# ViacheslavDanilov/oct_segmentation

Measured on AMD Instinct MI355X. Metric: OCT frames/sec (704x704, bf16) fwd+bwd, higher is better.
Workload: dtype bf16; 1 GPU; unetplusplus/resnet101 1-class 704x704, batch 16/GPU, fwd+Dice+bwd+allreduce+Adam; global_batch=16, parallelism=dp1

## Files before the change

include/octseg.h:

```cpp
#ifndef OCTSEG_H
#define OCTSEG_H
#include <stddef.h>
#include <stdint.h>

#ifdef __cplusplus
extern "C" {
#endif

typedef enum {
  OCTSEG_OK = 0,
  OCTSEG_BAD_SHAPE = -1,
  OCTSEG_BAD_DTYPE = -2,
  OCTSEG_UNSUPPORTED_ARCH = -3,
  OCTSEG_HIP_ERROR = -4,
  OCTSEG_BAD_ARG = -5
} octseg_status;

typedef enum { OCTSEG_F32 = 0, OCTSEG_BF16 = 1, OCTSEG_F16 = 2 } octseg_dtype;

typedef struct {
  const char* arch;
  const char* encoder;
  int classes;
  int batch, height, width;
  int dtype;
} octseg_net_desc;

typedef struct octseg_plan octseg_plan;

enum {
  OCTSEG_P_CONV = 0,
  OCTSEG_P_CONVT = 1,
  OCTSEG_P_STEM = 2,
  OCTSEG_P_VEC = 3
};
typedef struct {
  char name[128];
  int kind;
  int R, S, O, I, KP;
  size_t offset;
  size_t numel;
} octseg_param_info;
typedef struct {
  char name[128];
  int C;
  size_t mean_offset, var_offset;
} octseg_bn_info;

int octseg_version(void);
const char* octseg_last_error(void);

int octseg_plan_create(const octseg_net_desc* desc, octseg_plan** out);
int octseg_plan_destroy(octseg_plan* plan);
size_t octseg_plan_workspace_bytes(const octseg_plan* plan);
size_t octseg_plan_param_numel(const octseg_plan* plan);
size_t octseg_plan_buffer_numel(const octseg_plan* plan);
int octseg_plan_num_params(const octseg_plan* plan);
int octseg_plan_param_info(const octseg_plan* plan, int index, octseg_param_info* out);
int octseg_plan_num_bn(const octseg_plan* plan);
int octseg_plan_bn_info(const octseg_plan* plan, int index, octseg_bn_info* out);
double octseg_plan_fwd_macs(const octseg_plan* plan);
int octseg_plan_exec_macs(const octseg_plan* plan, double* out3);
int octseg_plan_find_tensor(const octseg_plan* plan, const char* conv_name, size_t* act_off,
                            size_t* grad_off, int* dims);

int octseg_profile_start(void);
int octseg_profile_stop(double* out);

int octseg_plan_params_changed(octseg_plan* plan);

int octseg_plan_set_dropout(octseg_plan* plan, const float* keep_dev);

int octseg_plan_set_drop_connect(octseg_plan* plan, const float* factors_dev);
int octseg_plan_num_drop_connect(const octseg_plan* plan);
float octseg_plan_drop_connect_rate(const octseg_plan* plan, int index);

int octseg_plan_set_graph(octseg_plan* plan, int enable);

int octseg_net_forward(octseg_plan* plan, const float* params, float* buffers, void* workspace,
                       const float* image, float* logits, int normalize, const float* mean,
                       const float* stdv, int train, void* stream);

#define OCTSEG_AUG_NPARAM 36
int octseg_augment(const float* img, const float* mask, float* img_out, float* mask_out, const float* params, int B,
                   int classes, int H, int W, void* stream);

int octseg_mask_assemble(const float* logits, int N, int classes, int H, int W, int ch, float* out, int out_h, int out_w,
                         int out_channels, int out_ch, const int* row_index, const int* col_index, void* stream);

#define OCTSEG_VOTE_MAX_MEMBERS 64
#define OCTSEG_VOTE_SOFT 0
#define OCTSEG_VOTE_MAJORITY 1
int octseg_vote_assemble(const float* const* logits, const int* classes, const int* ch, const int* view, int M, int N, int H, int W, int mode,
                         float* out, int out_h, int out_w, int out_channels, int out_ch, const int* row_index, const int* col_index, float* prob,
                         uint8_t* dissent, int* stats, void* stream);

#define OCTSEG_CURVE_BINS 256
int octseg_logit_histogram(const float* logits, const float* target, int N, int classes, int H, int W,
                           int* hist, void* stream);

int octseg_ingest_image(const uint8_t* src, int B, int src_h, int src_w, int swap_rb, float* out, int dst_h, int dst_w, const int* xtab,
                        const int* ytab, void* stream);
int octseg_ingest_mask(const uint8_t* src, int B, int src_h, int src_w, int src_channels, const int* channel_ids, int C, float* out, int dst_h,
                       int dst_w, const int* row_index, const int* col_index, void* stream);
int octseg_debug_set_ingest_variant(int variant);

int octseg_render_results(const float* stack, const uint8_t* frames, int N, int H, int W, int stack_channels, const int* class_channels,
                          const uint8_t* class_rgb, int C, const uint8_t* alpha_table, int ring_alpha, int close_iterations, uint8_t* overlay,
                          uint8_t* color_mask, void* stream);

int octseg_epoch_panels(const float* frames, const float* logits, const uint8_t* gt, int N, int S, int C, int src_h, int src_w, int src_channels,
                        const int* row_index, const int* col_index, const int* gt_channels, const uint8_t* class_rgb, const uint8_t* class_ids,
                        uint8_t* panels, uint8_t* labels, void* stream);

int octseg_stack_measure(const float* stack, int N, int H, int W, int stack_channels, const int* ray_pix, const int* ray_len, int R, int* counts,
                         int* radii, void* stream);

int octseg_stack_polar(const float* stack, int N, int H, int W, int stack_channels, const int* ray_pix, const int* ray_len, int R,
                       int* prof, unsigned char* map , void* stream);
int octseg_frames_unwrap(const unsigned char* frames, int N, int H, int W, int channels, const int* ray_pix, const int* ray_len, int R,
                         unsigned char* out, void* stream);

#define OCTSEG_MOMENT_FIELDS 12
#define OCTSEG_SHAPE_MAX_EXTENT 32768
int octseg_stack_moments(const float* stack, int N, int H, int W, int channels, long long* mom, void* stream);
int octseg_moment_origins(const float* stack, const long long* mom, int N, int H, int W, int channels, int ref_channel ,
                          int* origins, void* stream);
int octseg_stack_polar_at(const float* stack, int N, int H, int W, int channels, const int* origins, const int* ray_off, int R, int* prof,
                          int* len, void* stream);

size_t octseg_components_scratch_bytes(int planes, int H, int W);
int octseg_stack_components(const float* stack, int N, int H, int W, int channels, void* scratch, size_t scratch_bytes, int* labels, int* ncomp,
                            int* top, void* stream);
int octseg_stack_cleanup(const float* stack, int N, int H, int W, int channels, int smooth_k, int keep, int min_area, int fill_holes, void* scratch,
                         size_t scratch_bytes, float* out, int* ncomp, int* top, void* stream);

#define OCTSEG_CONTOUR_FIELDS 10
#define OCTSEG_CONTOUR_MAX_VERTICES (1 << 29)
int octseg_stack_contour_counts(const float* stack, int N, int H, int W, int channels, long long* counts, void* stream);
size_t octseg_contours_scratch_bytes(int planes, int H, int W, long long edge_capacity);
int octseg_stack_contours(const float* stack, int N, int H, int W, int channels, void* scratch, size_t scratch_bytes, long long edge_capacity,
                          long long contour_capacity, long long vertex_capacity, int* ncont, int* table, int* vertices, int* overflow,
                          void* stream);

#define OCTSEG_ACROSS_OVERLAP 0
#define OCTSEG_ACROSS_FULL 1
size_t octseg_lesions_scratch_bytes(int channels, int N, int H, int W);
int octseg_volume_components(const float* stack, int N, int H, int W, int channels, int across, void* scratch, size_t scratch_bytes, int* labels,
                             int* nles, int* top, int* profile, void* stream);
int octseg_volume_cleanup(const float* stack, int N, int H, int W, int channels, int across, int keep, int min_voxels, int min_slices, void* scratch,
                          size_t scratch_bytes, float* out, int* nles, int* top, void* stream);

// ... 40 lines not shown
                         const int* xkk, int xksize, const int* ybounds, const int* ykk, int yksize, void* stream);

int octseg_plan_set_frozen_bn(octseg_plan* plan, int on);
int octseg_plan_cam_target(const octseg_plan* plan, size_t* act_off, size_t* grad_off, int* dims);
int octseg_net_backward_seeded(octseg_plan* plan, const float* params, void* workspace, const float* dlogits, void* stream);
size_t octseg_cam_scratch_bytes(int N, int h, int w, int K);
int octseg_cam_maps(int dtype, const void* A, const void* G, int N, int h, int w, int K, int method, int S, void* scratch, float* maps,
                    float threshold, uint8_t* bin, const uint8_t* gt, int gt_h, int gt_w, const int* row_index, const int* col_index, int* counts,
                    const float* frames, const uint8_t* jet_bgr, double image_weight, uint8_t* overlay, void* stream);

int octseg_cam_overlay(const float* maps, const float* frames, const uint8_t* jet_bgr, int N, int S, double image_weight, uint8_t* overlay,
                       void* scratch, void* stream);

typedef enum { OCTSEG_LOSS_DICE = 0, OCTSEG_LOSS_BCE = 1, OCTSEG_LOSS_DICE_BCE = 2 } octseg_loss_kind;
int octseg_plan_set_loss(octseg_plan* plan, int kind);

int octseg_dice_forward(octseg_plan* plan, void* workspace, const float* logits, const float* target,
                        float* loss, long long* stats, void* stream);

int octseg_net_backward(octseg_plan* plan, const float* params, float* grads, void* workspace,
                        const float* logits, const float* target, float grad_scale, void* stream);

int octseg_net_train_step(octseg_plan* plan, const float* params, float* grads, float* buffers, void* workspace, const float* image,
                          const float* target, float* logits, float* loss, long long* stats, int normalize, const float* mean,
                          const float* stdv, float grad_scale, void* stream);
int octseg_plan_set_train_graph(octseg_plan* plan, int enable);

typedef void (*octseg_slice_cb)(void* user, int slice, size_t begin, size_t end);
int octseg_net_backward_sliced(octseg_plan* plan, const float* params, float* grads, void* workspace, const float* logits,
                               const float* target, float grad_scale, void* stream, int nslices, void* comm_stream,
                               octseg_slice_cb cb, void* user);

int octseg_optim_step(int kind, float* params, const float* grads, float* state_m, float* state_v,
                      size_t numel, float lr, float weight_decay, int step, float grad_scale,
                      void* stream);

int octseg_set_deterministic(int on);

int octseg_debug_set_stamp(unsigned long long* dev_buf);
int octseg_debug_set_serial(int on);

size_t octseg_conv2d_scratch_bytes(int dtype, int N, int H, int W, int Cin, int Cout, int R, int S);
int octseg_conv2d_forward(int dtype, const void* x, const float* w, const float* bias, void* y, int N,
                          int H, int W, int Cin, int Cout, int R, int S, int stride, int pad,
                          int transposed, void* scratch, void* stream);
int octseg_conv2d_backward_data(int dtype, const void* dy, const float* w, void* dx, int N, int H, int W,
                                int Cin, int Cout, int R, int S, int stride, int pad, int transposed,
                                void* scratch, void* stream);
int octseg_conv2d_backward_weight(int dtype, const void* x, const void* dy, float* dw, int N, int H,
                                  int W, int Cin, int Cout, int R, int S, int stride, int pad,
                                  int transposed, void* stream);

#define OCTSEG_CONV_MAX_SRC 5
typedef enum { OCTSEG_CONV_FORWARD = 0, OCTSEG_CONV_BACKWARD_DATA = 1, OCTSEG_CONV_BACKWARD_WEIGHT = 2 } octseg_conv_mode;
typedef enum { OCTSEG_ROUTE_THIN = 0, OCTSEG_ROUTE_GEMM1X1, OCTSEG_ROUTE_CONV3X3P, OCTSEG_ROUTE_MFMA16, OCTSEG_ROUTE_MFMA11,
               OCTSEG_ROUTE_MFMA_WIDEN,
               OCTSEG_ROUTE_MFMA11_MASKED, OCTSEG_ROUTE_MFMA16_MASKED } octseg_conv_route;
typedef enum { OCTSEG_WROUTE_THIN = 0, OCTSEG_WROUTE_WGRAD1X1, OCTSEG_WROUTE_CONVT16, OCTSEG_WROUTE_MFMA } octseg_wgrad_route;
typedef struct {
  const void* ptr; const float* scale; const float* shift;
  int C, H, W, up, relu;
} octseg_conv_src;
typedef struct { void* ptr; int accum, pool; } octseg_conv_dst;
typedef struct {
  int N, H, W, Cin, Cout, R, stride, pad, transposed;
  int nsrc;
  octseg_conv_src src[OCTSEG_CONV_MAX_SRC];
  const float* w; const float* wscale; const float* bias;
  int relu_out;
  float* stat_slab; int slab_row0;
  int head;
  octseg_conv_dst dst[OCTSEG_CONV_MAX_SRC];
  const void* dy; float* dW;
  void* scratch; size_t scratch_bytes;
} octseg_conv_layer_desc;
int octseg_conv_layer_op(int mode, int dtype, const octseg_conv_layer_desc* desc, void* stream);
int octseg_conv_layer_route(int mode, int dtype, const octseg_conv_layer_desc* desc, int* route_per_launch, int* nlaunch);
int octseg_conv_layer_slab_rows(int dtype, const octseg_conv_layer_desc* desc, int* rows);

int octseg_tied_layer_op(int pass, int dtype, const octseg_conv_layer_desc* desc, int wg_target, void* stream);
int octseg_tied_layer_route(int pass, int dtype, const octseg_conv_layer_desc* desc, int wg_target, int* route_per_launch, int* nlaunch);
size_t octseg_tied_layer_scratch_bytes(int dtype, const octseg_conv_layer_desc* desc);
int octseg_side_wgs(void);

typedef enum { OCTSEG_STEM_IM2COL = 0, OCTSEG_STEM_FORWARD = 1, OCTSEG_STEM_WGRAD = 2 } octseg_stem_stage;
typedef struct {
  int N, H, W;
  const float* img;
  int normalize; float mean[3], stdv[3];
  int ksize, pad, KP; void* col;
  const float* w; const float* wscale; const float* bias; int relu_out;
  void* y; float* stat_slab; int slab_row0;
  const void* dy; float* dW;
} octseg_stem_desc;
int octseg_stem_op(int stage, int dtype, const octseg_stem_desc* desc, void* stream);
int octseg_stem_slab_rows(int N, int H, int W);

typedef enum {
  OCTSEG_SWEEP_BN_FINALIZE_TRAIN = 0,
  OCTSEG_SWEEP_BN_FINALIZE_SMALL,
  OCTSEG_SWEEP_BN_FINALIZE_EVAL,
  OCTSEG_SWEEP_BN_FINALIZE_FROZEN,
  OCTSEG_SWEEP_BN_ACT,
  OCTSEG_SWEEP_BN_BWD_SMALL,
  OCTSEG_SWEEP_BN_BWD_REDUCE,
  OCTSEG_SWEEP_BN_BWD_FINALIZE,
  OCTSEG_SWEEP_BN_BWD_APPLY,
  OCTSEG_SWEEP_MASKED_ACCUM,
  OCTSEG_SWEEP_POOL2X2_ACCUM,
  OCTSEG_SWEEP_UP2_FILL,
  OCTSEG_SWEEP_RELU,
  OCTSEG_SWEEP_ADD2,
  OCTSEG_SWEEP_DROP_ELEM,
  OCTSEG_SWEEP_MERGE_DROP,
  OCTSEG_SWEEP_DROP_BWD,
  OCTSEG_SWEEP_CHANNEL_SUM,
  OCTSEG_SWEEP_TENSOR_STATS,
  OCTSEG_SWEEP_MAXPOOL_FWD,
  OCTSEG_SWEEP_MAXPOOL_BWD_IDX,
  OCTSEG_SWEEP_BILINEAR_RESIZE,
  OCTSEG_SWEEP_BILINEAR_RESIZE_ADJOINT,
  OCTSEG_SWEEP_BILINEAR_ADJOINT,
  OCTSEG_SWEEP_BIN_MEAN,
  OCTSEG_SWEEP_BIN_MEAN_BWD,
  OCTSEG_SWEEP_IMAGE_SUM,
  OCTSEG_SWEEP_IMAGE_BCAST,
  OCTSEG_SWEEP_SE_GATE,
  OCTSEG_SWEEP_SE_DGATE,
  OCTSEG_SWEEP_PARITY_PERMUTE,
  OCTSEG_SWEEP_MOSAIC,
  OCTSEG_SWEEP_DW_CONV,
  OCTSEG_SWEEP_DW_WGRAD,
  OCTSEG_SWEEP_CAM_SEED,
  OCTSEG_SWEEP_DWG_FWD,
  OCTSEG_SWEEP_DWG_BWD_DATA,
  OCTSEG_SWEEP_DWG_BWD_W,
  OCTSEG_SWEEP_BNX_FWD,
  OCTSEG_SWEEP_BNX_BWD,
  OCTSEG_SWEEP_DICE_BWD,
  OCTSEG_SWEEP_GN_FORWARD,
  OCTSEG_SWEEP_GN_BACKWARD,
  OCTSEG_SWEEP_SEFC_FWD,
  OCTSEG_SWEEP_SEFC_BWD,
  OCTSEG_SWEEP_NUM_OPS
} octseg_sweep;
int octseg_sweep_op(int op, int dtype, const void* const* ptrs, int nptrs, const long long* iargs, int niargs, const double* fargs,
                    int nfargs, void* stream);

typedef enum { OCTSEG_FPA_MAXPOOL2_FWD = 0, OCTSEG_FPA_MAXPOOL2_BWD, OCTSEG_FPA_IN_FWD, OCTSEG_FPA_IN_BWD, OCTSEG_FPA_PYR_FWD, OCTSEG_FPA_PYR_BWD,
               OCTSEG_FPA_MIX_FWD, OCTSEG_FPA_MIX_BWD, OCTSEG_FPA_NUM_STAGES } octseg_fpa_stage;
typedef struct {
  int N, H, W, C, K, train, accum;
  const void* x; void* p; void* dp; void* dx;
  const float* w; const float* b; float* y; const float* dy; float* dw; float* db;
  float* scratch; size_t scratch_floats; float* gscratch; size_t gscratch_floats;
  const float* pw[6]; const float* pb[6]; const float* pg[6]; const float* pbe[6]; float* prm[6]; float* prv[6];
  float* pdw[6]; float* pdb[6]; float* pdg[6]; float* pdbe[6];
  const float* uu; float* duu;
  const void* mid; const void* b1; void* out; const void* g; void* dmid;
} octseg_fpa_desc;
size_t octseg_fpa_scratch_floats(int N, int H, int W);
size_t octseg_fpa_gscratch_floats(int N, int H, int W);
size_t octseg_fpa_uu_offset(int N, int H, int W);
int octseg_fpa_op(int stage, int dtype, const octseg_fpa_desc* desc, void* stream);

typedef enum { OCTSEG_PAB_GEMM = 0, OCTSEG_PAB_SOFTMAX_FWD, OCTSEG_PAB_SOFTMAX_BWD, OCTSEG_PAB_MIX_FWD, OCTSEG_PAB_MIX_BWD, OCTSEG_PAB_NUM_STAGES } octseg_pab_stage;
// ... 17 lines not shown
```

oct_segmentation_amd/_lib.py:

```python
import ctypes as C
import os

def set_hw_queues_for_collectives():
    os.environ.setdefault('GPU_MAX_HW_QUEUES', '8')


if int(os.environ.get('WORLD_SIZE', '1') or 1) > 1:
    set_hw_queues_for_collectives()

import torch

_HERE = os.path.dirname(os.path.abspath(__file__))
LIB_PATH = os.path.join(_HERE, 'liboctseg_hip.so')

F32, BF16, F16 = 0, 1, 2
P_CONV, P_CONVT, P_STEM, P_VEC = 0, 1, 2, 3
OPT_KINDS = {'SGD': 0, 'Adam': 1, 'RMSprop': 2, 'RAdam': 3}


class NetDesc(C.Structure):
    _fields_ = [('arch', C.c_char_p), ('encoder', C.c_char_p), ('classes', C.c_int), ('batch', C.c_int),
                ('height', C.c_int), ('width', C.c_int), ('dtype', C.c_int)]


class ParamInfo(C.Structure):
    _fields_ = [('name', C.c_char * 128), ('kind', C.c_int), ('R', C.c_int), ('S', C.c_int), ('O', C.c_int),
                ('I', C.c_int), ('KP', C.c_int), ('offset', C.c_size_t), ('numel', C.c_size_t)]


class BNInfo(C.Structure):
    _fields_ = [('name', C.c_char * 128), ('C', C.c_int), ('mean_offset', C.c_size_t), ('var_offset', C.c_size_t)]


class ConvSrc(C.Structure):
    _fields_ = [('ptr', C.c_void_p), ('scale', C.c_void_p), ('shift', C.c_void_p), ('C', C.c_int), ('H', C.c_int), ('W', C.c_int),
                ('up', C.c_int), ('relu', C.c_int)]


class ConvDst(C.Structure):
    _fields_ = [('ptr', C.c_void_p), ('accum', C.c_int), ('pool', C.c_int)]


CONV_MAX_SRC = 5


class ConvLayerDesc(C.Structure):
    _fields_ = [('N', C.c_int), ('H', C.c_int), ('W', C.c_int), ('Cin', C.c_int), ('Cout', C.c_int), ('R', C.c_int), ('stride', C.c_int),
                ('pad', C.c_int), ('transposed', C.c_int), ('nsrc', C.c_int), ('src', ConvSrc * CONV_MAX_SRC), ('w', C.c_void_p),
                ('wscale', C.c_void_p), ('bias', C.c_void_p), ('relu_out', C.c_int), ('stat_slab', C.c_void_p), ('slab_row0', C.c_int),
                ('head', C.c_int), ('dst', ConvDst * CONV_MAX_SRC), ('dy', C.c_void_p), ('dW', C.c_void_p), ('scratch', C.c_void_p),
                ('scratch_bytes', C.c_size_t)]


class StemDesc(C.Structure):
    _fields_ = [('N', C.c_int), ('H', C.c_int), ('W', C.c_int), ('img', C.c_void_p), ('normalize', C.c_int), ('mean', C.c_float * 3),
                ('stdv', C.c_float * 3), ('ksize', C.c_int), ('pad', C.c_int), ('KP', C.c_int), ('col', C.c_void_p), ('w', C.c_void_p),
                ('wscale', C.c_void_p), ('bias', C.c_void_p), ('relu_out', C.c_int), ('y', C.c_void_p), ('stat_slab', C.c_void_p),
                ('slab_row0', C.c_int), ('dy', C.c_void_p), ('dW', C.c_void_p)]


_PF6 = C.c_void_p * 6


class FpaDesc(C.Structure):
    _fields_ = ([(k, C.c_int) for k in ('N', 'H', 'W', 'C', 'K', 'train', 'accum')] +
                [(k, C.c_void_p) for k in ('x', 'p', 'dp', 'dx', 'w', 'b', 'y', 'dy', 'dw', 'db')] +
                [('scratch', C.c_void_p), ('scratch_floats', C.c_size_t), ('gscratch', C.c_void_p), ('gscratch_floats', C.c_size_t)] +
                [(k, _PF6) for k in ('pw', 'pb', 'pg', 'pbe', 'prm', 'prv', 'pdw', 'pdb', 'pdg', 'pdbe')] +
                [(k, C.c_void_p) for k in ('uu', 'duu', 'mid', 'b1', 'out', 'g', 'dmid')])


class PabGemm(C.Structure):
    _fields_ = ([(k, C.c_void_p) for k in ('A', 'B', 'C')] +
                [(k, C.c_size_t) for k in ('sAb', 'sAm', 'sAk', 'sBb', 'sBk', 'sBn', 'sCb', 'sCm', 'sCn')] +
                [(k, C.c_int) for k in ('M', 'N', 'K', 'batch', 'a_f32', 'b_f32', 'c_f32', 'accum')])


class PabDesc(C.Structure):
    _fields_ = [('gemm', PabGemm), ('numelA', C.c_size_t), ('numelB', C.c_size_t), ('numelC', C.c_size_t),
                ('S', C.c_void_p), ('P', C.c_void_p), ('batch', C.c_int), ('n', C.c_size_t),
                ('x', C.c_void_p), ('M', C.c_void_p), ('y', C.c_void_p), ('dM', C.c_void_p), ('dy', C.c_void_p), ('N', C.c_int), ('HW', C.c_int),
                ('C', C.c_int)]


_P = C.c_void_p
LOSS_KINDS = {'dice': 0, 'bce': 1, 'dice+bce': 2}
SLICE_CB = C.CFUNCTYPE(None, C.c_void_p, C.c_int, C.c_size_t, C.c_size_t)
SYMBOLS = {
    'octseg_version': (C.c_int, []),
    'octseg_last_error': (C.c_char_p, []),
    'octseg_plan_create': (C.c_int, [C.POINTER(NetDesc), C.POINTER(_P)]),
    'octseg_plan_destroy': (C.c_int, [_P]),
    'octseg_plan_workspace_bytes': (C.c_size_t, [_P]),
    'octseg_plan_param_numel': (C.c_size_t, [_P]),
    'octseg_plan_buffer_numel': (C.c_size_t, [_P]),
    'octseg_plan_num_params': (C.c_int, [_P]),
    'octseg_plan_param_info': (C.c_int, [_P, C.c_int, C.POINTER(ParamInfo)]),
    'octseg_plan_num_bn': (C.c_int, [_P]),
    'octseg_plan_bn_info': (C.c_int, [_P, C.c_int, C.POINTER(BNInfo)]),
    'octseg_plan_fwd_macs': (C.c_double, [_P]),
    'octseg_plan_exec_macs': (C.c_int, [_P, C.POINTER(C.c_double)]),
    'octseg_plan_find_tensor': (C.c_int, [_P, C.c_char_p, C.POINTER(C.c_size_t), C.POINTER(C.c_size_t), C.POINTER(C.c_int)]),
    'octseg_profile_start': (C.c_int, []),
    'octseg_profile_stop': (C.c_int, [C.POINTER(C.c_double)]),
    'octseg_plan_params_changed': (C.c_int, [_P]),
    'octseg_plan_set_dropout': (C.c_int, [_P, _P]),
    'octseg_plan_set_drop_connect': (C.c_int, [_P, _P]),
    'octseg_plan_num_drop_connect': (C.c_int, [_P]),
    'octseg_plan_drop_connect_rate': (C.c_float, [_P, C.c_int]),
    'octseg_plan_set_graph': (C.c_int, [_P, C.c_int]),
    'octseg_net_forward': (C.c_int, [_P, _P, _P, _P, _P, _P, C.c_int, C.POINTER(C.c_float), C.POINTER(C.c_float),
                                     C.c_int, _P]),
    'octseg_augment': (C.c_int, [_P, _P, _P, _P, _P, C.c_int, C.c_int, C.c_int, C.c_int, _P]),
    'octseg_mask_assemble': (C.c_int, [_P, C.c_int, C.c_int, C.c_int, C.c_int, C.c_int, _P, C.c_int, C.c_int, C.c_int, C.c_int, _P, _P, _P]),
    'octseg_vote_assemble': (C.c_int, [_P, _P, _P, _P] + [C.c_int] * 5 + [_P] + [C.c_int] * 4 + [_P] * 6),
    'octseg_logit_histogram': (C.c_int, [_P, _P] + [C.c_int] * 4 + [_P, _P]),
    'octseg_ingest_image': (C.c_int, [_P, C.c_int, C.c_int, C.c_int, C.c_int, _P, C.c_int, C.c_int, _P, _P, _P]),
    'octseg_ingest_mask': (C.c_int, [_P, C.c_int, C.c_int, C.c_int, C.c_int, _P, C.c_int, _P, C.c_int, C.c_int, _P, _P, _P]),
    'octseg_debug_set_ingest_variant': (C.c_int, [C.c_int]),
    'octseg_render_results': (C.c_int, [_P, _P, C.c_int, C.c_int, C.c_int, C.c_int, _P, _P, C.c_int, _P, C.c_int, C.c_int, _P, _P, _P]),
    'octseg_epoch_panels': (C.c_int, [_P, _P, _P] + [C.c_int] * 6 + [_P] * 8),
    'octseg_stack_measure': (C.c_int, [_P, C.c_int, C.c_int, C.c_int, C.c_int, _P, _P, C.c_int, _P, _P, _P]),
    'octseg_stack_polar': (C.c_int, [_P, C.c_int, C.c_int, C.c_int, C.c_int, _P, _P, C.c_int, _P, _P, _P]),
    'octseg_frames_unwrap': (C.c_int, [_P, C.c_int, C.c_int, C.c_int, C.c_int, _P, _P, C.c_int, _P, _P]),
    'octseg_stack_moments': (C.c_int, [_P] + [C.c_int] * 4 + [_P, _P]),
    'octseg_moment_origins': (C.c_int, [_P, _P] + [C.c_int] * 5 + [_P, _P]),
    'octseg_stack_polar_at': (C.c_int, [_P] + [C.c_int] * 4 + [_P, _P, C.c_int, _P, _P, _P]),
    'octseg_components_scratch_bytes': (C.c_size_t, [C.c_int] * 3),
    'octseg_stack_components': (C.c_int, [_P] + [C.c_int] * 4 + [_P, C.c_size_t, _P, _P, _P, _P]),
    'octseg_stack_cleanup': (C.c_int, [_P] + [C.c_int] * 8 + [_P, C.c_size_t, _P, _P, _P, _P]),
    'octseg_stack_contour_counts': (C.c_int, [_P] + [C.c_int] * 4 + [_P, _P]),
    'octseg_contours_scratch_bytes': (C.c_size_t, [C.c_int] * 3 + [C.c_longlong]),
    'octseg_stack_contours': (C.c_int, [_P] + [C.c_int] * 4 + [_P, C.c_size_t] + [C.c_longlong] * 3 + [_P] * 5),
    'octseg_lesions_scratch_bytes': (C.c_size_t, [C.c_int] * 4),
    'octseg_volume_components': (C.c_int, [_P] + [C.c_int] * 5 + [_P, C.c_size_t, _P, _P, _P, _P, _P]),
    'octseg_volume_cleanup': (C.c_int, [_P] + [C.c_int] * 8 + [_P, C.c_size_t, _P, _P, _P, _P]),
    'octseg_match_scratch_bytes': (C.c_size_t, [C.c_int] * 4),
    'octseg_volume_match': (C.c_int, [_P, _P] + [C.c_int] * 5 + [_P, C.c_size_t, _P, _P, _P, _P, _P]),
    'octseg_distance_scratch_bytes': (C.c_size_t, [C.c_int] * 6),
    'octseg_stack_boundary': (C.c_int, [_P] + [C.c_int] * 4 + [_P, C.c_size_t, _P, _P]),
    'octseg_stack_distance': (C.c_int, [_P] + [C.c_int] * 5 + [_P, C.c_size_t, _P, _P]),
    'octseg_pair_distance_counts': (C.c_int, [_P, _P] + [C.c_int] * 5 + [_P] + [C.c_int] * 3 + [_P, C.c_size_t, _P, _P, _P]),
    'octseg_pair_distance_keys': (C.c_int, [_P, _P] + [C.c_int] * 5 + [_P] + [C.c_int] * 3 + [_P, C.c_size_t, C.c_longlong, _P, _P, C.c_longlong,
                                            _P, _P]),
    'octseg_pair_distance_min': (C.c_int, [_P, _P] + [C.c_int] * 5 + [_P] + [C.c_int] * 3 + [_P, C.c_size_t, _P, _P]),
    'octseg_volume_distance_scratch_bytes': (C.c_size_t, [C.c_int] * 7),
    'octseg_volume_boundary': (C.c_int, [_P] + [C.c_int] * 4 + [_P, C.c_size_t, _P, _P]),
    'octseg_volume_distance': (C.c_int, [_P] + [C.c_int] * 6 + [_P, C.c_size_t, _P, _P]),
    'octseg_volume_pair_distance_counts': (C.c_int, [_P, _P] + [C.c_int] * 5 + [_P] + [C.c_int] * 3 + [_P, C.c_size_t, _P, _P, _P]),
    'octseg_volume_pair_distance_keys': (C.c_int, [_P, _P] + [C.c_int] * 5 + [_P] + [C.c_int] * 4 + [_P, C.c_size_t, C.c_longlong, _P, _P,
                                                   C.c_longlong, _P, _P]),
    'octseg_volume_pair_distance_min': (C.c_int, [_P, _P] + [C.c_int] * 5 + [_P] + [C.c_int] * 4 + [_P, C.c_size_t, _P, _P]),
    'octseg_skeleton_scratch_bytes': (C.c_size_t, [C.c_int] * 4),
    'octseg_stack_skeleton': (C.c_int, [_P] + [C.c_int] * 5 + [_P, C.c_size_t, _P, _P, _P]),
    'octseg_volume_normalize': (C.c_int, [_P] + [C.c_int] * 6 + [_P, _P, _P]),
    'octseg_resize_pil_u8': (C.c_int, [_P] + [C.c_int] * 4 + [_P, _P, C.c_int, C.c_int, _P, _P, C.c_int, _P, _P, C.c_int, _P]),
    'octseg_plan_set_frozen_bn': (C.c_int, [_P, C.c_int]),
    'octseg_plan_cam_target': (C.c_int, [_P, C.POINTER(C.c_size_t), C.POINTER(C.c_size_t), C.POINTER(C.c_int)]),
    'octseg_net_backward_seeded': (C.c_int, [_P, _P, _P, _P, _P]),
    'octseg_cam_scratch_bytes': (C.c_size_t, [C.c_int] * 4),
    'octseg_cam_maps': (C.c_int, [C.c_int, _P, _P] + [C.c_int] * 6 + [_P, _P, C.c_float, _P, _P, C.c_int, C.c_int, _P, _P, _P, _P, _P, C.c_double, _P, _P]),
    'octseg_cam_overlay': (C.c_int, [_P, _P, _P, C.c_int, C.c_int, C.c_double, _P, _P, _P]),
    'octseg_plan_set_loss': (C.c_int, [_P, C.c_int]),
    'octseg_dice_forward': (C.c_int, [_P, _P, _P, _P, _P, _P, _P]),
    'octseg_net_backward': (C.c_int, [_P, _P, _P, _P, _P, _P, C.c_float, _P]),
    'octseg_net_train_step': (C.c_int, [_P, _P, _P, _P, _P, _P, _P, _P, _P, _P, C.c_int, C.POINTER(C.c_float), C.POINTER(C.c_float),
                                        C.c_float, _P]),
    'octseg_plan_set_train_graph': (C.c_int, [_P, C.c_int]),
    'octseg_net_backward_sliced': (C.c_int, [_P, _P, _P, _P, _P, _P, C.c_float, _P, C.c_int, _P, SLICE_CB, _P]),
    'octseg_optim_step': (C.c_int, [C.c_int, _P, _P, _P, _P, C.c_size_t, C.c_float, C.c_float, C.c_int, C.c_float, _P]),
    'octseg_set_deterministic': (C.c_int, [C.c_int]),
    'octseg_debug_set_stamp': (C.c_int, [_P]),
    'octseg_debug_set_serial': (C.c_int, [C.c_int]),
    'octseg_conv2d_scratch_bytes': (C.c_size_t, [C.c_int] * 8),
    'octseg_conv2d_forward': (C.c_int, [C.c_int, _P, _P, _P, _P] + [C.c_int] * 10 + [_P, _P]),
    'octseg_conv2d_backward_data': (C.c_int, [C.c_int, _P, _P, _P] + [C.c_int] * 10 + [_P, _P]),
    'octseg_conv2d_backward_weight': (C.c_int, [C.c_int, _P, _P, _P] + [C.c_int] * 10 + [_P]),
    'octseg_conv_layer_op': (C.c_int, [C.c_int, C.c_int, C.POINTER(ConvLayerDesc), _P]),
    'octseg_conv_layer_route': (C.c_int, [C.c_int, C.c_int, C.POINTER(ConvLayerDesc), C.POINTER(C.c_int), C.POINTER(C.c_int)]),
    'octseg_conv_layer_slab_rows': (C.c_int, [C.c_int, C.POINTER(ConvLayerDesc), C.POINTER(C.c_int)]),
    'octseg_tied_layer_op': (C.c_int, [C.c_int, C.c_int, C.POINTER(ConvLayerDesc), C.c_int, _P]),
    'octseg_tied_layer_route': (C.c_int, [C.c_int, C.c_int, C.POINTER(ConvLayerDesc), C.c_int, C.POINTER(C.c_int), C.POINTER(C.c_int)]),
    'octseg_tied_layer_scratch_bytes': (C.c_size_t, [C.c_int, C.POINTER(ConvLayerDesc)]),
    'octseg_side_wgs': (C.c_int, []),
    'octseg_stem_op': (C.c_int, [C.c_int, C.c_int, C.POINTER(StemDesc), _P]),
    'octseg_stem_slab_rows': (C.c_int, [C.c_int] * 3),
    'octseg_sweep_op': (C.c_int, [C.c_int, C.c_int, C.POINTER(_P), C.c_int, C.POINTER(C.c_longlong), C.c_int, C.POINTER(C.c_double), C.c_int, _P]),
    'octseg_fpa_scratch_floats': (C.c_size_t, [C.c_int] * 3),
    'octseg_fpa_gscratch_floats': (C.c_size_t, [C.c_int] * 3),
    'octseg_fpa_uu_offset': (C.c_size_t, [C.c_int] * 3),
    'octseg_fpa_op': (C.c_int, [C.c_int, C.c_int, C.POINTER(FpaDesc), _P]),
    'octseg_pab_op': (C.c_int, [C.c_int, C.c_int, C.POINTER(PabDesc), _P]),
}

_lib = None


def lib():
    global _lib
    if _lib is None:
        if not os.path.exists(LIB_PATH):
            raise RuntimeError(
                f'{LIB_PATH} not found: build it with `python -c "import __graft_entry__ as g; g.build()"` '
                f'(or `make -C oct_segmentation_amd/csrc`). There is no CPU fallback.')
        h = C.CDLL(LIB_PATH)
        for name, (res, args) in SYMBOLS.items():
            fn = getattr(h, name)
            fn.restype = res
            fn.argtypes = args
        _lib = h
    return _lib


def check(rc):
    if rc != 0:
        msg = lib().octseg_last_error().decode()
        if 'Expected more than 1 value per channel' in msg:
            raise ValueError(msg)
        raise RuntimeError(f'octseg error {rc}: {msg}')


def ptr(t):
    return None if t is None else C.c_void_p(t.data_ptr())


def stream_ptr():
    import torch
    return C.c_void_p(torch.cuda.current_stream().cuda_stream)
```

oct_segmentation_amd/csrc/api.cpp:

```cpp
#include "plan_internal.h"

#include <cctype>

using namespace octseg;
using namespace octseg::detail;

static std::string lower(const char* s) {
  std::string r(s ? s : "");
  for (auto& c : r) c = (char)tolower((unsigned char)c);
  return r;
}

template <class Outside, class Body>
static int graph_call(octseg_plan* p, bool train, bool same_key, hipGraphExec_t& exec, int& seen, hipStream_t st, Outside&& outside, Body&& body) {
  if (!same_key) {
    if (exec) { (void)hipGraphExecDestroy(exec); exec = nullptr; }
    seen = 0;
  }
  if (const int rc = outside()) return rc;
  auto replay = [&]() -> int { HIPCHK(hipGraphLaunch(exec, st)); if (train) p->packed_valid = false; return OCTSEG_OK; };
  if (exec) return replay();
  if (seen++ == 0) return body();
  if (train) p->packed_valid = false;
  hipGraph_t g = nullptr;
  HIPCHK(hipStreamBeginCapture(st, hipStreamCaptureModeThreadLocal));
  g_capturing = train;
  const int rc = body();
  g_capturing = false;
  const hipError_t ce = hipStreamEndCapture(st, &g);
  if (train) p->packed_valid = false;
  hipError_t ie = hipSuccess;
  if (!rc && ce == hipSuccess && (ie = hipGraphInstantiate(&exec, g, nullptr, nullptr, 0)) != hipSuccess) exec = nullptr;
  if (g) (void)hipGraphDestroy(g);
  if (rc) return rc;
  if (ce != hipSuccess) return fail(OCTSEG_HIP_ERROR, std::string(train ? "training-step capture: " : "") + hipGetErrorString(ce));
  if (ie != hipSuccess) return fail(OCTSEG_HIP_ERROR, hipGetErrorString(ie));
  return replay();
}

extern "C" {

int octseg_version(void) { return 100; }
const char* octseg_last_error(void) { return g_err.c_str(); }

int octseg_plan_create(const octseg_net_desc* d, octseg_plan** out) {
  if (!d || !out) return fail(OCTSEG_BAD_ARG, "null argument");
  *out = nullptr;
  if (d->dtype != OCTSEG_F32 && d->dtype != OCTSEG_BF16 && d->dtype != OCTSEG_F16) return fail(OCTSEG_BAD_DTYPE, "dtype must be f32, bf16 or f16");
  if (d->height <= 0 || d->width <= 0 || d->height % 32 != 0 || d->width % 32 != 0) {
    char buf[256];
    snprintf(buf, sizeof buf, "Wrong input shape height=%d, width=%d. Expected image height and width divisible by 32.",
             d->height, d->width);
    return fail(OCTSEG_BAD_SHAPE, buf);
  }
  if (d->batch <= 0 || d->classes <= 0 || d->classes > 16) return fail(OCTSEG_BAD_SHAPE, "batch > 0 and 1 <= classes <= 16 required");
  const std::string enc = lower(d->encoder);
  if (enc != "resnet18" && enc != "resnet34" && enc != "resnet50" && enc != "resnet101" && enc != "resnet152" && enc != "timm-regnetx_002" &&
      enc != "timm-regnetx_064" && enc != "timm-regnety_120" && enc != "efficientnet-b0" && enc != "efficientnet-b5" && enc != "efficientnet-b7")
    return fail(OCTSEG_UNSUPPORTED_ARCH, "unknown encoder '" + enc + "' (resnet18 | resnet34 | resnet50 | resnet101 | resnet152 | timm-regnetx_002 | timm-regnetx_064 | timm-regnety_120 | efficientnet-b0 | efficientnet-b5 | efficientnet-b7)");
  octseg_plan* P = new octseg_plan();
  P->arch = lower(d->arch); P->encoder = enc; P->classes = d->classes;
  P->B = d->batch; P->H = d->height; P->W = d->width; P->dtype = d->dtype;
  const int rc = build_plan(P);
  if (rc) { delete P; return rc; }
  *out = P;
  return OCTSEG_OK;
}
int octseg_plan_destroy(octseg_plan* p) {
  if (p) {
    if (p->side) (void)hipStreamDestroy(p->side);
    if (p->side_bwd) (void)hipStreamDestroy(p->side_bwd);
    if (p->ev_fork) (void)hipEventDestroy(p->ev_fork);
    if (p->ev_join) (void)hipEventDestroy(p->ev_join);
    if (p->ev_slice) (void)hipEventDestroy(p->ev_slice);
    if (p->graph_exec) (void)hipGraphExecDestroy(p->graph_exec);
    if (p->tgraph_exec) (void)hipGraphExecDestroy(p->tgraph_exec);
  }
  delete p;
  return OCTSEG_OK;
}
size_t octseg_plan_workspace_bytes(const octseg_plan* p) { return p ? p->ws_bytes : 0; }
size_t octseg_plan_param_numel(const octseg_plan* p) { return p ? p->param_numel : 0; }
size_t octseg_plan_buffer_numel(const octseg_plan* p) { return p ? p->buffer_numel : 0; }
int octseg_plan_num_params(const octseg_plan* p) { return p ? (int)p->params.size() : 0; }
int octseg_plan_num_bn(const octseg_plan* p) { return p ? (int)p->bns.size() : 0; }
double octseg_plan_fwd_macs(const octseg_plan* p) { return p ? p->fwd_macs : 0.0; }
int octseg_plan_exec_macs(const octseg_plan* p, double* out3) {
  if (p == nullptr || out3 == nullptr) return OCTSEG_BAD_ARG;
  for (int k = 0; k < 3; ++k) out3[k] = p->exec_macs[k];
  return OCTSEG_OK;
}

int octseg_plan_param_info(const octseg_plan* p, int i, octseg_param_info* o) {
  if (!p || !o || i < 0 || i >= (int)p->params.size()) return fail(OCTSEG_BAD_ARG, "param index out of range");
  const ParamInfo& q = p->params[i];
  memset(o, 0, sizeof(*o));
  snprintf(o->name, sizeof o->name, "%s", q.name.c_str());
  o->kind = q.kind; o->R = q.R; o->S = q.S; o->O = q.O; o->I = q.I; o->KP = q.KP; o->offset = q.off; o->numel = q.numel;
  return OCTSEG_OK;
}
int octseg_plan_bn_info(const octseg_plan* p, int i, octseg_bn_info* o) {
  if (!p || !o || i < 0 || i >= (int)p->bns.size()) return fail(OCTSEG_BAD_ARG, "bn index out of range");
  const BNInfo& b = p->bns[i];
  memset(o, 0, sizeof(*o));
  snprintf(o->name, sizeof o->name, "%s", b.name.c_str());
  o->C = b.C; o->mean_offset = b.rm_off; o->var_offset = b.rv_off;
  return OCTSEG_OK;
}

int octseg_profile_start(void) {
  for (auto& r : g_prof) { g_prof_pool.push_back(r.a); g_prof_pool.push_back(r.b); }
  g_prof.clear();
  g_prof_on = true;
  return OCTSEG_OK;
}
int octseg_profile_stop(double* out) {
  g_prof_on = false;
  if (!out) return fail(OCTSEG_BAD_ARG, "null argument");
  HIPCHK(hipDeviceSynchronize());
  for (int i = 0; i < 12; ++i) out[i] = 0.0;
  FILE* dump = nullptr;
  if (const char* path = getenv("OCTSEG_PROFILE_DUMP")) dump = fopen(path, "w");
  if (dump) fprintf(dump, "layer,class,ms,gflop,tflops\n");
  for (auto& r : g_prof) {
    float ms = 0.f;
    HIPCHK(hipEventElapsedTime(&ms, r.a, r.b));
    out[3 * r.kind] += ms; out[3 * r.kind + 1] += r.flops; out[3 * r.kind + 2] += 1.0;
    if (dump) fprintf(dump, "%s,%s,%.4f,%.3f,%.1f\n", r.name.c_str(), r.kind == 0 ? "fwd" : r.kind == 1 ? "dgrad" : r.kind == 2 ? "wgrad" : "hbm", ms,
                      r.flops / 1e9, ms > 0 ? r.flops / (ms * 1e-3) / 1e12 : 0.0);
  }
  if (dump) fclose(dump);
  for (auto& r : g_prof) { g_prof_pool.push_back(r.a); g_prof_pool.push_back(r.b); }
  g_prof.clear();
  return OCTSEG_OK;
}

int octseg_plan_find_tensor(const octseg_plan* p, const char* conv_name, size_t* act_off, size_t* grad_off, int* dims) {
  if (!p || !conv_name) return fail(OCTSEG_BAD_ARG, "null argument");
  for (auto& L : p->convs)
    if (L.name == conv_name && L.out >= 0) {
      const TensorInfo& t = p->tensors[L.out];
      if (act_off) *act_off = t.off;
      if (grad_off) *grad_off = t.goff;
      if (dims) { dims[0] = t.N; dims[1] = t.H; dims[2] = t.W; dims[3] = t.C; }
      return OCTSEG_OK;
    }
  return fail(OCTSEG_BAD_ARG, std::string("no conv layer named ") + conv_name);
}

int octseg_plan_params_changed(octseg_plan* p) {
  if (!p) return fail(OCTSEG_BAD_ARG, "null argument");
  p->packed_valid = false;
  return OCTSEG_OK;
}

int octseg_net_forward(octseg_plan* p, const float* params, float* buffers, void* workspace, const float* image,
                       float* logits, int normalize, const float* mean, const float* stdv, int train, void* stream) {
  if (!p || !params || !buffers || !workspace || !image || !logits) return fail(OCTSEG_BAD_ARG, "null argument");
  if (normalize && (!mean || !stdv)) return fail(OCTSEG_BAD_ARG, "normalize=1 needs mean/std");
  if (train && p->dtype == OCTSEG_F16)
    return fail(OCTSEG_BAD_DTYPE, "f16 is a serving dtype (eval forwards, reference predict.py); train in bf16 or f32");
  Exec E{p, params, nullptr, buffers, (char*)workspace, (hipStream_t)stream, train};
  if (train || !p->graph_enabled) return run_forward(E, image, logits, normalize, mean, stdv);
  octseg_plan::GraphKey key{params, buffers, workspace, image, logits, stream, normalize, {0, 0, 0}, {1, 1, 1}};
  if (normalize) for (int i = 0; i < 3; ++i) { key.mean[i] = mean[i]; key.stdv[i] = stdv[i]; }
  const bool same_key = key == p->graph_key;
  p->graph_key = key;
  return graph_call(p, false, same_key, p->graph_exec, p->graph_seen, E.st, [&] { return pack_all_weights(E, true); },
                    [&] { return run_forward(E, image, logits, normalize, mean, stdv); });
}

int octseg_plan_set_graph(octseg_plan* p, int enable) {
  if (!p) return fail(OCTSEG_BAD_ARG, "null argument");
  p->graph_enabled = enable != 0;
  if (!enable && p->graph_exec) { (void)hipGraphExecDestroy(p->graph_exec); p->graph_exec = nullptr; p->graph_seen = 0; }
  return OCTSEG_OK;
}

int octseg_plan_set_dropout(octseg_plan* p, const float* keep_dev) {
  if (!p) return fail(OCTSEG_BAD_ARG, "null argument");
  p->dropout_keep = keep_dev;
  return OCTSEG_OK;
}

int octseg_augment(const float* img, const float* mask, float* img_out, float* mask_out, const float* params, int B, int classes, int H,
                   int W, void* stream) {
  if (!img || !mask || !img_out || !mask_out || !params) return fail(OCTSEG_BAD_ARG, "null argument");
  if (B <= 0 || classes <= 0 || H <= 0 || W <= 0) return fail(OCTSEG_BAD_SHAPE, "augment: empty batch or frame");
  if (img == img_out || mask == mask_out) return fail(OCTSEG_BAD_ARG, "augment: outputs must not alias the inputs (gather)");
  HIPCHK(launch_augment(img, mask, img_out, mask_out, params, B, classes, H, W, (hipStream_t)stream));
  return OCTSEG_OK;
}

int octseg_mask_assemble(const float* logits, int N, int classes, int H, int W, int ch, float* out, int out_h, int out_w,
                         int out_channels, int out_ch, const int* row_index, const int* col_index, void* stream) {
  if (!logits || !out) return fail(OCTSEG_BAD_ARG, "null argument");
  if (N <= 0 || classes <= 0 || H <= 0 || W <= 0 || out_h <= 0 || out_w <= 0 || ch < 0 || ch >= classes || out_ch < 0 ||
      out_ch >= out_channels)
    return fail(OCTSEG_BAD_SHAPE, "mask_assemble: channel / extent out of range");
  HIPCHK(launch_mask_assemble(logits, N, classes, H, W, ch, out, out_h, out_w, out_channels, out_ch, row_index, col_index,
                              (hipStream_t)stream));
  return OCTSEG_OK;
}

static int g_ingest_variant = 0;
int octseg_debug_set_ingest_variant(int variant) {
  if (variant != 0 && variant != 1) return fail(OCTSEG_BAD_ARG, "ingest variant must be 0 (staged) or 1 (per-pixel gather)");
  g_ingest_variant = variant;
  return OCTSEG_OK;
}

int octseg_ingest_image(const uint8_t* src, int B, int src_h, int src_w, int swap_rb, float* out, int dst_h, int dst_w, const int* xtab,
                        const int* ytab, void* stream) {
  if (!src || !out || !xtab || !ytab) return fail(OCTSEG_BAD_ARG, "null argument");
  if (B <= 0 || src_h <= 0 || src_w <= 0 || dst_h <= 0 || dst_w <= 0) return fail(OCTSEG_BAD_SHAPE, "ingest_image: empty batch or frame");
  HIPCHK(launch_ingest_image(src, B, src_h, src_w, swap_rb != 0, out, dst_h, dst_w, xtab, ytab, g_ingest_variant, (hipStream_t)stream));
  return OCTSEG_OK;
}

int octseg_ingest_mask(const uint8_t* src, int B, int src_h, int src_w, int src_channels, const int* channel_ids, int C, float* out, int dst_h,
                       int dst_w, const int* row_index, const int* col_index, void* stream) {
  if (!src || !out || !channel_ids || !row_index || !col_index) return fail(OCTSEG_BAD_ARG, "null argument");
  if (B <= 0 || src_h <= 0 || src_w <= 0 || src_channels <= 0 || C <= 0 || dst_h <= 0 || dst_w <= 0)
    return fail(OCTSEG_BAD_SHAPE, "ingest_mask: empty batch, frame or class list");
  HIPCHK(launch_ingest_mask(src, B, src_h, src_w, src_channels, channel_ids, C, out, dst_h, dst_w, row_index, col_index, g_ingest_variant,
                            (hipStream_t)stream));
  return OCTSEG_OK;
}

int octseg_render_results(const float* stack, const uint8_t* frames, int N, int H, int W, int stack_channels, const int* class_channels,
                          const uint8_t* class_rgb, int C, const uint8_t* alpha_table, int ring_alpha, int close_iterations, uint8_t* overlay,
                          uint8_t* color_mask, void* stream) {
  if (!stack || !frames || !class_channels || !class_rgb || !alpha_table || !overlay || !color_mask) return fail(OCTSEG_BAD_ARG, "null argument");
  if (N <= 0 || H <= 0 || W <= 0 || stack_channels <= 0 || C <= 0 || C > 16)
    return fail(OCTSEG_BAD_SHAPE, "render_results: empty batch or frame, or not 1..16 classes");
// ... 386 lines not shown
```

oct_segmentation_amd/csrc/conv_api.cpp:

```cpp
#include "plan_internal.h"

using namespace octseg;
using namespace octseg::detail;

namespace {

struct Built {
  std::vector<ConvArgs> conv;
  std::vector<WgradArgs> wg;
  bool convt16 = false;
  ConvPackInfo pk{};
  int rows = 0;
};

bool aligned(const void* p) { return ((uintptr_t)p & 15) == 0; }

int build(int mode, int dtype, const octseg_conv_layer_desc* d, Built& B) {
  const std::string who = "conv_layer_op: ";
  auto bad_arg = [&](const char* m) { return fail(OCTSEG_BAD_ARG, who + m); };
  auto bad_shape = [&](const char* m) { return fail(OCTSEG_BAD_SHAPE, who + m); };
  if (mode != OCTSEG_CONV_FORWARD && mode != OCTSEG_CONV_BACKWARD_DATA && mode != OCTSEG_CONV_BACKWARD_WEIGHT) return bad_arg("unknown mode");
  if (dtype != OCTSEG_F32 && dtype != OCTSEG_BF16 && dtype != OCTSEG_F16) return fail(OCTSEG_BAD_DTYPE, who + "dtype must be f32, bf16 or f16");
  if (dtype == OCTSEG_F16 && mode != OCTSEG_CONV_FORWARD) return fail(OCTSEG_BAD_DTYPE, who + "f16 is the serving dtype: no gradient kernels");
  if (d == nullptr) return bad_arg("null descriptor");
// ... 158 lines not shown
  if (rc != OCTSEG_OK) return rc;
  int n = 0;
  if (mode == OCTSEG_CONV_BACKWARD_WEIGHT) {
    if (B.convt16) route_per_launch[n++] = OCTSEG_WROUTE_CONVT16;
    else
      for (auto& a : B.wg) {
        const WgradRoute r = wgrad_route(a, dtype);
        route_per_launch[n++] = a.ntaps <= 0 ? -1 : r == WROUTE_THIN ? OCTSEG_WROUTE_THIN : r == WROUTE_1X1 ? OCTSEG_WROUTE_WGRAD1X1 : OCTSEG_WROUTE_MFMA;
      }
  } else {
    for (auto& a : B.conv) route_per_launch[n++] = public_route(a, dtype);
  }
  *nlaunch = n;
  return OCTSEG_OK;
}

int octseg_conv_layer_slab_rows(int dtype, const octseg_conv_layer_desc* d, int* rows) {
  if (rows == nullptr) return fail(OCTSEG_BAD_ARG, "conv_layer_slab_rows: null output");
  Built B;
  const int rc = build(OCTSEG_CONV_FORWARD, dtype, d, B);
  if (rc != OCTSEG_OK) return rc;
  *rows = B.rows;
  return OCTSEG_OK;
}

}

namespace {

constexpr size_t TIE_TAB_BYTES = 512, TIE_PREFIX_BYTES = 512;
static_assert(4 * sizeof(PackJob) <= TIE_TAB_BYTES, "the job table fits its slot");

struct Tied {
  int Ca = 0, Cs = 0, ns = 0;
  Geom gu{}, gs{};
  TieImages im{};
  TieOffsets at{};
  size_t dk4_off = 0, bytes = 0;
  std::vector<PackJob> jobs; std::vector<unsigned long long> prefix; unsigned long long total = 0;
  std::vector<ConvArgs> conv;
  std::vector<WgradArgs> wg;
  bool convt16 = false, masked = false;
};

int tied_shape(int dtype, const octseg_conv_layer_desc* d, Tied& B) {
  const std::string who = "tied_layer_op: ";
  auto bad_shape = [&](const char* m) { return fail(OCTSEG_BAD_SHAPE, who + m); };
  if (dtype != OCTSEG_F32 && dtype != OCTSEG_BF16 && dtype != OCTSEG_F16) return fail(OCTSEG_BAD_DTYPE, who + "dtype must be f32, bf16 or f16");
  if (dtype != OCTSEG_BF16) return fail(OCTSEG_BAD_DTYPE, who + "the tied decomposition is a bf16 training path");
  if (d == nullptr) return fail(OCTSEG_BAD_ARG, who + "null descriptor");
  if (d->N < 1 || d->H < 1 || d->W < 1 || d->Cin < 1 || d->Cout < 1) return bad_shape("empty tensor");
  if (d->nsrc < 1 || d->nsrc > MAX_SRC) return bad_shape("1 .. 5 sources");
  if ((long long)d->N * d->H * d->W * std::max(d->Cin, d->Cout) >= (1ll << 31)) return bad_shape("tensor of 2^31 elements or more");
  int c = 0;
  TieQuery q{};
  q.esz = (int)dtype_size(dtype); q.transposed = d->transposed != 0; q.head = d->head != 0; q.has_bn = true; q.has_bias = d->bias != nullptr;
  q.R = q.S = d->R; q.stride = d->stride; q.pad = d->pad; q.nsrc = d->nsrc;
  q.up0_whole_grad = d->src[0].up == 1; q.skips_plain_grad = true;
  for (int i = 0; i < d->nsrc; ++i) {
    const octseg_conv_src& s = d->src[i];
    if (s.C < 1 || s.C % 8 != 0) return bad_shape("a source's C is not a whole number of 16-byte vectors");
    if (s.up != 0 && s.up != 1) return fail(OCTSEG_BAD_ARG, who + "up is 0 or 1");
    if ((s.H << s.up) != d->H || (s.W << s.up) != d->W) return bad_shape("a source's stored extent is not H >> up x W >> up");
    if (i > 0 && s.up) q.skips_plain_grad = false;
    c += s.C;
  }
  if (c != d->Cin) return bad_shape("the sources' channels do not add up to Cin");
  q.Ca = d->src[0].C; q.Cs = d->Cin - q.Ca; q.Cout = d->Cout;
  if (d->Cout % 8 != 0) return bad_shape("Cout is not a whole number of 16-byte vectors");
  if (!tie_eligible(q)) return bad_shape("the plan would not tie this layer (tie_eligible: src[0] nearest x2 with >= 64 channels, plain skips of 0 or >= 32, 3x3 stride 1 pad 1, Cout >= 32)");
  B.Ca = q.Ca; B.Cs = q.Cs; B.ns = d->nsrc;
  B.gu = Geom{4, 4, 2, 1, true, d->N, d->H / 2, d->W / 2, B.Ca, d->H, d->W, d->Cout};
  B.gs = Geom{3, 3, 1, 1, false, d->N, d->H, d->W, B.Cs, d->H, d->W, d->Cout};
  B.im = tie_images(dtype, B.gu, B.gs);
  size_t off = TIE_TAB_BYTES + TIE_PREFIX_BYTES;
  B.at.fu = off; off += align_up(conv_image_bytes(B.im.pk_fu, 16));
  B.at.du = off; off += align_up(conv_image_bytes(B.im.pk_du, B.im.du_taps()));
  if (B.Cs > 0) {
    B.at.fs = off; off += align_up(conv_image_bytes(B.im.pk_fs, 9));
    B.at.ds = off; off += align_up(conv_image_bytes(B.im.pk_ds, 9));
  }
  B.dk4_off = off; off += align_up(((size_t)16 * B.Ca + (size_t)9 * B.Cs) * d->Cout * sizeof(float));
  B.bytes = off;
  tie_pack_jobs(B.im, B.at, 0, d->Cout, d->Cin, B.Ca, B.Cs, B.jobs, B.prefix, B.total);
  return OCTSEG_OK;
}

int tied_build(int pass, int dtype, const octseg_conv_layer_desc* d, int wg_target, Tied& B) {
  const std::string who = "tied_layer_op: ";
  auto bad_arg = [&](const char* m) { return fail(OCTSEG_BAD_ARG, who + m); };
  if (pass != OCTSEG_CONV_FORWARD && pass != OCTSEG_CONV_BACKWARD_DATA && pass != OCTSEG_CONV_BACKWARD_WEIGHT) return bad_arg("unknown pass");
  const int rc = tied_shape(dtype, d, B);
  if (rc != OCTSEG_OK) return rc;
  const bool fwd = pass == OCTSEG_CONV_FORWARD, dgrad = pass == OCTSEG_CONV_BACKWARD_DATA;
  if (wg_target < 0) return bad_arg("negative wg_target");
  if (d->wscale || d->bias || d->relu_out || d->stat_slab || d->slab_row0 || d->head)
    return bad_arg("wscale, bias, relu_out, the slab and head mode are not part of a tied pass (training only; the statistics are a sweep of their own)");
  if (!aligned(d->w) || !aligned(d->dy) || !aligned(d->dW) || !aligned(d->scratch)) return bad_arg("misaligned pointer");
  if (d->scratch == nullptr) return bad_arg("null scratch");
  if (d->scratch_bytes < B.bytes) return bad_arg("scratch smaller than octseg_tied_layer_scratch_bytes()");
  SrcDesc src[MAX_SRC];
  int c0 = 0;
  for (int i = 0; i < d->nsrc; ++i) {
    const octseg_conv_src& s = d->src[i];
    if (!dgrad && (s.scale != nullptr) != (s.shift != nullptr)) return bad_arg("scale and shift come together");
    if (!dgrad && s.relu && s.scale == nullptr) return bad_arg("relu without the affine (the plan never builds it)");
    if (!dgrad && (s.ptr == nullptr || !aligned(s.ptr) || !aligned(s.scale) || !aligned(s.shift))) return bad_arg("null or misaligned source pointer");
    SrcDesc o;
    o.ptr = s.ptr; o.scale = dgrad ? nullptr : s.scale; o.shift = dgrad ? nullptr : s.shift; o.C = s.C; o.c0 = c0; o.H = s.H; o.W = s.W; o.up = s.up;
    o.relu = s.relu ? 1 : 0;
    src[i] = o;
    c0 += s.C;
  }
  char* ws = (char*)d->scratch;
  const int O = d->Cout;
  if (fwd) {
    if (d->w == nullptr) return bad_arg("null weight");
    if (d->dst[0].ptr == nullptr || !aligned(d->dst[0].ptr)) return bad_arg("null or misaligned destination");
    if (d->dst[0].accum || d->dst[0].pool) return bad_arg("the tied forward stores its output (no accum, no pool)");
    DstDesc dd;
    dd.ptr = d->dst[0].ptr; dd.C = O; dd.c0 = 0; dd.cn = O; dd.H = d->H; dd.W = d->W; dd.accum = 0; dd.pool = 0;
    if (B.Cs > 0) {
      std::vector<ConvArgs> v;
      fwd_launches(B.gs, v);
      ConvArgs& a = v[0];
      a.nsrc = B.ns - 1;
      for (int i = 1; i < B.ns; ++i) { a.src[i - 1] = src[i]; a.src[i - 1].c0 -= B.Ca; }
      a.W = ws + B.at.fs;
      a.dst[0] = dd; a.ndst = 1; a.out_mode = OUT_STORE;
      B.conv.push_back(a);
    }
    std::vector<ConvArgs> v;
    fwd_launches(B.gu, v);
    for (auto& a : v) {
      a.nsrc = 1; a.src[0] = src[0]; a.src[0].up = 0; a.src[0].c0 = 0;
      a.W = ws + B.at.fu;
      dd.accum = B.Cs > 0 ? 1 : 0;
      a.dst[0] = dd; a.ndst = 1; a.out_mode = OUT_STORE;
      B.conv.push_back(a);
    }
  } else if (dgrad) {
    if (d->w == nullptr || d->dy == nullptr) return bad_arg("null weight or dy");
    for (int i = 0; i < d->nsrc; ++i) {
      if (d->dst[i].ptr == nullptr || !aligned(d->dst[i].ptr)) return bad_arg("null or misaligned destination");
      if (d->dst[i].pool) return bad_arg("pool: the tied data gradient is computed at the low resolution, nothing is pooled");
    }
    const size_t esz = dtype_size(dtype);
    std::vector<ConvArgs> lu;
    B.masked = B.im.du_masked;
    if (B.masked) { lu.resize(1); tied_dgrad_masked(B.gu, lu[0]); }
    else dgrad_launches(B.gu, lu);
    for (int k = 0; k < (int)lu.size(); ++k) {
      ConvArgs& a = lu[k];
      if (B.masked) {
        for (int p = 0; p < 4; ++p) {
          SrcDesc& s = a.src[p];
          s.ptr = (const char*)d->dy + ((size_t)(p >> 1) * d->W + (p & 1)) * O * esz;
          s.scale = nullptr; s.shift = nullptr; s.C = 2 * O; s.c0 = p * O; s.H = d->H / 2; s.W = d->W; s.up = 0; s.relu = 0;
        }
      } else {
        SrcDesc s;
        s.ptr = d->dy; s.scale = nullptr; s.shift = nullptr; s.C = O; s.c0 = 0; s.H = d->H; s.W = d->W; s.up = 0; s.relu = 0;
        a.src[0] = s; a.nsrc = 1;
        a.Cin = O;
      }
      a.W = ws + B.at.du;
      DstDesc t;
      t.ptr = d->dst[0].ptr; t.C = B.Ca; t.c0 = 0; t.cn = B.Ca; t.H = d->H / 2; t.W = d->W / 2; t.accum = k == 0 ? (d->dst[0].accum ? 1 : 0) : 1; t.pool = 0;
      a.dst[0] = t; a.ndst = 1; a.out_mode = OUT_STORE; a.bias = nullptr; a.stat_slab = nullptr;
      B.conv.push_back(a);
    }
    if (B.Cs > 0) {
      std::vector<ConvArgs> ls;
      dgrad_launches(B.gs, ls);
      ConvArgs& a = ls[0];
      SrcDesc s;
      s.ptr = d->dy; s.scale = nullptr; s.shift = nullptr; s.C = O; s.c0 = 0; s.H = d->H; s.W = d->W; s.up = 0; s.relu = 0;
      a.src[0] = s; a.nsrc = 1;
      a.Cin = O;
      a.W = ws + B.at.ds;
      int nd = 0, cc = 0;
      for (int i = 1; i < d->nsrc; ++i) {
        DstDesc t;
        t.ptr = d->dst[i].ptr; t.C = src[i].C; t.c0 = cc; t.cn = src[i].C; t.H = d->H; t.W = d->W; t.accum = d->dst[i].accum ? 1 : 0; t.pool = 0;
        a.dst[nd++] = t;
        cc += src[i].C;
      }
      a.ndst = nd; a.out_mode = OUT_STORE; a.bias = nullptr; a.stat_slab = nullptr;
      B.conv.push_back(a);
    }
  } else {
    if (d->dy == nullptr || d->dW == nullptr) return bad_arg("null dy or dW");
    float* dK4 = (float*)(ws + B.dk4_off);
    float* dW3s = dK4 + (size_t)16 * O * B.Ca;
    wgrad_launches(B.gu, B.wg);
    for (auto& a : B.wg) {
      a.nsrc = 1; a.src[0] = src[0]; a.src[0].up = 0; a.src[0].c0 = 0;
      a.dy = d->dy; a.dyC = O; a.dW = dK4; a.stamp = nullptr;
      a.wg_target = wg_target;
    }
    B.convt16 = wgrad_convt16_eligible(B.wg[0], dtype);
    if (B.Cs > 0) {
      std::vector<WgradArgs> lw;
      wgrad_launches(B.gs, lw);
      WgradArgs& a = lw[0];
      a.nsrc = B.ns - 1;
      for (int i = 1; i < B.ns; ++i) { a.src[i - 1] = src[i]; a.src[i - 1].c0 -= B.Ca; }
      a.dy = d->dy; a.dyC = O; a.dW = dW3s; a.stamp = nullptr;
      a.wg_target = wg_target;
      B.wg.push_back(a);
    }
  }
  return OCTSEG_OK;
}

int tied_route_of(const ConvArgs& a, int dtype) {
  const int r = public_route(a, dtype);
  if (a.taps_per_src == 0) return r;
  return r == OCTSEG_ROUTE_MFMA11 ? OCTSEG_ROUTE_MFMA11_MASKED : r == OCTSEG_ROUTE_MFMA16 ? OCTSEG_ROUTE_MFMA16_MASKED : r;
}

}

extern "C" {

int octseg_tied_layer_op(int pass, int dtype, const octseg_conv_layer_desc* d, int wg_target, void* stream) {
  Tied B;
  const int rc = tied_build(pass, dtype, d, wg_target, B);
  if (rc != OCTSEG_OK) return rc;
  hipStream_t st = (hipStream_t)stream;
  char* ws = (char*)d->scratch;
  if (pass == OCTSEG_CONV_BACKWARD_WEIGHT) {
    const size_t O = d->Cout;
    float* dK4 = (float*)(ws + B.dk4_off);
    float* dW3s = dK4 + (size_t)16 * O * B.Ca;
    HIPCHK(hipMemsetAsync(dK4, 0, ((size_t)16 * B.Ca + (size_t)9 * B.Cs) * O * sizeof(float), st));
    if (B.convt16) HIPCHK(launch_wgrad_convt16(dtype, B.wg[0], st));
    else
      for (int k = 0; k < 4; ++k) HIPCHK(launch_wgrad(dtype, B.wg[k], st));
    if (B.Cs > 0) HIPCHK(launch_wgrad(dtype, B.wg[4], st));
    HIPCHK(launch_tied_fold(dK4, B.Cs > 0 ? dW3s : nullptr, d->dW, d->Cout, B.Ca, B.Cs, st));
    return OCTSEG_OK;
  }
  HIPCHK(hipMemcpyAsync(ws, B.jobs.data(), B.jobs.size() * sizeof(PackJob), hipMemcpyHostToDevice, st));
  HIPCHK(hipMemcpyAsync(ws + TIE_TAB_BYTES, B.prefix.data(), B.prefix.size() * sizeof(unsigned long long), hipMemcpyHostToDevice, st));
  HIPCHK(hipStreamSynchronize(st));
  HIPCHK(launch_pack_all(dtype, d->w, ws, (const PackJob*)ws, (const unsigned long long*)(ws + TIE_TAB_BYTES), (int)B.jobs.size(), B.total, 0, st));
  for (auto& a : B.conv) HIPCHK(launch_conv(dtype, a, st));
  return OCTSEG_OK;
}

int octseg_tied_layer_route(int pass, int dtype, const octseg_conv_layer_desc* d, int wg_target, int* route_per_launch, int* nlaunch) {
  if (route_per_launch == nullptr || nlaunch == nullptr) return fail(OCTSEG_BAD_ARG, "tied_layer_route: null output");
  Tied B;
  const int rc = tied_build(pass, dtype, d, wg_target, B);
  if (rc != OCTSEG_OK) return rc;
  int n = 0;
  if (pass == OCTSEG_CONV_BACKWARD_WEIGHT) {
    auto name = [&](const WgradArgs& a) {
      const WgradRoute r = wgrad_route(a, dtype);
      return a.ntaps <= 0 ? -1 : r == WROUTE_THIN ? (int)OCTSEG_WROUTE_THIN : r == WROUTE_1X1 ? (int)OCTSEG_WROUTE_WGRAD1X1 : (int)OCTSEG_WROUTE_MFMA;
    };
    if (B.convt16) route_per_launch[n++] = OCTSEG_WROUTE_CONVT16;
    else
      for (int k = 0; k < 4; ++k) route_per_launch[n++] = name(B.wg[k]);
    if (B.Cs > 0) route_per_launch[n++] = name(B.wg[4]);
  } else {
    for (auto& a : B.conv) route_per_launch[n++] = tied_route_of(a, dtype);
  }
  *nlaunch = n;
  return OCTSEG_OK;
}

size_t octseg_tied_layer_scratch_bytes(int dtype, const octseg_conv_layer_desc* d) {
  Tied B;
  return tied_shape(dtype, d, B) == OCTSEG_OK ? B.bytes : 0;
}

int octseg_side_wgs(void) { return side_wgs(); }

}
```

oct_segmentation_amd/csrc/elementwise.hip:

```cpp
#include "common.h"
#include "ev.h"

#include <cstdlib>
#include <type_traits>
#include "kernels.h"
#include "sigmoid.h"

namespace octseg {

__device__ __forceinline__ bool slab_sum(const float* __restrict__ slab, int rows, int C, int cpb, double* part, unsigned* counters,
                                         double& s1, double& s2, int& c) {
  __shared__ double red[1280][2];
  __shared__ unsigned is_last;
  const int sh = __ffs(cpb) - 1, RL = (int)blockDim.x >> sh, pitch = cpb + 1;
  const int rl = threadIdx.x >> sh, cl = threadIdx.x & (cpb - 1);
  const int G = gridDim.y;
  c = blockIdx.x * cpb + cl;
  const int per = (rows + G - 1) / G;
  const int r0 = blockIdx.y * per, r1 = min(rows, r0 + per);
  s1 = 0.0; s2 = 0.0;
  if (c < C) {
    int r = r0 + rl;
    for (; r + 7 * RL < r1; r += 8 * RL) {
      float2 v[8];
// ... 869 lines not shown
  constexpr int MAXV = MAXC / VEC;
  const size_t npix = (size_t)a.B * a.HW;
  const bool want_dice = a.loss_kind != LOSS_BCE, want_bce = a.loss_kind != LOSS_DICE;
  const float bce_scale = grad_scale / ((float)a.B * (float)a.C * (float)a.HW);
  for (size_t p = (size_t)blockIdx.x * blockDim.x + threadIdx.x; p < npix; p += (size_t)gridDim.x * blockDim.x) {
    const size_t b = p / a.HW, i = p - b * a.HW;
    float d[MAXC];
#pragma unroll
    for (int c = 0; c < MAXC; ++c) {
      d[c] = 0.f;
      if (c < a.C) {
        const float I = (float)a.sums[c * DICE_NS], S = (float)a.sums[c * DICE_NS + 1], Tt = (float)a.sums[c * DICE_NS + 2];
        if (want_bce) {
          const float z = a.logits[(b * a.C + c) * a.HW + i], t = a.target[(b * a.C + c) * a.HW + i];
          d[c] = (sigmoid_acc(z) - t) * bce_scale;
        }
        if (want_dice && Tt > 0.f) {
          const float z = a.logits[(b * a.C + c) * a.HW + i], t = a.target[(b * a.C + c) * a.HW + i];
          const float e = expf(-fabsf(z));
          const float dpdz = e / ((1.0f + e) * (1.0f + e));
          float dscore;
          if (S > 1e-7f) dscore = (2.0f * t * S - 2.0f * I) / (S * S);
          else dscore = 2.0f * t / 1e-7f;
          d[c] += -dscore * dpdz * grad_scale / (float)a.C;
        }
      }
    }
    const size_t row = p * (size_t)(CP / VEC);
#pragma unroll
    for (int v = 0; v < MAXV; ++v)
      if (v < CP / VEC) stv<T>(dl, row + v, EV<T>::pack(d + v * VEC));
  }
}
hipError_t launch_dice_bwd(int dtype, const DiceArgs& a, float grad_scale, void* dlogits, int CP, hipStream_t st) {
  OCTSEG_NO_F16(dtype);
  if (a.C > CP || CP > 16 || CP % 8 != 0) return hipErrorInvalidValue;
  const size_t npix = (size_t)a.B * a.HW;
  const int gr = grid_for(npix, 256);
  OCTSEG_LAUNCH_TRAIN(dice_bwd_kernel, dim3(gr), dim3(256), a, grad_scale, dlogits, CP);
  return hipGetLastError();
}

template <typename T>
__global__ __launch_bounds__(256) void pack_image_kernel(const float* w, void* img, int taps, int O, int I, int transpose,
                                                         int BN, int RB, int nchunks, int ntiles, const float* oscale) {
  constexpr int VEC = EV<T>::VEC;
  const int VPR = RB / 16, KC = RB / (int)sizeof(T), swz_div = 256 / RB;
  const int rows = transpose ? I : O, K = transpose ? O : I;
  const size_t total = (size_t)taps * nchunks * ntiles * BN * VPR;
  for (size_t v = (size_t)blockIdx.x * blockDim.x + threadIdx.x; v < total; v += (size_t)gridDim.x * blockDim.x) {
    size_t rem = v;
    const int q = (int)(rem % VPR); rem /= VPR;
    const int row = (int)(rem % BN); rem /= BN;
    const int nt = (int)(rem % ntiles); rem /= ntiles;
    const int chunk = (int)(rem % nchunks);
    const int tap = (int)(rem / nchunks);
    const int lq = q ^ ((row / swz_div) & (VPR - 1));
    const int co = nt * BN + row, c0 = chunk * KC + lq * VEC;
    float x[VEC];
#pragma unroll
    for (int i = 0; i < VEC; ++i) {
      const int c = c0 + i;
      float val = 0.f;
      if (co < rows && c < K) val = transpose ? w[((size_t)tap * O + c) * I + co] : w[((size_t)tap * O + co) * I + c];
      if (oscale != nullptr && !transpose && co < rows) val *= oscale[co];
      x[i] = val;
    }
    stv<T>(img, v, EV<T>::pack(x));
  }
}
hipError_t launch_pack_weight_image(int dtype, const float* w, void* img, int taps, int O, int I, int transpose,
                                    const ConvPackInfo& p, hipStream_t st, const float* oscale) {
  const size_t total = (size_t)taps * p.nchunks * p.ntiles * p.BN * (p.RB / 16);
  const int gr = grid_for(total, 256, 4096);
  if (dtype == DT_F16)
    hipLaunchKernelGGL(pack_image_kernel<f16_t>, dim3(gr), dim3(256), 0, st, w, img, taps, O, I, transpose, p.BN, p.RB, p.nchunks, p.ntiles, oscale);
  else if (dtype == DT_F32)
    hipLaunchKernelGGL(pack_image_kernel<float>, dim3(gr), dim3(256), 0, st, w, img, taps, O, I, transpose, p.BN, p.RB, p.nchunks, p.ntiles, oscale);
  else
    hipLaunchKernelGGL(pack_image_kernel<bf16_t>, dim3(gr), dim3(256), 0, st, w, img, taps, O, I, transpose, p.BN, p.RB, p.nchunks, p.ntiles, oscale);
  return hipGetLastError();
}

template <typename T>
__global__ __launch_bounds__(256) void pack_all_kernel(const float* params, char* ws, const PackJob* tab, const unsigned long long* prefix,
                                                       int njobs, unsigned long long total, int fold) {
  constexpr int VEC = EV<T>::VEC;
  for (unsigned long long g = (unsigned long long)blockIdx.x * blockDim.x + threadIdx.x; g < total; g += (unsigned long long)gridDim.x * blockDim.x) {
    int lo = 0, hi = njobs - 1;
    while (lo < hi) {
      const int mid = (lo + hi + 1) >> 1;
      if (prefix[mid] <= g) lo = mid; else hi = mid - 1;
    }
    const PackJob jb = tab[lo];
    if (fold && jb.src_I != 0) continue;
    const float* w = params + jb.src_off;
    const int VPR = jb.RB / 16, KC = jb.RB / (int)sizeof(T), swz_div = 256 / jb.RB;
    const int rows = jb.transpose ? jb.I : jb.O, K = jb.transpose ? jb.O : jb.I, sI = jb.src_I ? jb.src_I : jb.I;
    size_t rem = (size_t)(g - prefix[lo]);
    const size_t v = rem;
    const int q = (int)(rem % VPR); rem /= VPR;
    const int row = (int)(rem % jb.BN); rem /= jb.BN;
    const int nt = (int)(rem % jb.ntiles); rem /= jb.ntiles;
    const int chunk = (int)(rem % jb.nchunks);
    const int tap = (int)(rem / jb.nchunks);
    const int lq = q ^ ((row / swz_div) & (VPR - 1));
    const int co = nt * jb.BN + row, c0 = chunk * KC + lq * VEC;
    float osc = 1.f;
    if (fold && !jb.transpose && jb.scale_off != ~(size_t)0 && co < rows) osc = ((const float*)(ws + jb.scale_off))[co];
    float x[VEC];
#pragma unroll
    for (int i = 0; i < VEC; ++i) {
      const int c = c0 + i;
      float val = 0.f;
      if (jb.tied == 2) {
        if (co < jb.I && c < 4 * jb.O) {
          const int p = c / jb.O, o = c - p * jb.O;
          const int u = (p >> 1) + 1 + 2 * (tap / 3 - 1), vv = (p & 1) + 1 + 2 * (tap % 3 - 1);
          if (u >= 0 && u <= 3 && vv >= 0 && vv <= 3)
            for (int r3 = max(0, 2 - u); r3 <= min(2, 3 - u); ++r3)
              for (int s3 = max(0, 2 - vv); s3 <= min(2, 3 - vv); ++s3) val += w[((size_t)(r3 * 3 + s3) * jb.O + o) * sI + co + jb.src_c0];
        }
      } else if (co < rows && c < K) {
        const int o = jb.transpose ? c : co, ci = (jb.transpose ? co : c) + jb.src_c0;
        if (!jb.tied) val = w[((size_t)tap * jb.O + o) * sI + ci];
        else {
          const int u = tap >> 2, vv = tap & 3;
          for (int r3 = max(0, 2 - u); r3 <= min(2, 3 - u); ++r3)
            for (int s3 = max(0, 2 - vv); s3 <= min(2, 3 - vv); ++s3) val += w[((size_t)(r3 * 3 + s3) * jb.O + o) * sI + ci];
        }
        if (!jb.transpose) val *= osc;
      }
      x[i] = val;
    }
    stv<T>(ws + jb.dst_off, v, EV<T>::pack(x));
  }
}
hipError_t launch_pack_all(int dtype, const float* params, void* ws, const PackJob* tab, const unsigned long long* prefix, int njobs,
                           unsigned long long total, int fold, hipStream_t st) {
  const int gr = grid_for((size_t)total, 256, 8192);
  if (dtype == DT_F16) hipLaunchKernelGGL(pack_all_kernel<f16_t>, dim3(gr), dim3(256), 0, st, params, (char*)ws, tab, prefix, njobs, total, fold);
  else if (dtype == DT_F32) hipLaunchKernelGGL(pack_all_kernel<float>, dim3(gr), dim3(256), 0, st, params, (char*)ws, tab, prefix, njobs, total, fold);
  else hipLaunchKernelGGL(pack_all_kernel<bf16_t>, dim3(gr), dim3(256), 0, st, params, (char*)ws, tab, prefix, njobs, total, fold);
  return hipGetLastError();
}

__global__ __launch_bounds__(256) void tied_fold_kernel(const float* dK4, const float* dW3s, float* dW3, int O, int Ca, int Cs) {
  const int I = Ca + Cs;
  const size_t total = (size_t)9 * O * I;
  for (size_t idx = (size_t)blockIdx.x * blockDim.x + threadIdx.x; idx < total; idx += (size_t)gridDim.x * blockDim.x) {
    const int i = (int)(idx % I);
    const int o = (int)((idx / I) % O);
    const int t = (int)(idx / ((size_t)I * O));
    float val;
    if (i < Ca) {
      const int r3 = t / 3, s3 = t - 3 * r3;
      val = 0.f;
      for (int u = 2 - r3; u <= 3 - r3; ++u)
        for (int v = 2 - s3; v <= 3 - s3; ++v) val += dK4[((size_t)(u * 4 + v) * O + o) * Ca + i];
    } else {
      val = dW3s[((size_t)t * O + o) * Cs + (i - Ca)];
    }
    dW3[idx] += val;
  }
}
hipError_t launch_tied_fold(const float* dK4, const float* dW3s, float* dW3, int O, int Ca, int Cs, hipStream_t st) {
  hipLaunchKernelGGL(tied_fold_kernel, dim3(grid_for((size_t)9 * O * (Ca + Cs), 256)), dim3(256), 0, st, dK4, dW3s, dW3, O, Ca, Cs);
  return hipGetLastError();
}

__global__ __launch_bounds__(256) void mask_assemble_kernel(const float* logits, int N, int C, int SH, int SW, int ch, float* out, int OH,
                                                            int OW, int OC, int out_ch, const int* rows, const int* cols) {
  const size_t total = (size_t)N * OH * OW;
  for (size_t i = (size_t)blockIdx.x * blockDim.x + threadIdx.x; i < total; i += (size_t)gridDim.x * blockDim.x) {
    const int x = (int)(i % OW);
    const int y = (int)((i / OW) % OH);
    const int n = (int)(i / ((size_t)OW * OH));
    int sy = rows ? rows[y] : (int)(((long long)(2 * y + 1) * SH) / (2 * OH));
    int sx = cols ? cols[x] : (int)(((long long)(2 * x + 1) * SW) / (2 * OW));
    sy = min(max(sy, 0), SH - 1); sx = min(max(sx, 0), SW - 1);
    const float z = logits[(((size_t)n * C + ch) * SH + sy) * SW + sx];
    out[i * OC + out_ch] = sigmoid_acc(z) > 0.5f ? 1.f : 0.f;
  }
}
hipError_t launch_mask_assemble(const float* logits, int N, int C, int SH, int SW, int ch, float* out, int OH, int OW, int OC, int out_ch,
                                const int* rows, const int* cols, hipStream_t st) {
  hipLaunchKernelGGL(mask_assemble_kernel, dim3(grid_for((size_t)N * OH * OW, 256)), dim3(256), 0, st, logits, N, C, SH, SW, ch, out, OH, OW,
                     OC, out_ch, rows, cols);
  return hipGetLastError();
}

__global__ __launch_bounds__(256) void optim_kernel(const OptArgs a, float bc1, float bc2, float radam_rect, int radam_use) {
  for (size_t i = (size_t)blockIdx.x * blockDim.x + threadIdx.x; i < a.n; i += (size_t)gridDim.x * blockDim.x) {
    float p = a.p[i];
    float g = a.g[i] * a.grad_scale;
    if (a.wd != 0.f) g = fmaf(a.wd, p, g);
    if (a.kind == 0) {
      p -= a.lr * g;
    } else if (a.kind == 2) {
      float v = a.alpha * a.v[i] + (1.f - a.alpha) * g * g;
      a.v[i] = v;
      p -= a.lr * g / (sqrtf(v) + a.eps);
    } else {
      float m = a.m[i] + (g - a.m[i]) * (1.f - a.beta1);
      float v = a.beta2 * a.v[i] + (1.f - a.beta2) * g * g;
      a.m[i] = m; a.v[i] = v;
      if (a.kind == 1) {
        const float denom = sqrtf(v) / sqrtf(bc2) + a.eps;
        p -= (a.lr / bc1) * (m / denom);
      } else {
        const float mhat = m / bc1;
        if (radam_use) p -= mhat * a.lr * (sqrtf(bc2) / (sqrtf(v) + a.eps)) * radam_rect;
        else p -= mhat * a.lr;
      }
    }
    a.p[i] = p;
  }
}
hipError_t launch_optim_step(const OptArgs& a, hipStream_t st) {
  const double b1t = pow((double)a.beta1, (double)a.step), b2t = pow((double)a.beta2, (double)a.step);
  const float bc1 = (float)(1.0 - b1t), bc2 = (float)(1.0 - b2t);
  float rect = 1.f; int use = 0;
  if (a.kind == 3) {
    const double rho_inf = 2.0 / (1.0 - (double)a.beta2) - 1.0;
    const double rho_t = rho_inf - 2.0 * a.step * b2t / (1.0 - b2t);
    if (rho_t > 5.0) {
// ... 10 lines not shown
```

oct_segmentation_amd/csrc/kernels.h:

```cpp
#pragma once
#include "common.h"

namespace octseg {

int conv_num_mtiles(const ConvArgs& a, int dtype);
int conv_num_mtiles_flat(const ConvArgs& a, int dtype);
struct ConvPackInfo { int BN, RB, nchunks, ntiles; };
ConvPackInfo conv_pack_info(const ConvArgs& a, int dtype);
static inline size_t conv_image_bytes(const ConvPackInfo& p, int wtaps) {
  return (size_t)wtaps * p.nchunks * p.ntiles * p.BN * p.RB;
}
hipError_t launch_conv(int dtype, const ConvArgs& a, hipStream_t st);
enum ConvRoute { ROUTE_THIN, ROUTE_GEMM1X1, ROUTE_CONV3X3P, ROUTE_MFMA };
enum ConvTile { TILE_16, TILE_11, TILE_WIDE_N };
ConvRoute conv_route(const ConvArgs& a, int dtype);
int conv_mfma_tile(const ConvArgs& a, int dtype);
bool conv_masked_eligible(const ConvArgs& a, int dtype);

bool gemm1x1_eligible(const ConvArgs& a, int dtype);
int gemm1x1_rows(const ConvArgs& a);
hipError_t launch_gemm1x1(int dtype, const ConvArgs& a, hipStream_t st);

bool deterministic_mode();

// ... 87 lines not shown
hipError_t launch_bn_finalize_train(const float* slab, int rows, int C, double count, const float* gamma,
                                    const float* beta, float* running_mean, float* running_var,
                                    float momentum, float eps, float* scale, float* shift, float* mean,
                                    float* rstd, double* part, unsigned* counters, hipStream_t st);
constexpr int SLAB_PART_CAP = 16384;
constexpr int BN_SMALL_COUNT = 1024;
hipError_t launch_bn_finalize_small(int dtype, const void* y, int count, int C, const float* gamma, const float* beta, float* running_mean,
                                    float* running_var, float momentum, float eps, float* scale, float* shift, float* mean, float* rstd,
                                    hipStream_t st);
hipError_t launch_bn_finalize_eval(int C, const float* gamma, const float* beta, const float* running_mean,
                                   const float* running_var, float eps, float* scale, float* shift,
                                   hipStream_t st);

hipError_t launch_bn_finalize_frozen(int C, const float* gamma, const float* beta, const float* running_mean, const float* running_var, float eps,
                                     float* scale, float* shift, float* mean, float* rstd, float* coef, hipStream_t st);

struct BnEvalJob { size_t gamma_off, beta_off, rm_off, rv_off , ss_off ; int C;
                   size_t bias_off;
                   float eps;        };
hipError_t launch_bn_finalize_eval_all(const float* params, const float* buffers, void* ws, const BnEvalJob* tab, const unsigned* prefix,
                                       int njobs, unsigned total, float eps, hipStream_t st);

struct BnActArgs {
  const void* y; const float* scale; const float* shift;
  const void* res; const float* rscale; const float* rshift;
  const void* post;
  void* out; size_t npix; int C; int relu;
  unsigned char* maskbits;
};
hipError_t launch_bn_act(int dtype, const BnActArgs& a, hipStream_t st);

struct BnBwdArgs {
  const void* g; const void* y; const void* out;
  const unsigned char* maskbits;
  const float* scale; const float* shift; const float* mean; const float* rstd; const float* gamma;
  size_t npix; int C; int mask;
  float* slab; int rows;
  float* dgamma; float* dbeta;
  float* coef;
  void* dy;
  double* part; unsigned* counters;
  void* res_grad; int res_store;
};

hipError_t launch_bn_bwd_small(int dtype, const BnBwdArgs& a, hipStream_t st);
hipError_t launch_bn_bwd_reduce(int dtype, const BnBwdArgs& a, hipStream_t st);
hipError_t launch_bn_bwd_finalize(const BnBwdArgs& a, hipStream_t st);
hipError_t launch_bn_bwd_apply(int dtype, const BnBwdArgs& a, hipStream_t st);

hipError_t launch_masked_accum(int dtype, void* dst, const void* g, const void* out_mask, size_t n, int store,
                               hipStream_t st);
hipError_t launch_pool2x2_accum(int dtype, void* dst, const void* src, int N, int H, int W, int C, int store,
                                hipStream_t st);
hipError_t launch_channel_sum(int dtype, const void* g, size_t npix, int Cstride, int C, float* out,
                              hipStream_t st);

hipError_t launch_maxpool_fwd(int dtype, const void* in, void* out, unsigned char* idx ,
                              int N, int H, int W, int C, hipStream_t st);
hipError_t launch_maxpool_bwd_idx(int dtype, const unsigned char* idx, const void* gout, void* gin, int N, int H, int W, int C, int store,
                                  hipStream_t st);
hipError_t launch_stem_im2col(int dtype, const float* img, void* col, int N, int H, int W, int KP,
                              const float* mean, const float* stdv, int normalize, hipStream_t st, int ksize = 7, int pad = -1 );

constexpr int DICE_NS = 4;
enum { LOSS_DICE = 0, LOSS_BCE = 1, LOSS_DICE_BCE = 2 };
struct DiceArgs {
  const float* logits; const float* target; int B, C; size_t HW;
  int loss_kind;
  double* sums;
  long long* stats;
  float* loss;
};
hipError_t launch_dice_fwd(const DiceArgs& a, hipStream_t st);
hipError_t launch_dice_bwd(int dtype, const DiceArgs& a, float grad_scale, void* dlogits, int CP,
                           hipStream_t st);

hipError_t launch_pack_weight_image(int dtype, const float* w, void* img, int taps, int O, int I, int transpose,
                                    const ConvPackInfo& p, hipStream_t st, const float* oscale = nullptr);

struct PackJob { size_t src_off , dst_off ; int taps, O, I, transpose, BN, RB, nchunks, ntiles;
                 size_t scale_off;
                 int src_I;
                 int src_c0;
                 int tied;          };
hipError_t launch_tied_fold(const float* dK4, const float* dW3s, float* dW3, int O, int Ca, int Cs, hipStream_t st);
hipError_t launch_pack_all(int dtype, const float* params, void* ws, const PackJob* tab, const unsigned long long* prefix, int njobs,
                           unsigned long long total, int fold, hipStream_t st);

struct GnArgs {
  const void* y;
  const void* g; void* dy;
  void* out;
  const float* gamma; const float* beta; float* dgamma; float* dbeta;
  float* part;
  float* ss;
  float* stat;
  float* coef;
  size_t HW; int C, G, cpg; float eps;
};
int gn_num_slabs(size_t HW);
hipError_t launch_gn_forward(int dtype, const GnArgs& a, int N, int H, int W, int up, hipStream_t st);
hipError_t launch_gn_backward(int dtype, const GnArgs& a, int N, hipStream_t st);
hipError_t launch_bilinear_adjoint(int dtype, const void* gout, void* gin, int N, int H, int W, int C, int up, hipStream_t st);
hipError_t launch_up2_fill(int dtype, const void* in, void* out, int N, int H, int W, int C, hipStream_t st);
hipError_t launch_merge_drop(int dtype, const void* a0, const void* a1, const void* a2, const void* a3, const float* m, float mscale, void* out,
                             int N, size_t HW, int C, hipStream_t st);
hipError_t launch_drop_bwd(int dtype, const void* gout, const float* m, float mscale, void* gin, int N, size_t HW, int C, hipStream_t st);
hipError_t launch_bilinear_nchw(const float* z, float* out, int NC, int H, int W, int up, hipStream_t st);

hipError_t launch_parity_permute(int dtype, const void* src, void* dst, int N, int H, int W, int C, int to_coarse, int accum, hipStream_t st);
hipError_t launch_dw_conv(int dtype, const void* in, int inC, int ic0, void* out, int outC, int oc0, const float* w, int wC, int wc0, int N, int H,
                          int W, int C, int dil, int flip, int accum, hipStream_t st);
hipError_t launch_dw_wgrad(int dtype, const void* in, int inC, int ic0, const void* gout, int goC, int oc0, float* dw, int wC, int wc0, int N, int H,
                           int W, int C, int dil, hipStream_t st);
hipError_t launch_image_sum(int dtype, const void* in, void* out, int N, int HW, int C, float div, hipStream_t st);
hipError_t launch_image_bcast(int dtype, const void* in, void* out, int N, int HW, int C, float scale, int accum, hipStream_t st);
hipError_t launch_drop_elem(int dtype, const void* in, const float* keep, float mscale, void* out, size_t numel, hipStream_t st);
hipError_t launch_bilinear_up(int dtype, const void* in, void* out, int N, int H, int W, int C, int up, hipStream_t st);
hipError_t launch_mosaic(int dtype, const void* src, void* dst, int N, int H, int W, int C, int r, int to_mosaic, int accum, hipStream_t st);
hipError_t launch_tensor_stats(int dtype, const void* y, size_t npix, int C, float* slab, int rows, hipStream_t st);
hipError_t launch_bin_mean(int dtype, const void* in, void* out, int N, int H, int W, int C, int k, hipStream_t st);
hipError_t launch_bin_mean_bwd(int dtype, const void* gout, void* gin, int N, int H, int W, int C, int k, int accum, hipStream_t st);
hipError_t launch_bilinear_resize(int dtype, const void* in, void* out, int N, int IH, int IW, int OH, int OW, int C, hipStream_t st);
hipError_t launch_bilinear_resize_adjoint(int dtype, const void* gout, void* gin, int N, int IH, int IW, int OH, int OW, int C, hipStream_t st);
bool bilinear_adjoint_grid(long long npx, int& gy, int& gz);
hipError_t launch_relu(int dtype, const void* in, const void* mask, void* out, size_t numel, hipStream_t st);

hipError_t launch_mask_assemble(const float* logits, int N, int C, int SH, int SW, int ch, float* out, int OH, int OW, int OC, int out_ch,
                                const int* rows, const int* cols, hipStream_t st);

constexpr int VOTE_MAX_MEMBERS = 64;
struct VoteArgs {
  const float* z[VOTE_MAX_MEMBERS]; int classes[VOTE_MAX_MEMBERS], ch[VOTE_MAX_MEMBERS], view[VOTE_MAX_MEMBERS];
  int M, N, H, W, mode;
  float* out; int OH, OW, OC, out_ch;
  const int* rows; const int* cols;
  float* prob; uint8_t* dissent; int* stats;
};
hipError_t launch_vote_assemble(const VoteArgs& a, hipStream_t st);

constexpr int CURVE_BINS = 256;
hipError_t launch_logit_histogram(const float* logits, const float* target, int N, int classes, int H, int W, int* hist, hipStream_t st);

constexpr int AUG_NPARAM = 36;
hipError_t launch_augment(const float* img, const float* mask, float* img_out, float* mask_out, const float* params, int B, int C, int H,
                          int W, hipStream_t st);

hipError_t launch_ingest_image(const uint8_t* src, int B, int Hs, int Ws, int swap_rb, float* out, int Hd, int Wd, const int* xtab,
                               const int* ytab, int variant, hipStream_t st);
hipError_t launch_ingest_mask(const uint8_t* src, int B, int Hs, int Ws, int Cs, const int* ch_ids, int C, float* out, int Hd, int Wd,
                              const int* rows, const int* cols, int variant, hipStream_t st);

hipError_t launch_render_results(const float* stack, const uint8_t* frames, int N, int H, int W, int SC, const int* class_ch,
                                 const uint8_t* class_rgb, int C, const uint8_t* alpha_tab, int ring_alpha, int iters, uint8_t* overlay,
                                 uint8_t* cmask, hipStream_t st);

hipError_t launch_epoch_panels(const float* frames, const float* logits, const uint8_t* gt, int N, int S, int C, int Hs, int Ws, int SC,
                               const int* rows, const int* cols, const int* gt_ch, const uint8_t* class_rgb, const uint8_t* class_ids,
                               uint8_t* panels, uint8_t* labels, hipStream_t st);

hipError_t launch_stack_measure(const float* stack, int N, int H, int W, int SC, const int* ray_pix, const int* ray_len, int R, int* counts,
                                int* radii, hipStream_t st);

hipError_t launch_stack_polar(const float* stack, int N, int H, int W, int SC, const int* ray_pix, const int* ray_len, int R, int* prof,
                              uint8_t* map, hipStream_t st);
hipError_t launch_frames_unwrap(const uint8_t* frames, int N, int H, int W, int C, const int* ray_pix, const int* ray_len, int R, uint8_t* out,
                                hipStream_t st);

constexpr int SHAPE_MOMENT_FIELDS = 12;
constexpr int SHAPE_MAX_EXTENT = 32768;
// ... 79 lines not shown
```

oct_segmentation_amd/csrc/plan.h:

```cpp
#pragma once
#include <string>
#include <vector>
#include "common.h"
#include "kernels.h"
#include "../../include/octseg.h"

namespace octseg {

struct TensorInfo {
  int N, H, W, C;
  size_t off;
  size_t goff;
  bool need_grad;
  bool external;
  size_t mask_off = 0;
  int grad_alias = -1;
};

struct Value {
  int t = -1;
  int bn = -1;
};

struct ParamInfo {
// ... 52 lines not shown

enum OpKind { OP_STEM_COL, OP_CONV, OP_BN_FIN, OP_BN_ACT, OP_MAXPOOL,
              OP_UP2,
              OP_GN,
              OP_MERGE,
              OP_UPLOGITS,
              OP_PARITY,
              OP_DW,
              OP_GAP,
              OP_BCAST,
              OP_DROPE,
              OP_UPB,
              OP_BINPOOL,
              OP_RESIZE,
              OP_RELU,
              OP_DROP2D,
              OP_MOSAIC,
              OP_STATS,
              OP_SEGATE,
              OP_DWG,
              OP_BNX,
              OP_SEFC,
              OP_PAB,
              OP_FPA,
              OP_ADD };
struct Op {
  OpKind kind;
  int conv = -1;
  int bn = -1;
  Value y, res;
  int post = -1;
  bool relu = true;
  int in = -1, out = -1;
  int lane = 0;
  int gn = -1, up = 1;
  int ins[4] = {-1, -1, -1, -1};
  int dwp = -1, oc0 = 0, wc0 = 0;
  bool dw_first = true;
  size_t aux_off = 0;
  bool conv_bn = false;
};

}

struct octseg_plan {
  std::string arch, encoder;
  int classes, B, H, W, dtype;
  std::vector<octseg::TensorInfo> tensors;
  std::vector<octseg::ParamInfo> params;
  std::vector<octseg::BNInfo> bns;
  std::vector<octseg::ConvLayer> convs;
  std::vector<octseg::GNInfo> gns;
  std::vector<octseg::Op> ops;
  int head_up = 1;
  size_t z4_off = 0, dz4_off = 0;
  const float* stem_image = nullptr; int stem_normalize = 0; float stem_mean[3] = {0, 0, 0}, stem_std[3] = {1, 1, 1};
  const float* dropout_keep = nullptr;
  float dropout_p = 0.2f;
  size_t param_numel = 0, buffer_numel = 0;
  size_t ws_bytes = 0;
  size_t act_begin = 0, act_end = 0, grad_begin = 0, grad_end = 0;
  size_t slab_off = 0, slab_bytes = 0;
  bool has_lanes = false;
  size_t fin_part_off = 0, fin_cnt_off = 0;
  size_t pool_idx_off = 0;
  size_t tmp_off = 0, tmp_bytes = 0;
  size_t se_part_off = 0;
  int stem_pad = 3;
  const float* drop_connect = nullptr;
  std::vector<float> dc_rates;
  std::string run_error;
  struct { int w[6], b[6], bn[6]; int pool = -1; size_t scratch_off = 0, gscratch_off = 0; } fpa;
  size_t dlogits_off = 0;
  bool frozen_bn = false;
  int loss_kind = 0;
  size_t dice_off = 0;
  int col_tensor = -1;
  int stem_k = 7;
  int dlogits_C = 16;
  double fwd_macs = 0;
  double exec_macs[3] = {0, 0, 0};
  size_t tie_scratch_off = 0;
  bool packed_valid = false;
  bool packed_fold = false;
  const void* packed_buffers = nullptr;
  const void* packed_ws = nullptr;
  const void* packed_params = nullptr;
  std::vector<octseg::PackJob> pack_jobs;
  std::vector<unsigned long long> pack_prefix;
  unsigned long long pack_total = 0;
  size_t pack_tab_off = 0, pack_prefix_off = 0;
  const void* pack_tab_ws = nullptr;
  std::vector<octseg::BnEvalJob> bn_jobs;
  std::vector<unsigned> bn_prefix;
  unsigned bn_total = 0;
  size_t bn_tab_off = 0, bn_prefix_off = 0;
  hipStream_t side = nullptr;
  hipStream_t side_bwd = nullptr;
  hipEvent_t ev_fork = nullptr, ev_join = nullptr, ev_slice = nullptr;
  bool graph_enabled = false;
  int graph_seen = 0;
  hipGraphExec_t graph_exec = nullptr;
  struct GraphKey {
    const void* params; const void* buffers; const void* ws; const void* image; const void* logits; const void* stream;
    int normalize; float mean[3], stdv[3];
    bool operator==(const GraphKey& o) const {
      return params == o.params && buffers == o.buffers && ws == o.ws && image == o.image && logits == o.logits &&
             stream == o.stream && normalize == o.normalize && mean[0] == o.mean[0] && mean[1] == o.mean[1] &&
             mean[2] == o.mean[2] && stdv[0] == o.stdv[0] && stdv[1] == o.stdv[1] && stdv[2] == o.stdv[2];
    }
  } graph_key{};
  bool tgraph_enabled = false;
  int tgraph_seen = 0;
  hipGraphExec_t tgraph_exec = nullptr;
  struct TrainKey {
    const void *params, *grads, *buffers, *ws, *image, *target, *logits, *loss, *stats, *stream, *dropout, *drop_connect;
    int normalize; float mean[3], stdv[3], grad_scale;
    bool operator==(const TrainKey& o) const {
      return params == o.params && grads == o.grads && buffers == o.buffers && ws == o.ws && image == o.image && target == o.target &&
             logits == o.logits && loss == o.loss && stats == o.stats && stream == o.stream && dropout == o.dropout && drop_connect == o.drop_connect &&
             normalize == o.normalize && grad_scale == o.grad_scale && mean[0] == o.mean[0] && mean[1] == o.mean[1] &&
             mean[2] == o.mean[2] && stdv[0] == o.stdv[0] && stdv[1] == o.stdv[1] && stdv[2] == o.stdv[2];
    }
  } tgraph_key{};
};
```

oct_segmentation_amd/csrc/plan_backward.cpp:

```cpp
#include "plan_internal.h"

namespace octseg {
namespace detail {

int side_wgs() { return 144; }

static int bn_backward(Exec& E, int bn, const void* g, int mask, const void* out_mask, void* res_grad = nullptr, int res_store = 0,
                       const unsigned char* maskbits = nullptr) {
  octseg_plan* P = E.P;
  const BNInfo& b = P->bns[bn];
  const TensorInfo& t = P->tensors[b.y];
  BnBwdArgs a;
  memset(&a, 0, sizeof(a));
  a.g = g; a.y = E.act(b.y); a.out = out_mask; a.maskbits = maskbits;
  a.scale = E.bn_scale(bn); a.shift = E.bn_shift(bn); a.mean = E.bn_mean(bn); a.rstd = E.bn_rstd(bn);
  a.gamma = E.params + P->params[b.gamma].off;
  a.npix = (size_t)t.N * t.H * t.W; a.C = b.C; a.mask = mask;
  a.slab = (float*)(E.ws + P->slab_off);
  a.part = (double*)(E.ws + P->fin_part_off); a.counters = (unsigned*)(E.ws + P->fin_cnt_off);
  const int VEC = ev_vec(P->dtype);
  const int vpc = b.C / VEC;
  const int tpv = vpc >= 256 ? 1 : 256 / vpc;
  size_t rows = (a.npix + tpv - 1) / tpv;
  if (rows > 1024) rows = 1024;
// ... 230 lines not shown
    if (up_src >= 0) {
      const TensorInfo& t = P->tensors[L.srcs[up_src].v.t];
      const int ti = L.srcs[up_src].v.t;
      const int acc = E.claim(ti);
      HIPCHK(launch_pool2x2_accum(P->dtype, E.grad(ti), E.ws + P->tmp_off, t.N, t.H, t.W, t.C, acc ? 0 : 1, E.st));
    }
    return OCTSEG_OK;
  };
  if (!E.data_only) { const int rc = wgrad_part(); if (rc) return rc; }
  return dgrad_part();
}

DiceArgs dice_args(const octseg_plan* P, char* ws, const float* logits, const float* target) {
  DiceArgs a;
  memset(&a, 0, sizeof(a));
  a.logits = logits; a.target = target; a.B = P->B; a.C = P->classes; a.HW = (size_t)P->H * P->W;
  a.sums = (double*)(ws + P->dice_off); a.loss_kind = P->loss_kind;
  return a;
}

static void slice_plan(const octseg_plan* P, SliceCtx& S) {
  const int n = S.n;
  S.bounds.assign(n + 1, 0);
  S.bounds[n] = P->param_numel;
  for (int k = 1; k < n; ++k) {
    const size_t want = P->param_numel * (size_t)k / n;
    size_t b = P->param_numel;
    for (auto& q : P->params) if (q.off >= want && q.off < b) b = q.off;
    S.bounds[k] = b;
  }
  for (int k = 1; k <= n; ++k) S.bounds[k] = std::max(S.bounds[k], S.bounds[k - 1]);
  S.last_op.assign(n, -1);
  auto touch = [&](int oi, int param) {
    if (param < 0) return;
    const size_t off = P->params[param].off;
    for (int k = 0; k < n; ++k)
      if (off >= S.bounds[k] && off < S.bounds[k + 1]) { if (S.last_op[k] < 0 || oi < S.last_op[k]) S.last_op[k] = oi; }
  };
  for (int oi = 0; oi < (int)P->ops.size(); ++oi) {
    const Op& op = P->ops[oi];
    if (op.kind == OP_CONV) { touch(oi, P->convs[op.conv].w); touch(oi, P->convs[op.conv].b); }
    else if (op.kind == OP_BN_FIN) { if (P->bns[op.bn].lazy) { touch(oi, P->bns[op.bn].gamma); touch(oi, P->bns[op.bn].beta); } }
    else if (op.kind == OP_GN) { touch(oi, P->gns[op.gn].gamma); touch(oi, P->gns[op.gn].beta); }
    else if (op.kind == OP_DW || op.kind == OP_DWG) touch(oi, op.dwp);
    else if (op.kind == OP_BNX) { touch(oi, P->bns[op.y.bn].gamma); touch(oi, P->bns[op.y.bn].beta); }
    else if (op.kind == OP_SEFC) { for (int i = 0; i < 4; ++i) touch(oi, op.ins[i]); }
    else if (op.kind == OP_FPA) {
      for (int l = 0; l < 6; ++l) { touch(oi, P->fpa.w[l]); touch(oi, P->fpa.b[l]); touch(oi, P->bns[P->fpa.bn[l]].gamma); touch(oi, P->bns[P->fpa.bn[l]].beta); }
    }
    else if (op.kind == OP_BN_ACT) {
      touch(oi, P->bns[op.y.bn].gamma); touch(oi, P->bns[op.y.bn].beta);
      if (op.res.t >= 0 && op.res.bn >= 0) { touch(oi, P->bns[op.res.bn].gamma); touch(oi, P->bns[op.res.bn].beta); }
    }
  }
}

int run_backward(Exec& E, const float* logits, const float* target, float grad_scale, SliceCtx* S) {
  octseg_plan* P = E.P;
  if (S) slice_plan(P, *S);
  auto fire = [&](int k) -> int {
    if (S->bounds[k + 1] == S->bounds[k]) return OCTSEG_OK;
    if (!P->ev_slice) HIPCHK(hipEventCreateWithFlags(&P->ev_slice, hipEventDisableTiming));
    HIPCHK(hipEventRecord(P->ev_slice, E.st));
    HIPCHK(hipStreamWaitEvent(S->comm, P->ev_slice, 0));
    if (E.wst && E.wst != E.st) {
      HIPCHK(hipEventRecord(P->ev_slice, E.wst));
      HIPCHK(hipStreamWaitEvent(S->comm, P->ev_slice, 0));
    }
    S->cb(S->user, k, S->bounds[k], S->bounds[k + 1]);
    return OCTSEG_OK;
  };
  if (E.data_only) {
    if (S || !P->frozen_bn) return fail(OCTSEG_BAD_ARG, "a data-only backward needs the plan in frozen-BatchNorm mode and takes no slices");
    for (int oi = (int)P->ops.size() - 1; oi > E.stop_op; --oi) {
      const OpKind k = P->ops[oi].kind;
      if (k == OP_GN || k == OP_DW || k == OP_DWG || k == OP_BNX || k == OP_FPA || k == OP_MERGE || k == OP_DROPE || k == OP_DROP2D)
        return fail(OCTSEG_UNSUPPORTED_ARCH, "a data-only backward of this graph is not built (" + P->arch + ")");
    }
  } else {
    HIPCHK(hipMemsetAsync(E.grads, 0, P->param_numel * sizeof(float), E.st));
  }
  HIPCHK(hipMemsetAsync(E.ws + P->fin_cnt_off, 0, 2 * 64 * sizeof(unsigned), E.st));
  E.ginit.assign(P->tensors.size(), 0);
  if (!serial_mode() && !E.data_only) {
    hipStream_t* wsp = P->tgraph_enabled ? &P->side : &P->side_bwd;
    if (!*wsp) HIPCHK(create_side_stream(wsp, !P->tgraph_enabled));
    if (!P->ev_fork) {
      HIPCHK(hipEventCreateWithFlags(&P->ev_fork, hipEventDisableTiming));
      HIPCHK(hipEventCreateWithFlags(&P->ev_join, hipEventDisableTiming));
    }
    E.wst = *wsp;
    HIPCHK(hipEventRecord(P->ev_fork, E.st));
    HIPCHK(hipStreamWaitEvent(E.wst, P->ev_fork, 0));
  }
  if (E.seed) {
    HIPCHK(launch_cam_seed(P->dtype, E.seed, E.ws + P->dlogits_off, P->B, P->classes, (size_t)P->H * P->W, P->dlogits_C, E.st));
  } else {
    const DiceArgs da = dice_args(P, E.ws, logits, target);
    HIPCHK(launch_dice_bwd(P->dtype, da, grad_scale, E.ws + P->dlogits_off, P->dlogits_C, E.st));
  }
  int rc;
  for (int oi = (int)P->ops.size() - 1; oi >= 0; --oi) {
    if (oi == E.stop_op) break;
    const Op& op = P->ops[oi];
    switch (op.kind) {
      case OP_STEM_COL: break;
      case OP_CONV: {
        const ConvLayer& L = P->convs[op.conv];
        if (L.head) rc = conv_backward(E, L, E.ws + (P->head_up > 1 ? P->dz4_off : P->dlogits_off), P->dlogits_C);
        else if (L.sliced) rc = conv_backward(E, L, (char*)E.grad(L.out) + (size_t)L.out_c0 * dtype_size(P->dtype), P->tensors[L.out].C);
        else rc = conv_backward(E, L, E.grad(L.out), L.Cout);
        if (rc) return rc;
        break;
      }
      case OP_BN_FIN: {
        const BNInfo& b = P->bns[op.bn];
        if (b.lazy) {
          rc = bn_backward(E, op.bn, E.grad(b.y), 1, nullptr);
          if (rc) return rc;
        }
        break;
      }
      case OP_BN_ACT: {
        const TensorInfo& t = P->tensors[op.out];
        const void* G = E.grad(op.out);
        const size_t n = (size_t)t.N * t.H * t.W * t.C;
        const int mask = !op.relu ? 0 : (op.post >= 0 ? 1 : 2);
        const bool fuse_res = mask == 2 && op.res.t >= 0 && op.res.bn < 0 && P->tensors[op.res.t].need_grad &&
                              E.grad(op.res.t) != G && E.grad(op.res.t) != E.grad(P->bns[op.y.bn].y);
        const unsigned char* mbits = (mask == 2 && t.mask_off) ? (const unsigned char*)(E.ws + t.mask_off) : nullptr;
        if (fuse_res) {
          const int acc = E.claim(op.res.t);
          rc = bn_backward(E, op.y.bn, G, mask, E.act(op.out), E.grad(op.res.t), acc ? 0 : 1, mbits);
        } else {
          rc = bn_backward(E, op.y.bn, G, mask, E.act(op.out), nullptr, 0, mbits);
        }
        if (rc) return rc;
        if (op.res.t >= 0 && !fuse_res) {
          if (op.res.bn >= 0) {
            rc = bn_backward(E, op.res.bn, G, op.relu ? 2 : 0, E.act(op.out), nullptr, 0, (op.relu && t.mask_off) ? (const unsigned char*)(E.ws + t.mask_off) : nullptr);
            if (rc) return rc;
          } else if (P->tensors[op.res.t].need_grad) {
            const int acc = E.claim(op.res.t);
            HIPCHK(launch_masked_accum(P->dtype, E.grad(op.res.t), G, op.relu ? E.act(op.out) : nullptr, n, acc ? 0 : 1, E.st));
          }
        }
        if (op.post >= 0 && P->tensors[op.post].need_grad) {
          const int acc = E.claim(op.post);
          HIPCHK(launch_masked_accum(P->dtype, E.grad(op.post), G, nullptr, n, acc ? 0 : 1, E.st));
        }
        break;
      }
      case OP_DROP2D: {
        const TensorInfo& t = P->tensors[op.out];
        HIPCHK(launch_drop_bwd(P->dtype, E.grad(op.out), P->dropout_keep, 1.0f / (1.0f - P->dropout_p), E.grad(op.in), t.N, (size_t)t.H * t.W, t.C, E.st));
        E.ginit[op.in] = 1;
        break;
      }
      case OP_RELU: {
        const TensorInfo& t = P->tensors[op.out];
        HIPCHK(launch_relu(P->dtype, E.grad(op.out), E.act(op.out), E.grad(op.in), (size_t)t.N * t.H * t.W * t.C, E.st));
        E.ginit[op.in] = 1;
        break;
      }
      case OP_RESIZE: {
        const TensorInfo& ti = P->tensors[op.in];
// ... 255 lines not shown
```

oct_segmentation_amd/csrc/plan_build.cpp:

```cpp
#include "plan_internal.h"

#include <map>

namespace octseg {
namespace detail {

namespace {

struct Builder {
  octseg_plan* P;
  size_t esz;

  int tensor(int N, int H, int W, int C, bool need_grad = true, bool external = false) {
    TensorInfo t{N, H, W, C, 0, 0, need_grad, external};
    P->tensors.push_back(t);
    return (int)P->tensors.size() - 1;
  }
  int param(const std::string& name, int kind, int R, int S, int O, int I, int KP) {
    ParamInfo p;
    p.name = name; p.kind = kind; p.R = R; p.S = S; p.O = O; p.I = I; p.KP = KP;
    p.numel = kind == OCTSEG_P_VEC ? (size_t)O : kind == OCTSEG_P_STEM ? (size_t)O * KP : (size_t)R * S * O * I;
    p.off = P->param_numel;
    P->param_numel += (p.numel + 3) / 4 * 4;
    P->params.push_back(p);
// ... 778 lines not shown
      const int t = b.tensor(tx.N, tx.H, tx.W, tx.C);
      b.dw(X, t, 0, wp, 0, rates[i]);
      cat.push_back({b.conv(pre + ".0.1", {{mat(t), 0}}, 256, 1, 1, 0, pre + ".1", false), 0});
    }
    {
      const std::string pre = A + ".convs.4";
      const int g = b.gap(X);
      const Value v = b.conv(pre + ".1", {{mat(g), 0}}, 256, 1, 1, 0, pre + ".2", false);
      cat.push_back({mat(b.bcast(b.bn_act(v, Value(), -1, true), tx.H, tx.W)), 0});
    }
    const Value pr = b.conv(A + ".project.0", cat, 256, 1, 1, 0, A + ".project.1", false);
    const int pd = b.drope(b.bn_act(pr, Value(), -1, true));
    const int wp1 = b.dw_param("decoder.aspp.1.0", 256);
    const int t1 = b.tensor(tx.N, tx.H, tx.W, 256);
    b.dw(pd, t1, 0, wp1, 0, 1);
    const Value a2 = b.conv("decoder.aspp.1.1", {{mat(t1), 0}}, 256, 1, 1, 0, "decoder.aspp.2", false);
    const int au = b.upb(b.bn_act(a2, Value(), -1, true), 4);
    const Value h1 = b.conv("decoder.block1.0", {{mat(f[1]), 0}}, 48, 1, 1, 0, "decoder.block1.1", false);
    const int hm = b.bn_act(h1, Value(), -1, true);
    const int wp2 = b.dw_param("decoder.block2.0.0", 256 + 48);
    const TensorInfo tu = P->tensors[au];
    const int t2 = b.tensor(tu.N, tu.H, tu.W, 256 + 48);
    b.dw(au, t2, 0, wp2, 0, 1);
    b.dw(hm, t2, 256, wp2, 256, 1);
    x = b.conv("decoder.block2.0.1", {{mat(t2), 0}}, 256, 1, 1, 0, "decoder.block2.1", false);
  } else {
    return fail(OCTSEG_UNSUPPORTED_ARCH, "unknown arch '" + P->arch + "' (unet | unetplusplus | linknet | fpn | deeplabv3plus | deeplabv3 | pspnet | manet | pan)");
  }
  b.conv("segmentation_head.0", {{x, 0}}, P->classes, head_k, 1, head_k / 2, "", true, false, true);
  if (P->head_up > 1) { Op op; op.kind = OP_UPLOGITS; P->ops.push_back(op); }

  if (!regnet && !effnet && P->arch != "manet" && P->arch != "pan" && P->arch != "fpn" && P->arch != "deeplabv3plus" && P->arch != "pspnet" && P->arch != "deeplabv3") assign_lanes(P);

  P->dlogits_C = 16;
  const size_t esz = dtype_size(P->dtype);
  size_t off = 0;
  P->act_begin = off;
  for (auto& t : P->tensors) { t.off = off; off += align_up((size_t)t.N * t.H * t.W * t.C * esz); }
  P->act_end = off;
  P->grad_begin = off;
  for (auto& t : P->tensors)
    if (t.need_grad && t.grad_alias < 0) { t.goff = off; off += align_up((size_t)t.N * t.H * t.W * t.C * esz); }
  for (auto& t : P->tensors)
    if (t.need_grad && t.grad_alias >= 0) t.goff = P->tensors[t.grad_alias].goff;
  P->grad_end = off;
  for (auto& op : P->ops)
    if (op.kind == OP_BN_ACT && op.relu && op.post < 0) {
      TensorInfo& t = P->tensors[op.out];
      const size_t nvec = (size_t)t.N * t.H * t.W * t.C * esz / 16;
      t.mask_off = off; off += align_up(nvec);
    }
  for (auto& g : P->gns) {
    const TensorInfo& t = P->tensors[g.y];
    const size_t S = (size_t)gn_num_slabs((size_t)t.H * t.W);
    g.part_off = off; off += align_up((size_t)t.N * S * g.C * 2 * sizeof(float));
    g.ss_off = off; off += align_up((size_t)t.N * g.C * 2 * sizeof(float));
    g.stat_off = off; off += align_up((size_t)t.N * g.G * 2 * sizeof(float));
    g.coef_off = off; off += align_up((size_t)t.N * g.G * 2 * sizeof(float));
  }
  if (P->head_up > 1) {
    const size_t h4 = P->H / P->head_up, w4 = P->W / P->head_up;
    P->z4_off = off; off += align_up((size_t)P->B * P->classes * h4 * w4 * sizeof(float));
    P->dz4_off = off; off += align_up((size_t)P->B * h4 * w4 * 16 * esz);
  }
  for (auto& bn : P->bns) { bn.ss_off = off; off += align_up((size_t)bn.C * 6 * sizeof(float)); }
  size_t slab = 0, tmp = 0, tie_scratch = 0;
  for (auto& L : P->convs) {
    Geom g{L.R, L.S, L.stride, L.pad, L.transposed, L.N, L.IH, L.IW, L.Cin, L.OH, L.OW, L.Cout};
    if (L.stem) { g.R = g.S = 1; g.pad = 0; }
    const int wtaps = g.R * g.S;
    std::vector<ConvArgs> la;
    fwd_launches(g, la);
    L.pk_fwd = conv_pack_info(la[0], P->dtype);
    L.wimg_fwd_off = off; off += align_up(conv_image_bytes(L.pk_fwd, wtaps));
    L.has_dgrad = false;
    for (auto& s : L.srcs) L.has_dgrad = L.has_dgrad || P->tensors[s.v.t].need_grad;
    if (L.has_dgrad) {
      std::vector<ConvArgs> ld;
      dgrad_launches(g, ld);
      ConvArgs d0 = ld[0];
      for (auto& d : ld) if (d.ntaps > 0) { d0 = d; break; }
      d0.Cin = L.head ? P->dlogits_C : L.Cout;
      L.pk_dgrad = conv_pack_info(d0, P->dtype);
      L.wimg_dgrad_off = off; off += align_up(conv_image_bytes(L.pk_dgrad, wtaps));
    }
    L.tie = 0;
    if (tie_mask() != 0 && !L.srcs.empty()) {
      TieQuery q{};
      q.esz = (int)esz; q.transposed = L.transposed; q.stem = L.stem; q.head = L.head; q.sliced = L.sliced; q.accum_out = L.accum_out;
      q.has_bn = L.bn >= 0; q.has_bias = L.b >= 0; q.R = L.R; q.S = L.S; q.stride = L.stride; q.pad = L.pad; q.nsrc = (int)L.srcs.size();
      q.up0_whole_grad = L.srcs[0].up && L.srcs[0].cn == 0 && P->tensors[L.srcs[0].v.t].need_grad;
      q.skips_plain_grad = true;
      for (size_t i = 1; i < L.srcs.size(); ++i)
        q.skips_plain_grad = q.skips_plain_grad && !L.srcs[i].up && L.srcs[i].cn == 0 && P->tensors[L.srcs[i].v.t].need_grad;
      q.Ca = P->tensors[L.srcs[0].v.t].C; q.Cs = L.Cin - q.Ca; q.Cout = L.Cout;
      if (tie_eligible(q)) {
        const int Ca = q.Ca, Cs = q.Cs;
        L.tie = tie_mask(); L.tie_Ca = Ca; L.tie_Cs = Cs;
        const TieImages im = tie_images(P->dtype, tie_geom_up(L), tie_geom_skip(L));
        L.tie_pk_fu = im.pk_fu; L.tie_pk_du = im.pk_du; L.tie_du_masked = im.du_masked;
        L.tie_fu_off = off; off += align_up(conv_image_bytes(L.tie_pk_fu, 16));
        L.tie_du_off = off; off += align_up(conv_image_bytes(L.tie_pk_du, im.du_taps()));
        if (Cs > 0) {
          L.tie_pk_fs = im.pk_fs; L.tie_pk_ds = im.pk_ds;
          L.tie_fs_off = off; off += align_up(conv_image_bytes(L.tie_pk_fs, 9));
          L.tie_ds_off = off; off += align_up(conv_image_bytes(L.tie_pk_ds, 9));
        }
        tie_scratch = std::max(tie_scratch, ((size_t)16 * Ca + (size_t)9 * Cs) * L.Cout * sizeof(float));
      }
    }
    if ((L.tie & 1) && L.bn >= 0) {
      P->bns[L.bn].rows = 512;
      slab = std::max(slab, (size_t)512 * L.Cout * 2 * sizeof(float));
    } else if (L.bn >= 0 && L.stem && (P->stem_k == 7 && thin_stem_eligible(P->dtype))) {
      P->bns[L.bn].rows = thin_stem_rows(L.N, P->H, P->W);
      slab = std::max(slab, (size_t)P->bns[L.bn].rows * L.Cout * 2 * sizeof(float));
    } else if (L.bn >= 0) {
      int rows = 0;
      for (auto& a : la) {
        a.nsrc = 0;
        int c0 = 0;
        for (auto& s : L.srcs) {
          SrcDesc d{}; d.H = P->tensors[s.v.t].H; d.W = P->tensors[s.v.t].W; d.up = s.up; d.C = P->tensors[s.v.t].C; d.c0 = c0;
          c0 += s.cn ? s.cn : d.C; a.src[a.nsrc++] = d;
        }
        DstDesc dd{}; dd.H = L.OH; dd.W = L.OW; dd.C = L.Cout; dd.cn = L.Cout; a.dst[0] = dd; a.ndst = 1;
        a.bias = L.b >= 0 ? (const float*)(uintptr_t)16 : nullptr;
        a.stat_slab = (float*)(uintptr_t)16;
        a.Wmaster = (const float*)(uintptr_t)16; a.wO = L.Cout; a.wI = L.Cin; a.wtrans = 0;
        a.out_mode = L.head ? OUT_HEAD_NCHW : OUT_STORE;
        rows += conv_num_mtiles_flat(a, P->dtype);
      }
      P->bns[L.bn].rows = rows;
      slab = std::max(slab, (size_t)rows * L.Cout * 2 * sizeof(float));
    }
    for (auto& s : L.srcs)
      if (s.up) tmp = std::max(tmp, (size_t)L.N * L.IH * L.IW * P->tensors[s.v.t].C * esz);
  }
  for (auto& bn : P->bns)
    if (bn.rows == 0) bn.rows = 512;
  P->pack_jobs.clear(); P->pack_prefix.clear(); P->pack_total = 0;
  for (auto& L : P->convs) {
    const int taps = L.stem ? 1 : L.R * L.S;
    for (int tr = 0; tr < 2; ++tr) {
      if (tr == 1 && !L.has_dgrad) continue;
      const ConvPackInfo& pk = tr ? L.pk_dgrad : L.pk_fwd;
      PackJob j{P->params[L.w].off, tr ? L.wimg_dgrad_off : L.wimg_fwd_off, taps, L.Cout, L.Cin, tr, pk.BN, pk.RB, pk.nchunks, pk.ntiles,
                (!tr && L.bn >= 0) ? P->bns[L.bn].ss_off : (!tr && L.fold_bn >= 0) ? P->bns[L.fold_bn].ss_off + (size_t)L.out_c0 * sizeof(float) : ~(size_t)0};
      P->pack_prefix.push_back(P->pack_total);
      P->pack_jobs.push_back(j);
      P->pack_total += (unsigned long long)taps * pk.nchunks * pk.ntiles * pk.BN * (pk.RB / 16);
    }
    if (L.tie)
      tie_pack_jobs(TieImages{L.tie_pk_fu, L.tie_pk_du, L.tie_pk_fs, L.tie_pk_ds, L.tie_du_masked},
                    TieOffsets{L.tie_fu_off, L.tie_du_off, L.tie_fs_off, L.tie_ds_off}, P->params[L.w].off, L.Cout, L.Cin, L.tie_Ca, L.tie_Cs,
                    P->pack_jobs, P->pack_prefix, P->pack_total);
  }
  P->bn_jobs.clear(); P->bn_prefix.clear(); P->bn_total = 0;
  for (auto& b : P->bns) {
    P->bn_prefix.push_back(P->bn_total);
    P->bn_jobs.push_back(BnEvalJob{P->params[b.gamma].off, P->params[b.beta].off, b.rm_off, b.rv_off, b.ss_off, b.C, ~(size_t)0, b.eps});
    P->bn_total += (unsigned)b.C;
  }
  for (auto& L : P->convs)
    if (L.bn >= 0 && L.b >= 0) P->bn_jobs[L.bn].bias_off = P->params[L.b].off;
  P->bn_tab_off = off; off += align_up(P->bn_jobs.size() * sizeof(BnEvalJob));
  P->bn_prefix_off = off; off += align_up(P->bn_prefix.size() * sizeof(unsigned));
  P->pack_tab_off = off; off += align_up(P->pack_jobs.size() * sizeof(PackJob));
  P->pack_prefix_off = off; off += align_up(P->pack_prefix.size() * sizeof(unsigned long long));
  for (auto& bn : P->bns) slab = std::max(slab, (size_t)1024 * bn.C * 2 * sizeof(float));
  P->slab_off = off; P->slab_bytes = align_up(slab); off += 2 * align_up(slab);
  P->fin_part_off = off; off += 2 * align_up((size_t)SLAB_PART_CAP * 2 * sizeof(double));
  P->fin_cnt_off = off; off += align_up(2 * 64 * sizeof(unsigned));
  {
    size_t pool_elems = 0;
    for (auto& op : P->ops)
      if (op.kind == OP_MAXPOOL) { const TensorInfo& t = P->tensors[op.out]; pool_elems = std::max(pool_elems, (size_t)t.N * t.H * t.W * t.C); }
    P->pool_idx_off = off; off += align_up(pool_elems);
  }
  P->tmp_off = off; P->tmp_bytes = tmp; off += align_up(tmp);
  P->tie_scratch_off = off; off += align_up(tie_scratch);
  for (int k = 0; k < 3; ++k) {
    P->exec_macs[k] = P->fwd_macs;
    for (auto& L : P->convs)
      if (L.tie & (1 << k)) P->exec_macs[k] -= layer_macs(L) * L.tie_Ca / L.Cin * (5.0 / 9.0);
  }
  {
    size_t se_part = 0;
    for (auto& op : P->ops)
      if (op.kind == OP_SEGATE) { const TensorInfo& t = P->tensors[op.in]; se_part = std::max(se_part, (size_t)t.N * se_dgate_shares(t.H * t.W) * t.C * sizeof(float)); }
    P->se_part_off = off; off += align_up(se_part);
    for (auto& op : P->ops)
      if (op.kind == OP_SEFC) { const TensorInfo& t = P->tensors[op.in]; op.aux_off = off; off += align_up((size_t)2 * t.N * op.up * sizeof(float)); }
      else if (op.kind == OP_FPA) {
        const TensorInfo& t = P->tensors[op.in];
        P->fpa.scratch_off = off; off += align_up(fpa_pyr_scratch_floats(t.N, t.H, t.W) * sizeof(float));
        P->fpa.gscratch_off = off; off += align_up((fpa_pyr_gscratch_floats(t.N, t.H, t.W) + (size_t)t.N * t.H * t.W) * sizeof(float));
      }
      else if (op.kind == OP_PAB) {
        const TensorInfo& t = P->tensors[op.in];
        const size_t hw = (size_t)t.H * t.W;
        op.aux_off = off; off += align_up((size_t)t.N * hw * hw * sizeof(float)) * 2 + align_up((size_t)t.N * hw * t.C * sizeof(float));
      }
  }
  P->dlogits_off = off; off += align_up((size_t)P->B * P->H * P->W * P->dlogits_C * esz);
  P->dice_off = off; off += align_up((size_t)(1 + P->B) * P->classes * DICE_NS * sizeof(double));
  P->ws_bytes = off;
  return OCTSEG_OK;
}

}
}
```

oct_segmentation_amd/csrc/plan_forward.cpp:

```cpp
#include "plan_internal.h"

namespace octseg {
namespace detail {

thread_local std::string g_err;
int fail(int code, const std::string& msg) { g_err = msg; return code; }

bool g_prof_on = false;
bool g_capturing = false;
bool g_prof_hbm = false;
std::vector<ProfRec> g_prof;
std::vector<hipEvent_t> g_prof_pool;
hipEvent_t prof_event() {
  if (!g_prof_pool.empty()) { hipEvent_t e = g_prof_pool.back(); g_prof_pool.pop_back(); return e; }
  hipEvent_t e;
  if (hipEventCreate(&e) != hipSuccess) return nullptr;
  return e;
}

hipError_t create_side_stream(hipStream_t* st, bool backward) {
  if (backward) {
    int least = 0, greatest = 0;
    hipError_t e = hipDeviceGetStreamPriorityRange(&least, &greatest);
    if (e != hipSuccess) return e;
    return hipStreamCreateWithPriority(st, hipStreamNonBlocking, least);
  }
  return hipStreamCreateWithFlags(st, hipStreamNonBlocking);
}

int pack_all_weights(Exec& E, bool fold) {
  octseg_plan* P = E.P;
  if (P->packed_valid && P->packed_fold == fold && P->packed_ws == (const void*)E.ws && P->packed_params == (const void*)E.params &&
      (!fold || P->packed_buffers == (const void*)E.buffers))
    return OCTSEG_OK;
  if (P->pack_tab_ws != (const void*)E.ws) {
    HIPCHK(hipMemcpyAsync(E.ws + P->pack_tab_off, P->pack_jobs.data(), P->pack_jobs.size() * sizeof(PackJob), hipMemcpyHostToDevice, E.st));
    HIPCHK(hipMemcpyAsync(E.ws + P->pack_prefix_off, P->pack_prefix.data(), P->pack_prefix.size() * sizeof(unsigned long long),
                          hipMemcpyHostToDevice, E.st));
    if (!P->bn_jobs.empty()) {
      HIPCHK(hipMemcpyAsync(E.ws + P->bn_tab_off, P->bn_jobs.data(), P->bn_jobs.size() * sizeof(BnEvalJob), hipMemcpyHostToDevice, E.st));
      HIPCHK(hipMemcpyAsync(E.ws + P->bn_prefix_off, P->bn_prefix.data(), P->bn_prefix.size() * sizeof(unsigned), hipMemcpyHostToDevice, E.st));
    }
    P->pack_tab_ws = E.ws;
  }
  if (fold && !P->bn_jobs.empty())
    HIPCHK(launch_bn_finalize_eval_all(E.params, E.buffers, E.ws, (const BnEvalJob*)(E.ws + P->bn_tab_off),
                                       (const unsigned*)(E.ws + P->bn_prefix_off), (int)P->bn_jobs.size(), P->bn_total, 1e-5f, E.st));
  HIPCHK(launch_pack_all(P->dtype, E.params, E.ws, (const PackJob*)(E.ws + P->pack_tab_off),
                         (const unsigned long long*)(E.ws + P->pack_prefix_off), (int)P->pack_jobs.size(), P->pack_total, fold ? 1 : 0, E.st));
  P->packed_valid = true; P->packed_fold = fold; P->packed_ws = E.ws; P->packed_params = E.params; P->packed_buffers = E.buffers;
  return OCTSEG_OK;
}

static const void* fwd_weight(const Exec& E, const ConvLayer& L) { return E.ws + L.wimg_fwd_off; }

static int tied_forward(Exec& E, const ConvLayer& L, hipStream_t st, float* slab) {
  octseg_plan* P = E.P;
  SrcDesc src[MAX_SRC];
  const int ns = E.fill_srcs(L, src);
  DstDesc d;
  d.ptr = E.act(L.out); d.C = L.Cout; d.c0 = 0; d.cn = L.Cout; d.H = L.OH; d.W = L.OW; d.accum = 0; d.pool = 0;
  const double macs = layer_macs(L);
  if (L.tie_Cs > 0) {
    std::vector<ConvArgs> v;
    fwd_launches(tie_geom_skip(L), v);
    ConvArgs& a = v[0];
    a.nsrc = ns - 1;
    for (int i = 1; i < ns; ++i) { a.src[i - 1] = src[i]; a.src[i - 1].c0 -= L.tie_Ca; }
    a.W = E.ws + L.tie_fs_off;
    a.dst[0] = d; a.ndst = 1; a.out_mode = OUT_STORE;
    ProfScope ps(0, 2.0 * macs * L.tie_Cs / L.Cin, st, L.name);
    HIPCHK(launch_conv(P->dtype, a, st));
  }
  std::vector<ConvArgs> v;
  fwd_launches(tie_geom_up(L), v);
  for (auto& a : v) {
    a.nsrc = 1; a.src[0] = src[0]; a.src[0].up = 0; a.src[0].c0 = 0;
    a.W = E.ws + L.tie_fu_off;
    d.accum = L.tie_Cs > 0 ? 1 : 0;
    a.dst[0] = d; a.ndst = 1; a.out_mode = OUT_STORE;
    ProfScope ps(0, 2.0 * macs * L.tie_Ca / L.Cin / 4.0, st, L.name);
    HIPCHK(launch_conv(P->dtype, a, st));
  }
  const BNInfo& b = P->bns[L.bn];
  HIPCHK(launch_tensor_stats(P->dtype, E.act(L.out), (size_t)L.N * L.OH * L.OW, b.C, slab, b.rows, st));
  return OCTSEG_OK;
}

int run_forward(Exec& E, const float* image, float* logits, int normalize, const float* mean, const float* stdv) {
  octseg_plan* P = E.P;
  if (!P->run_error.empty()) return fail(OCTSEG_BAD_SHAPE, P->run_error);
  const bool frozen = E.train && P->frozen_bn;
  if (E.train && !frozen)
    for (auto& b : P->bns)
      if (b.count <= 1.0) {
        const TensorInfo& t = P->tensors[b.y];
        char buf[192];
        snprintf(buf, sizeof buf, "Expected more than 1 value per channel when training, got input size torch.Size([%d, %d, %d, %d])",
                 t.N, t.C, t.H, t.W);
        return fail(OCTSEG_BAD_SHAPE, buf);
      }
  int rc = pack_all_weights(E, !E.train);
  if (rc) return rc;
  if (E.train) HIPCHK(hipMemsetAsync(E.ws + P->fin_cnt_off, 0, 2 * 64 * sizeof(unsigned), E.st));
  const bool folded = !E.train;
  const bool lanes = P->has_lanes && !serial_mode();
  hipStream_t lst[2] = {E.st, E.st};
  if (lanes) {
    const bool low = E.train && !P->tgraph_enabled;
    hipStream_t* lsp = low ? &P->side_bwd : &P->side;
    if (!*lsp) HIPCHK(create_side_stream(lsp, low));
    if (!P->ev_fork) {
      HIPCHK(hipEventCreateWithFlags(&P->ev_fork, hipEventDisableTiming));
      HIPCHK(hipEventCreateWithFlags(&P->ev_join, hipEventDisableTiming));
    }
    lst[1] = *lsp;
  }
  std::vector<int> tseq(P->tensors.size(), 0), bseq(P->bns.size(), 0);
  int enq[2] = {1, 0}, seen[2] = {0, 0};
  auto need = [&](int lane, int stamp) -> int {
    if (!lanes) return OCTSEG_OK;
    const int pl = stamp >> 24, ps = stamp & 0xffffff;
    if (pl == lane || ps <= seen[lane]) return OCTSEG_OK;
    hipEvent_t ev = lane == 1 ? P->ev_fork : P->ev_join;
    HIPCHK(hipEventRecord(ev, lst[pl]));
    HIPCHK(hipStreamWaitEvent(lst[lane], ev, 0));
    seen[lane] = enq[pl];
    return OCTSEG_OK;
  };
  auto need_val = [&](int lane, const Value& v) -> int {
    int rc2 = OCTSEG_OK;
    if (v.t >= 0) rc2 = need(lane, tseq[v.t]);
// ... 342 lines not shown
```

oct_segmentation_amd/csrc/plan_geom.cpp:

```cpp
#include "plan_internal.h"

namespace octseg {
namespace detail {

static void set_taps(int* tdy, int* tdx, int* tw, int n, int& ntaps, int& min_dy,
                     int& min_dx, int& span_y, int& span_x) {
  ntaps = n;
  if (n == 0) { min_dy = min_dx = 0; span_y = span_x = 1; return; }
  int mny = 127, mnx = 127, mxy = -127, mxx = -127;
  for (int i = 0; i < n; ++i) {
    mny = std::min(mny, (int)tdy[i]); mxy = std::max(mxy, (int)tdy[i]);
    mnx = std::min(mnx, (int)tdx[i]); mxx = std::max(mxx, (int)tdx[i]);
  }
  (void)tw;
  min_dy = mny; min_dx = mnx; span_y = mxy - mny + 1; span_x = mxx - mnx + 1;
}

void fwd_launches(const Geom& g, std::vector<ConvArgs>& out) {
  if (!g.transposed) {
    ConvArgs a;
    memset(&a, 0, sizeof(a));
    int n = 0;
    for (int r = 0; r < g.R; ++r)
      for (int s = 0; s < g.S; ++s) { a.tap_dy[n] = r - g.pad; a.tap_dx[n] = s - g.pad; a.tap_w[n] = r * g.S + s; ++n; }
// ... 82 lines not shown
        WgradArgs a;
        memset(&a, 0, sizeof(a));
        int n = 0;
        for (int r = 0; r < g.R; ++r) {
          if (((py + g.pad - r) & 1) != 0) continue;
          for (int s = 0; s < g.S; ++s) {
            if (((px + g.pad - s) & 1) != 0) continue;
            a.tap_dy[n] = (py + g.pad - r) / 2; a.tap_dx[n] = (px + g.pad - s) / 2; a.tap_w[n] = r * g.S + s; ++n;
          }
        }
        set_taps(a.tap_dy, a.tap_dx, a.tap_w, n, a.ntaps, a.min_dy, a.min_dx, a.span_y, a.span_x);
        a.istride = 1; a.N = g.N; a.IH = g.IH; a.IW = g.IW; a.OH = g.IH; a.OW = g.IW;
        a.Cin = g.Cin; a.Cout = g.Cout; a.DH = g.OH; a.DW = g.OW; a.dstride = 2; a.doy = py; a.dox = px;
        out.push_back(a);
      }
  }
}

void tied_dgrad_masked(const Geom& g, ConvArgs& a) {
  memset(&a, 0, sizeof(a));
  int n = 0;
  for (int t = 0; t < 9; ++t) { a.tap_dy[n] = t / 3 - 1; a.tap_dx[n] = t % 3 - 1; a.tap_w[n] = t; ++n; }
  set_taps(a.tap_dy, a.tap_dx, a.tap_w, n, a.ntaps, a.min_dy, a.min_dx, a.span_y, a.span_x);
  a.istride = 1; a.N = g.N; a.IH = g.IH; a.IW = g.IW; a.OH = g.IH; a.OW = g.IW;
  a.Cin = 4 * g.Cout; a.Cout = g.Cin; a.ostride = 1;
  a.taps_per_src = 4; a.nsrc = 4;
  for (int p = 0; p < 4; ++p) {
    const int py = p >> 1, px = p & 1;
    int list = 0, k = 0;
    for (int t = 0; t < 9; ++t) {
      const int r = py + 1 + 2 * (t / 3 - 1), s = px + 1 + 2 * (t % 3 - 1);
      if (r >= 0 && r <= 3 && s >= 0 && s <= 3) list |= t << (4 * k++);
    }
    a.src_taps[p] = list;
    SrcDesc d{};
    d.C = 2 * g.Cout; d.c0 = p * g.Cout; d.H = g.IH; d.W = 2 * g.IW;
    a.src[p] = d;
  }
}

int tie_mask() {
  const char* e = getenv("OCTSEG_TIED");
  if (e == nullptr) return 2 | 4;
  int v = 0;
  for (const char* c = e; *c; ++c) v |= *c == 'f' ? 1 : *c == 'd' ? 2 : *c == 'w' ? 4 : 0;
  return v;
}

Geom tie_geom_up(const ConvLayer& L) { return Geom{4, 4, 2, 1, true, L.N, L.IH / 2, L.IW / 2, L.tie_Ca, L.OH, L.OW, L.Cout}; }
Geom tie_geom_skip(const ConvLayer& L) { return Geom{3, 3, 1, 1, false, L.N, L.IH, L.IW, L.tie_Cs, L.OH, L.OW, L.Cout}; }

bool tie_eligible(const TieQuery& q) {
  if (!(q.esz == 2 && !q.transposed && !q.stem && !q.head && !q.sliced && !q.accum_out && q.R == 3 && q.S == 3 && q.stride == 1 && q.pad == 1 &&
        q.has_bn && !q.has_bias && q.nsrc >= 1 && q.up0_whole_grad))
    return false;
  if (!q.skips_plain_grad) return false;
  return q.Ca >= 64 && q.Ca % 8 == 0 && q.Cs % 8 == 0 && q.Cout >= 32 && (q.Cs == 0 || q.Cs >= 32);
}

TieImages tie_images(int dtype, const Geom& gu, const Geom& gs) {
  TieImages im{};
  std::vector<ConvArgs> v;
  fwd_launches(gu, v);
  im.pk_fu = conv_pack_info(v[0], dtype);
  v.clear();
  im.du_masked = false;
  if (gu.Cout % 64 == 0) {
    ConvArgs am;
    tied_dgrad_masked(gu, am);
    DstDesc dd{}; dd.H = gu.IH; dd.W = gu.IW; dd.C = gu.Cin; dd.cn = gu.Cin; am.dst[0] = dd; am.ndst = 1;
    if (conv_masked_eligible(am, dtype)) { im.du_masked = true; v.push_back(am); }
  }
  if (!im.du_masked) dgrad_launches(gu, v);
  im.pk_du = conv_pack_info(v[0], dtype);
  if (gs.Cin > 0) {
    v.clear(); fwd_launches(gs, v);
    im.pk_fs = conv_pack_info(v[0], dtype);
    v.clear(); dgrad_launches(gs, v);
    im.pk_ds = conv_pack_info(v[0], dtype);
  }
  return im;
}

void tie_pack_jobs(const TieImages& im, const TieOffsets& at, size_t w_off, int Cout, int Cin, int Ca, int Cs, std::vector<PackJob>& jobs,
                   std::vector<unsigned long long>& prefix, unsigned long long& total) {
  auto add = [&](size_t dst, int ntaps, int I, int c0, int tr, int tied, const ConvPackInfo& pk) {
    PackJob j{w_off, dst, ntaps, Cout, I, tr, pk.BN, pk.RB, pk.nchunks, pk.ntiles, ~(size_t)0, Cin, c0, tied};
    prefix.push_back(total);
    jobs.push_back(j);
    total += (unsigned long long)ntaps * pk.nchunks * pk.ntiles * pk.BN * (pk.RB / 16);
  };
  add(at.fu, 16, Ca, 0, 0, 1, im.pk_fu);
  add(at.du, im.du_taps(), Ca, 0, 1, im.du_masked ? 2 : 1, im.pk_du);
  if (Cs > 0) {
    add(at.fs, 9, Cs, Ca, 0, 0, im.pk_fs);
    add(at.ds, 9, Cs, Ca, 1, 0, im.pk_ds);
  }
}

double layer_macs(const ConvLayer& L) {
  return (double)L.N * L.OH * L.OW * L.Cout * (L.stem ? 3.0 * L.stem_k * L.stem_k : (double)L.Cin * (L.transposed ? 4.0 : (double)L.R * L.S));
}

bool geom_ok(int dtype, int Cin, int Cout, int R, int S, int stride, int transposed) {
  const int v = ev_vec(dtype);
  (void)Cout;
  if (Cin % v != 0) return false;
  if (R != S || R < 1 || R > 7) return false;
  if (stride != 1 && stride != 2) return false;
  if (transposed && !(R == 4 && stride == 2)) return false;
  return true;
}
Geom op_geom(int N, int H, int W, int Cin, int Cout, int R, int S, int stride, int pad, int transposed) {
  Geom g{R, S, stride, pad, transposed != 0, N, H, W, Cin, 0, 0, Cout};
  if (transposed) { g.OH = H * 2; g.OW = W * 2; } else { g.OH = (H + 2 * pad - R) / stride + 1; g.OW = (W + 2 * pad - S) / stride + 1; }
  return g;
}

}
}
```

oct_segmentation_amd/csrc/plan_internal.h:

```cpp
#pragma once
#include "plan.h"
#include "ev.h"

#include <algorithm>
#include <cstdint>
#include <cstdio>
#include <cstdlib>
#include <cstring>
#include <string>
#include <vector>

namespace octseg {
namespace detail __attribute__((visibility("hidden"))) {

extern thread_local std::string g_err;
int fail(int code, const std::string& msg);
#define HIPCHK(expr)                                                                      \
  do {                                                                                    \
    hipError_t _e = (expr);                                                               \
    if (_e != hipSuccess)                                                                 \
      return fail(OCTSEG_HIP_ERROR, std::string(#expr) + ": " + hipGetErrorString(_e));   \
  } while (0)

inline size_t align_up(size_t x, size_t a = 256) { return (x + a - 1) / a * a; }

struct ProfRec { hipEvent_t a, b; int kind; double flops; std::string name; };
extern bool g_prof_on;
extern bool g_capturing;
extern bool g_prof_hbm;
extern std::vector<ProfRec> g_prof;
extern std::vector<hipEvent_t> g_prof_pool;
hipEvent_t prof_event();
struct ProfScope {
  hipStream_t st; ProfRec r; bool on;
  ProfScope(int kind, double flops, hipStream_t s, const std::string& name = std::string()) : st(s), on(g_prof_on && !g_capturing) {
    if (kind == 3 && !g_prof_hbm) on = false;
    if (!on) return;
    r.kind = kind; r.flops = flops; r.name = name; r.a = prof_event(); r.b = prof_event();
    if (!r.a || !r.b) { on = false; return; }
    (void)hipEventRecord(r.a, st);
  }
  ~ProfScope() {
    if (!on) return;
    (void)hipEventRecord(r.b, st);
    g_prof.push_back(r);
  }
};

struct Geom {
  int R, S, stride, pad;
  bool transposed;
  int N, IH, IW, Cin, OH, OW, Cout;
};
void fwd_launches(const Geom& g, std::vector<ConvArgs>& out);
void dgrad_launches(const Geom& g, std::vector<ConvArgs>& out);
void wgrad_launches(const Geom& g, std::vector<WgradArgs>& out);
void tied_dgrad_masked(const Geom& g, ConvArgs& a);
int tie_mask();
Geom tie_geom_up(const ConvLayer& L);
Geom tie_geom_skip(const ConvLayer& L);
struct TieQuery {
  int esz;
  bool transposed, stem, head, sliced, accum_out, has_bn, has_bias;
  int R, S, stride, pad, nsrc;
  bool up0_whole_grad;
  bool skips_plain_grad;
  int Ca, Cs, Cout;
};
bool tie_eligible(const TieQuery& q);
struct TieImages {
  ConvPackInfo pk_fu, pk_du, pk_fs, pk_ds;
  bool du_masked;
  int du_taps() const { return du_masked ? 9 : 16; }
};
TieImages tie_images(int dtype, const Geom& up, const Geom& skip);
struct TieOffsets { size_t fu, du, fs, ds; };
void tie_pack_jobs(const TieImages& im, const TieOffsets& at, size_t w_off, int Cout, int Cin, int Ca, int Cs, std::vector<PackJob>& jobs,
                   std::vector<unsigned long long>& prefix, unsigned long long& total);
int side_wgs();
double layer_macs(const ConvLayer& L);
bool geom_ok(int dtype, int Cin, int Cout, int R, int S, int stride, int transposed);
Geom op_geom(int N, int H, int W, int Cin, int Cout, int R, int S, int stride, int pad, int transposed);

bool serial_mode();
hipError_t create_side_stream(hipStream_t* st, bool backward = false);

struct Exec {
  octseg_plan* P;
  const float* params;
  float* grads;
  float* buffers;
  char* ws;
  hipStream_t st;
  int train;
  hipStream_t wst = nullptr;
  const float* seed = nullptr;
  bool data_only = false;
  int stop_op = -1;
  std::vector<char> ginit;
  int claim(int t) { const int acc = ginit[t] ? 1 : 0; ginit[t] = 1; return acc; }

  void* act(int t) const { return ws + P->tensors[t].off; }
  void* grad(int t) const { return ws + P->tensors[t].goff; }
  float* ss(int bn) const { return (float*)(ws + P->bns[bn].ss_off); }
  float* bn_scale(int bn) const { return ss(bn); }
  float* bn_shift(int bn) const { return ss(bn) + P->bns[bn].C; }
  float* bn_mean(int bn) const { return ss(bn) + 2 * P->bns[bn].C; }
  float* bn_rstd(int bn) const { return ss(bn) + 3 * P->bns[bn].C; }
  float* bn_coef(int bn) const { return ss(bn) + 4 * P->bns[bn].C; }

  GnArgs gn_args(int gi) const {
    const GNInfo& g = P->gns[gi];
    const TensorInfo& t = P->tensors[g.y];
    GnArgs a;
    memset(&a, 0, sizeof(a));
    a.y = act(g.y);
    a.gamma = params + P->params[g.gamma].off; a.beta = params + P->params[g.beta].off;
    if (grads) { a.dgamma = grads + P->params[g.gamma].off; a.dbeta = grads + P->params[g.beta].off; }
    a.part = (float*)(ws + g.part_off); a.ss = (float*)(ws + g.ss_off); a.stat = (float*)(ws + g.stat_off); a.coef = (float*)(ws + g.coef_off);
    a.HW = (size_t)t.H * t.W; a.C = g.C; a.G = g.G; a.cpg = g.C / g.G; a.eps = 1e-5f;
    return a;
  }
  Geom geom(const ConvLayer& L) const {
    Geom g{L.R, L.S, L.stride, L.pad, L.transposed, L.N, L.IH, L.IW, L.Cin, L.OH, L.OW, L.Cout};
    if (L.stem) { g.R = g.S = 1; g.pad = 0; }
    return g;
  }
  int fill_srcs(const ConvLayer& L, SrcDesc* src) const {
    int c0 = 0, n = 0;
    for (auto& s : L.srcs) {
      const TensorInfo& t = P->tensors[s.v.t];
      SrcDesc d;
      d.ptr = (char*)act(s.v.t) + (size_t)s.c0 * dtype_size(P->dtype);
      d.scale = s.v.bn >= 0 ? bn_scale(s.v.bn) + s.c0 : nullptr;
      d.shift = s.v.bn >= 0 ? bn_shift(s.v.bn) + s.c0 : nullptr;
      d.C = t.C; d.c0 = c0; d.H = t.H; d.W = t.W; d.up = s.up; d.relu = s.v.bn >= 0 ? 1 : 0;
      src[n++] = d;
      c0 += s.cn ? s.cn : t.C;
    }
    return n;
  }
};

struct SliceCtx {
  int n = 0;
  hipStream_t comm = nullptr;
  octseg_slice_cb cb = nullptr;
  void* user = nullptr;
  std::vector<size_t> bounds;
  std::vector<int> last_op;
};

int build_plan(octseg_plan* P);
int pack_all_weights(Exec& E, bool fold);
int run_forward(Exec& E, const float* image, float* logits, int normalize, const float* mean, const float* stdv);
DiceArgs dice_args(const octseg_plan* P, char* ws, const float* logits, const float* target);
int run_backward(Exec& E, const float* logits, const float* target, float grad_scale, SliceCtx* S = nullptr);
int cam_target_op(const octseg_plan* P);

}
// ... 2 lines not shown
```

Baseline: 259.4 frames/s.

## Split weight packing into forward and gradient groups, overlap gradient packing on side stream

Weight-image packing jobs are tagged by group (forward, forward-tied, gradient) and sorted, so forward images can be packed on the main stream while dgrad/transposed images are packed on a side stream joined later by an event. The pack kernel is rewritten to process one block per tile, with vectorised float4 loads and a shared-memory transpose for transposed images, replacing the per-element binary search. Validity is tracked separately for forward and gradient images. It adds event/stream synchronisation complexity and some debug API surface.

```diff
diff --git a/include/octseg.h b/include/octseg.h
--- a/include/octseg.h
+++ b/include/octseg.h
@@ -68,6 +68,15 @@
 int octseg_profile_stop(double* out);
 
 int octseg_plan_params_changed(octseg_plan* plan);
+int octseg_plan_pack_info(const octseg_plan* plan, int group, int* jobs, size_t* bytes);
+typedef struct {
+  size_t param_offset, bytes;
+  int taps, O, I, transpose, BN, RB, nchunks, ntiles, src_I, src_c0;
+  int tied;
+  int group;
+  int eval;
+} octseg_pack_job_info;
+int octseg_plan_pack_job(const octseg_plan* plan, int index, octseg_pack_job_info* out);
 
 int octseg_plan_set_dropout(octseg_plan* plan, const float* keep_dev);
 
@@ -274,6 +283,8 @@
 int octseg_tied_layer_route(int pass, int dtype, const octseg_conv_layer_desc* desc, int wg_target, int* route_per_launch, int* nlaunch);
 size_t octseg_tied_layer_scratch_bytes(int dtype, const octseg_conv_layer_desc* desc);
 int octseg_side_wgs(void);
+int octseg_debug_pack_jobs(int dtype, const float* w, octseg_pack_job_info* jobs, int njobs, const float* oscale, int single, void* scratch,
+                           size_t scratch_bytes, size_t* image_off, void* stream);
 
 typedef enum { OCTSEG_STEM_IM2COL = 0, OCTSEG_STEM_FORWARD = 1, OCTSEG_STEM_WGRAD = 2 } octseg_stem_stage;
 typedef struct {
diff --git a/oct_segmentation_amd/_lib.py b/oct_segmentation_amd/_lib.py
--- a/oct_segmentation_amd/_lib.py
+++ b/oct_segmentation_amd/_lib.py
@@ -30,6 +30,11 @@
 
 class BNInfo(C.Structure):
     _fields_ = [('name', C.c_char * 128), ('C', C.c_int), ('mean_offset', C.c_size_t), ('var_offset', C.c_size_t)]
+
+
+class PackJobInfo(C.Structure):
+    _fields_ = ([('param_offset', C.c_size_t), ('bytes', C.c_size_t)] +
+                [(k, C.c_int) for k in ('taps', 'O', 'I', 'transpose', 'BN', 'RB', 'nchunks', 'ntiles', 'src_I', 'src_c0', 'tied', 'group', 'eval')])
 
 
 class ConvSrc(C.Structure):
@@ -104,6 +109,8 @@
     'octseg_profile_start': (C.c_int, []),
     'octseg_profile_stop': (C.c_int, [C.POINTER(C.c_double)]),
     'octseg_plan_params_changed': (C.c_int, [_P]),
+    'octseg_plan_pack_info': (C.c_int, [_P, C.c_int, C.POINTER(C.c_int), C.POINTER(C.c_size_t)]),
+    'octseg_plan_pack_job': (C.c_int, [_P, C.c_int, C.POINTER(PackJobInfo)]),
     'octseg_plan_set_dropout': (C.c_int, [_P, _P]),
     'octseg_plan_set_drop_connect': (C.c_int, [_P, _P]),
     'octseg_plan_num_drop_connect': (C.c_int, [_P]),
@@ -182,6 +189,7 @@
     'octseg_tied_layer_op': (C.c_int, [C.c_int, C.c_int, C.POINTER(ConvLayerDesc), C.c_int, _P]),
     'octseg_tied_layer_route': (C.c_int, [C.c_int, C.c_int, C.POINTER(ConvLayerDesc), C.c_int, C.POINTER(C.c_int), C.POINTER(C.c_int)]),
     'octseg_tied_layer_scratch_bytes': (C.c_size_t, [C.c_int, C.POINTER(ConvLayerDesc)]),
+    'octseg_debug_pack_jobs': (C.c_int, [C.c_int, _P, C.POINTER(PackJobInfo), C.c_int, _P, C.c_int, _P, C.c_size_t, C.POINTER(C.c_size_t), _P]),
     'octseg_side_wgs': (C.c_int, []),
     'octseg_stem_op': (C.c_int, [C.c_int, C.c_int, C.POINTER(StemDesc), _P]),
     'octseg_stem_slab_rows': (C.c_int, [C.c_int] * 3),
diff --git a/oct_segmentation_amd/csrc/api.cpp b/oct_segmentation_amd/csrc/api.cpp
--- a/oct_segmentation_amd/csrc/api.cpp
+++ b/oct_segmentation_amd/csrc/api.cpp
@@ -18,17 +18,19 @@
     seen = 0;
   }
   if (const int rc = outside()) return rc;
-  auto replay = [&]() -> int { HIPCHK(hipGraphLaunch(exec, st)); if (train) p->packed_valid = false; return OCTSEG_OK; };
+  auto replay = [&]() -> int { HIPCHK(hipGraphLaunch(exec, st)); if (train) p->packed_valid = p->packed_grad_valid = false; return OCTSEG_OK; };
   if (exec) return replay();
   if (seen++ == 0) return body();
-  if (train) p->packed_valid = false;
+  if (train) p->packed_valid = p->packed_grad_valid = false;
   hipGraph_t g = nullptr;
   HIPCHK(hipStreamBeginCapture(st, hipStreamCaptureModeThreadLocal));
   g_capturing = train;
   const int rc = body();
   g_capturing = false;
   const hipError_t ce = hipStreamEndCapture(st, &g);
-  if (train) p->packed_valid = false;
+  if (train) {
+    p->packed_valid = p->packed_grad_valid = false; p->pack_pending = false;
+  }
   hipError_t ie = hipSuccess;
   if (!rc && ce == hipSuccess && (ie = hipGraphInstantiate(&exec, g, nullptr, nullptr, 0)) != hipSuccess) exec = nullptr;
   if (g) (void)hipGraphDestroy(g);
@@ -68,8 +70,10 @@
 }
 int octseg_plan_destroy(octseg_plan* p) {
   if (p) {
-    if (p->side) (void)hipStreamDestroy(p->side);
-    if (p->side_bwd) (void)hipStreamDestroy(p->side_bwd);
+    if (p->side) { (void)hipStreamSynchronize(p->side); (void)hipStreamDestroy(p->side); }
+    if (p->side_bwd) { (void)hipStreamSynchronize(p->side_bwd); (void)hipStreamDestroy(p->side_bwd); }
+    if (p->ev_pack_fork) (void)hipEventDestroy(p->ev_pack_fork);
+    if (p->ev_pack) (void)hipEventDestroy(p->ev_pack);
     if (p->ev_fork) (void)hipEventDestroy(p->ev_fork);
     if (p->ev_join) (void)hipEventDestroy(p->ev_join);
     if (p->ev_slice) (void)hipEventDestroy(p->ev_slice);
@@ -150,7 +154,27 @@
 
 int octseg_plan_params_changed(octseg_plan* p) {
   if (!p) return fail(OCTSEG_BAD_ARG, "null argument");
-  p->packed_valid = false;
+  p->packed_valid = p->packed_grad_valid = false;
+  return OCTSEG_OK;
+}
+
+int octseg_plan_pack_info(const octseg_plan* p, int group, int* jobs, size_t* bytes) {
+  if (!p || group < 0 || group > 3) return fail(OCTSEG_BAD_ARG, "pack_info: null plan, or group not 0 forward, 1 gradient, 2 eval, 3 all");
+  const int* nj = p->pack_group_jobs; const size_t* nb = p->pack_group_bytes;
+  const int j = group == 0 ? nj[PACK_FWD] + nj[PACK_FWD_TIED] : group == 1 ? nj[PACK_GRAD] : group == 2 ? nj[PACK_FWD] : nj[0] + nj[1] + nj[2];
+  const size_t b = group == 0 ? nb[PACK_FWD] + nb[PACK_FWD_TIED] : group == 1 ? nb[PACK_GRAD] : group == 2 ? nb[PACK_FWD] : nb[0] + nb[1] + nb[2];
+  if (jobs) *jobs = j;
+  if (bytes) *bytes = b;
+  return OCTSEG_OK;
+}
+int octseg_plan_pack_job(const octseg_plan* p, int i, octseg_pack_job_info* o) {
+  if (!p || !o || i < 0 || i >= (int)p->pack_jobs.size()) return fail(OCTSEG_BAD_ARG, "pack job index out of range");
+  const PackJob& j = p->pack_jobs[i];
+  memset(o, 0, sizeof(*o));
+  o->param_offset = j.src_off; o->bytes = pack_job_bytes(j);
+  o->taps = j.taps; o->O = j.O; o->I = j.I; o->transpose = j.transpose; o->BN = j.BN; o->RB = j.RB; o->nchunks = j.nchunks; o->ntiles = j.ntiles;
+  o->src_I = j.src_I ? j.src_I : j.I; o->src_c0 = j.src_c0; o->tied = j.tied;
+  o->group = j.group == PACK_GRAD ? 1 : 0; o->eval = j.group == PACK_FWD ? 1 : 0;
   return OCTSEG_OK;
 }
 
diff --git a/oct_segmentation_amd/csrc/conv_api.cpp b/oct_segmentation_amd/csrc/conv_api.cpp
--- a/oct_segmentation_amd/csrc/conv_api.cpp
+++ b/oct_segmentation_amd/csrc/conv_api.cpp
@@ -264,7 +264,7 @@
   }
   B.dk4_off = off; off += align_up(((size_t)16 * B.Ca + (size_t)9 * B.Cs) * d->Cout * sizeof(float));
   B.bytes = off;
-  tie_pack_jobs(B.im, B.at, 0, d->Cout, d->Cin, B.Ca, B.Cs, B.jobs, B.prefix, B.total);
+  tie_pack_jobs(B.im, B.at, 1 | 2, 0, d->Cout, d->Cin, B.Ca, B.Cs, B.jobs, B.prefix, B.total);
   return OCTSEG_OK;
 }
 
@@ -427,7 +427,7 @@
   HIPCHK(hipMemcpyAsync(ws, B.jobs.data(), B.jobs.size() * sizeof(PackJob), hipMemcpyHostToDevice, st));
   HIPCHK(hipMemcpyAsync(ws + TIE_TAB_BYTES, B.prefix.data(), B.prefix.size() * sizeof(unsigned long long), hipMemcpyHostToDevice, st));
   HIPCHK(hipStreamSynchronize(st));
-  HIPCHK(launch_pack_all(dtype, d->w, ws, (const PackJob*)ws, (const unsigned long long*)(ws + TIE_TAB_BYTES), (int)B.jobs.size(), B.total, 0, st));
+  HIPCHK(launch_pack_all(dtype, d->w, ws, (const PackJob*)ws, (const unsigned long long*)(ws + TIE_TAB_BYTES), (int)B.jobs.size(), 0, B.total, 0, st));
   for (auto& a : B.conv) HIPCHK(launch_conv(dtype, a, st));
   return OCTSEG_OK;
 }
@@ -461,4 +461,54 @@
 
 int octseg_side_wgs(void) { return side_wgs(); }
 
-}
+int octseg_debug_pack_jobs(int dtype, const float* w, octseg_pack_job_info* jobs, int njobs, const float* oscale, int single, void* scratch,
+                           size_t scratch_bytes, size_t* image_off, void* stream) {
+  const std::string who = "debug_pack_jobs: ";
+  if (dtype != OCTSEG_F32 && dtype != OCTSEG_BF16 && dtype != OCTSEG_F16) return fail(OCTSEG_BAD_DTYPE, who + "dtype must be f32, bf16 or f16");
+  if (!w || !jobs || !image_off || njobs < 1 || njobs > 64) return fail(OCTSEG_BAD_ARG, who + "null argument, or not 1..64 jobs");
+  const int esz = (int)dtype_size(dtype);
+  std::vector<PackJob> tab; std::vector<unsigned long long> prefix; unsigned long long total = 0;
+  int maxO = 0;
+  for (int k = 0; k < njobs; ++k) maxO = std::max(maxO, jobs[k].O);
+  size_t off = align_up(njobs * sizeof(PackJob));
+  const size_t prefix_off = off; off += align_up(njobs * sizeof(unsigned long long));
+  const size_t scale_off = off; off += align_up((size_t)std::max(maxO, 1) * sizeof(float));
+  for (int k = 0; k < njobs; ++k) {
+    octseg_pack_job_info& q = jobs[k];
+    if (q.taps < 1 || q.O < 1 || q.I < 1 || q.BN < 32 || q.BN > 256 || q.BN % 32 != 0 || (q.RB != 64 && q.RB != 128) || q.tied < 0 || q.tied > 2 ||
+        q.src_c0 < 0 || q.src_I < q.src_c0 + q.I)
+      return fail(OCTSEG_BAD_SHAPE, who + "job outside what the packers stage");
+    if ((q.tied == 1 && q.taps != 16) || (q.tied == 2 && !(q.taps == 9 && q.transpose))) return fail(OCTSEG_BAD_SHAPE, who + "tied job with the wrong tap count");
+    if (single && (q.tied || q.src_I != q.I || q.src_c0)) return fail(OCTSEG_BAD_ARG, who + "launch_pack_weight_image packs plain whole-weight images only");
+    const int KC = q.RB / esz, rows = q.transpose ? q.I : q.O, K = q.transpose ? (q.tied == 2 ? 4 * q.O : q.O) : q.I;
+    q.nchunks = (K + KC - 1) / KC; q.ntiles = (rows + q.BN - 1) / q.BN;
+    PackJob j{q.param_offset, off, q.taps, q.O, q.I, q.transpose ? 1 : 0, q.BN, q.RB, q.nchunks, q.ntiles,
+              (q.eval && oscale && !q.transpose) ? scale_off : ~(size_t)0, q.src_I == q.I ? 0 : q.src_I, q.src_c0, q.tied, q.transpose ? PACK_GRAD : PACK_FWD};
+    q.bytes = pack_job_bytes(j);
+    image_off[k] = off; off += align_up(q.bytes);
+    prefix.push_back(total); tab.push_back(j); total += pack_job_blocks(j);
+  }
+  image_off[njobs] = off;
+  if (scratch == nullptr) return OCTSEG_OK;
+  if (!aligned(w) || !aligned(scratch)) return fail(OCTSEG_BAD_ARG, who + "misaligned pointer");
+  if (scratch_bytes < off) return fail(OCTSEG_BAD_ARG, who + "scratch smaller than image_off[njobs]");
+  hipStream_t st = (hipStream_t)stream;
+  char* ws = (char*)scratch;
+  if (oscale) HIPCHK(hipMemcpyAsync(ws + scale_off, oscale, (size_t)maxO * sizeof(float), hipMemcpyDeviceToDevice, st));
+  if (single) {
+    for (int k = 0; k < njobs; ++k) {
+      const PackJob& j = tab[k];
+      const ConvPackInfo pk{j.BN, j.RB, j.nchunks, j.ntiles};
+      HIPCHK(launch_pack_weight_image(dtype, w + j.src_off, ws + j.dst_off, j.taps, j.O, j.I, j.transpose, pk, st,
+                                      j.scale_off != ~(size_t)0 ? (const float*)(ws + scale_off) : nullptr));
+    }
+    return OCTSEG_OK;
+  }
+  HIPCHK(hipMemcpyAsync(ws, tab.data(), tab.size() * sizeof(PackJob), hipMemcpyHostToDevice, st));
+  HIPCHK(hipMemcpyAsync(ws + prefix_off, prefix.data(), prefix.size() * sizeof(unsigned long long), hipMemcpyHostToDevice, st));
+  HIPCHK(hipStreamSynchronize(st));
+  HIPCHK(launch_pack_all(dtype, w, ws, (const PackJob*)ws, (const unsigned long long*)(ws + prefix_off), njobs, 0, total, 1, st));
+  return OCTSEG_OK;
+}
+
+}
diff --git a/oct_segmentation_amd/csrc/elementwise.hip b/oct_segmentation_amd/csrc/elementwise.hip
--- a/oct_segmentation_amd/csrc/elementwise.hip
+++ b/oct_segmentation_amd/csrc/elementwise.hip
@@ -975,66 +975,118 @@
   return hipGetLastError();
 }
 
+constexpr int PACK_RT = 64, PACK_KC_MAX = 64;
+
+static __device__ __forceinline__ void pack_src4(const float* __restrict__ w, int O, int sI, int c0s, int nI, bool vec_ok, int o, int i0, bool sum,
+                                                 int tap, int r_lo, int r_hi, int s_lo, int s_hi, float* x) {
+  const bool vec = vec_ok && i0 + 3 < nI;
+  auto ld4 = [&](int t, float* y) {
+    const float* src = w + ((size_t)t * O + o) * sI + c0s + i0;
+    if (vec) { const float4 f = *(const float4*)src; y[0] = f.x; y[1] = f.y; y[2] = f.z; y[3] = f.w; }
+    else {
+#pragma unroll
+      for (int j = 0; j < 4; ++j) y[j] = i0 + j < nI ? src[j] : 0.f;
+    }
+  };
+  if (!sum) { ld4(tap, x); return; }
+  x[0] = x[1] = x[2] = x[3] = 0.f;
+  for (int r3 = r_lo; r3 <= r_hi; ++r3)
+    for (int s3 = s_lo; s3 <= s_hi; ++s3) {
+      float y[4];
+      ld4(r3 * 3 + s3, y);
+#pragma unroll
+      for (int j = 0; j < 4; ++j) x[j] += y[j];
+    }
+}
+
 template <typename T>
 __global__ __launch_bounds__(256) void pack_all_kernel(const float* params, char* ws, const PackJob* tab, const unsigned long long* prefix,
-                                                       int njobs, unsigned long long total, int fold) {
+                                                       int njobs, unsigned long long base, int fold) {
   constexpr int VEC = EV<T>::VEC;
-  for (unsigned long long g = (unsigned long long)blockIdx.x * blockDim.x + threadIdx.x; g < total; g += (unsigned long long)gridDim.x * blockDim.x) {
-    int lo = 0, hi = njobs - 1;
-    while (lo < hi) {
-      const int mid = (lo + hi + 1) >> 1;
-      if (prefix[mid] <= g) lo = mid; else hi = mid - 1;
-    }
-    const PackJob jb = tab[lo];
-    if (fold && jb.src_I != 0) continue;
-    const float* w = params + jb.src_off;
-    const int VPR = jb.RB / 16, KC = jb.RB / (int)sizeof(T), swz_div = 256 / jb.RB;
-    const int rows = jb.transpose ? jb.I : jb.O, K = jb.transpose ? jb.O : jb.I, sI = jb.src_I ? jb.src_I : jb.I;
-    size_t rem = (size_t)(g - prefix[lo]);
-    const size_t v = rem;
-    const int q = (int)(rem % VPR); rem /= VPR;
-    const int row = (int)(rem % jb.BN); rem /= jb.BN;
-    const int nt = (int)(rem % jb.ntiles); rem /= jb.ntiles;
-    const int chunk = (int)(rem % jb.nchunks);
-    const int tap = (int)(rem / jb.nchunks);
-    const int lq = q ^ ((row / swz_div) & (VPR - 1));
-    const int co = nt * jb.BN + row, c0 = chunk * KC + lq * VEC;
-    float osc = 1.f;
-    if (fold && !jb.transpose && jb.scale_off != ~(size_t)0 && co < rows) osc = ((const float*)(ws + jb.scale_off))[co];
-    float x[VEC];
-#pragma unroll
-    for (int i = 0; i < VEC; ++i) {
-      const int c = c0 + i;
-      float val = 0.f;
-      if (jb.tied == 2) {
-        if (co < jb.I && c < 4 * jb.O) {
-          const int p = c / jb.O, o = c - p * jb.O;
+  __shared__ float tile[PACK_KC_MAX * (PACK_RT + 1)];
+  const unsigned long long g = base + blockIdx.x;
+  int lo = 0, hi = njobs - 1;
+  while (lo < hi) {
+    const int mid = (lo + hi + 1) >> 1;
+    if (prefix[mid] <= g) lo = mid; else hi = mid - 1;
+  }
+  const PackJob jb = tab[lo];
+  const float* w = params + jb.src_off;
+  const int VPR = jb.RB / 16, KC = jb.RB / (int)sizeof(T), swz_div = 256 / jb.RB;
+  const int O = jb.O, sI = jb.src_I ? jb.src_I : jb.I;
+  const bool vec_ok = (sI & 3) == 0 && (jb.src_c0 & 3) == 0 && (((uintptr_t)w) & 15) == 0;
+  const unsigned blk = (unsigned)(g - prefix[lo]);
+  const int nt = (int)(blk % (unsigned)jb.ntiles), chunk = (int)((blk / (unsigned)jb.ntiles) % (unsigned)jb.nchunks);
+  const int tap = (int)(blk / ((unsigned)jb.ntiles * (unsigned)jb.nchunks));
+  char* img = ws + jb.dst_off;
+  const size_t v0 = (size_t)blk * jb.BN * VPR;
+  if (!jb.transpose) {
+    const int u = tap >> 2, vv = tap & 3;
+    const int r_lo = max(0, 2 - u), r_hi = min(2, 3 - u), s_lo = max(0, 2 - vv), s_hi = min(2, 3 - vv);
+    const float* scale = (fold && jb.scale_off != ~(size_t)0) ? (const float*)(ws + jb.scale_off) : nullptr;
+    for (int v = threadIdx.x; v < jb.BN * VPR; v += 256) {
+      const int q = v % VPR, row = v / VPR;
+      const int lq = q ^ ((row / swz_div) & (VPR - 1));
+      const int co = nt * jb.BN + row, c0 = chunk * KC + lq * VEC;
+      float x[VEC];
+#pragma unroll
+      for (int i = 0; i < VEC; ++i) x[i] = 0.f;
+      if (co < O) {
+#pragma unroll
+        for (int h = 0; h < VEC / 4; ++h)
+          if (c0 + 4 * h < jb.I) pack_src4(w, O, sI, jb.src_c0, jb.I, vec_ok, co, c0 + 4 * h, jb.tied == 1, tap, r_lo, r_hi, s_lo, s_hi, x + 4 * h);
+        if (scale != nullptr) {
+          const float osc = scale[co];
+#pragma unroll
+          for (int i = 0; i < VEC; ++i)
+            if (c0 + i < jb.I) x[i] *= osc;
+        }
+      }
+      stv<T>(img, v0 + v, EV<T>::pack(x));
+    }
+    return;
+  }
+  const int K = jb.tied == 2 ? 4 * O : O;
+  for (int sub = 0; sub < jb.BN; sub += PACK_RT) {
+    for (int e = threadIdx.x; e < KC * (PACK_RT / 4); e += 256) {
+      const int kk = e / (PACK_RT / 4), r4 = (e % (PACK_RT / 4)) * 4;
+      const int c = chunk * KC + kk, co = nt * jb.BN + sub + r4;
+      float x[4] = {0.f, 0.f, 0.f, 0.f};
+      if (c < K && co < jb.I && sub + r4 < jb.BN) {
+        if (jb.tied == 2) {
+          const int p = c / O, o = c - p * O;
           const int u = (p >> 1) + 1 + 2 * (tap / 3 - 1), vv = (p & 1) + 1 + 2 * (tap % 3 - 1);
           if (u >= 0 && u <= 3 && vv >= 0 && vv <= 3)
-            for (int r3 = max(0, 2 - u); r3 <= min(2, 3 - u); ++r3)
-              for (int s3 = max(0, 2 - vv); s3 <= min(2, 3 - vv); ++s3) val += w[((size_t)(r3 * 3 + s3) * jb.O + o) * sI + co + jb.src_c0];
+            pack_src4(w, O, sI, jb.src_c0, jb.I, vec_ok, o, co, true, 0, max(0, 2 - u), min(2, 3 - u), max(0, 2 - vv), min(2, 3 - vv), x);
+        } else {
+          const int u = tap >> 2, vv = tap & 3;
+          pack_src4(w, O, sI, jb.src_c0, jb.I, vec_ok, c, co, jb.tied == 1, tap, max(0, 2 - u), min(2, 3 - u), max(0, 2 - vv), min(2, 3 - vv), x);
         }
-      } else if (co < rows && c < K) {
-        const int o = jb.transpose ? c : co, ci = (jb.transpose ? co : c) + jb.src_c0;
-        if (!jb.tied) val = w[((size_t)tap * jb.O + o) * sI + ci];
-        else {
-          const int u = tap >> 2, vv = tap & 3;
-          for (int r3 = max(0, 2 - u); r3 <= min(2, 3 - u); ++r3)
-            for (int s3 = max(0, 2 - vv); s3 <= min(2, 3 - vv); ++s3) val += w[((size_t)(r3 * 3 + s3) * jb.O + o) * sI + ci];
-        }
-        if (!jb.transpose) val *= osc;
-      }
-      x[i] = val;
-    }
-    stv<T>(ws + jb.dst_off, v, EV<T>::pack(x));
+      }
+#pragma unroll
+      for (int j = 0; j < 4; ++j) tile[kk * (PACK_RT + 1) + r4 + j] = x[j];
+    }
+    __syncthreads();
+    const int nrow = min(PACK_RT, jb.BN - sub);
+    for (int v = threadIdx.x; v < nrow * VPR; v += 256) {
+      const int q = v % VPR, r = v / VPR, row = sub + r;
+      const int lq = q ^ ((row / swz_div) & (VPR - 1));
+      float x[VEC];
+#pragma unroll
+      for (int i = 0; i < VEC; ++i) x[i] = tile[(lq * VEC + i) * (PACK_RT + 1) + r];
+      stv<T>(img, v0 + (size_t)sub * VPR + v, EV<T>::pack(x));
+    }
+    __syncthreads();
   }
 }
 hipError_t launch_pack_all(int dtype, const float* params, void* ws, const PackJob* tab, const unsigned long long* prefix, int njobs,
-                           unsigned long long total, int fold, hipStream_t st) {
-  const int gr = grid_for((size_t)total, 256, 8192);
-  if (dtype == DT_F16) hipLaunchKernelGGL(pack_all_kernel<f16_t>, dim3(gr), dim3(256), 0, st, params, (char*)ws, tab, prefix, njobs, total, fold);
-  else if (dtype == DT_F32) hipLaunchKernelGGL(pack_all_kernel<float>, dim3(gr), dim3(256), 0, st, params, (char*)ws, tab, prefix, njobs, total, fold);
-  else hipLaunchKernelGGL(pack_all_kernel<bf16_t>, dim3(gr), dim3(256), 0, st, params, (char*)ws, tab, prefix, njobs, total, fold);
+                           unsigned long long base, unsigned long long nblocks, int fold, hipStream_t st) {
+  if (nblocks == 0) return hipSuccess;
+  if (nblocks > 0x7fffffffull) return hipErrorInvalidValue;
+  const dim3 gr((unsigned)nblocks);
+  if (dtype == DT_F16) hipLaunchKernelGGL(pack_all_kernel<f16_t>, gr, dim3(256), 0, st, params, (char*)ws, tab, prefix, njobs, base, fold);
+  else if (dtype == DT_F32) hipLaunchKernelGGL(pack_all_kernel<float>, gr, dim3(256), 0, st, params, (char*)ws, tab, prefix, njobs, base, fold);
+  else hipLaunchKernelGGL(pack_all_kernel<bf16_t>, gr, dim3(256), 0, st, params, (char*)ws, tab, prefix, njobs, base, fold);
   return hipGetLastError();
 }
 
diff --git a/oct_segmentation_amd/csrc/kernels.h b/oct_segmentation_amd/csrc/kernels.h
--- a/oct_segmentation_amd/csrc/kernels.h
+++ b/oct_segmentation_amd/csrc/kernels.h
@@ -193,10 +193,14 @@
                  size_t scale_off;
                  int src_I;
                  int src_c0;
-                 int tied;          };
+                 int tied;
+                 int group;         };
+enum { PACK_FWD = 0, PACK_FWD_TIED = 1, PACK_GRAD = 2 };
+static inline unsigned long long pack_job_blocks(const PackJob& j) { return (unsigned long long)j.taps * j.nchunks * j.ntiles; }
+static inline size_t pack_job_bytes(const PackJob& j) { return (size_t)pack_job_blocks(j) * j.BN * j.RB; }
 hipError_t launch_tied_fold(const float* dK4, const float* dW3s, float* dW3, int O, int Ca, int Cs, hipStream_t st);
 hipError_t launch_pack_all(int dtype, const float* params, void* ws, const PackJob* tab, const unsigned long long* prefix, int njobs,
-                           unsigned long long total, int fold, hipStream_t st);
+                           unsigned long long base, unsigned long long nblocks, int fold, hipStream_t st);
 
 struct GnArgs {
   const void* y;
diff --git a/oct_segmentation_amd/csrc/plan.h b/oct_segmentation_amd/csrc/plan.h
--- a/oct_segmentation_amd/csrc/plan.h
+++ b/oct_segmentation_amd/csrc/plan.h
@@ -158,6 +158,7 @@
   double exec_macs[3] = {0, 0, 0};
   size_t tie_scratch_off = 0;
   bool packed_valid = false;
+  bool packed_grad_valid = false;
   bool packed_fold = false;
   const void* packed_buffers = nullptr;
   const void* packed_ws = nullptr;
@@ -165,6 +166,11 @@
   std::vector<octseg::PackJob> pack_jobs;
   std::vector<unsigned long long> pack_prefix;
   unsigned long long pack_total = 0;
+  unsigned long long pack_group_end[3] = {0, 0, 0};
+  int pack_group_jobs[3] = {0, 0, 0};
+  size_t pack_group_bytes[3] = {0, 0, 0};
+  hipEvent_t ev_pack_fork = nullptr, ev_pack = nullptr;
+  bool pack_pending = false;
   size_t pack_tab_off = 0, pack_prefix_off = 0;
   const void* pack_tab_ws = nullptr;
   std::vector<octseg::BnEvalJob> bn_jobs;
diff --git a/oct_segmentation_amd/csrc/plan_backward.cpp b/oct_segmentation_amd/csrc/plan_backward.cpp
--- a/oct_segmentation_amd/csrc/plan_backward.cpp
+++ b/oct_segmentation_amd/csrc/plan_backward.cpp
@@ -336,6 +336,7 @@
   }
   HIPCHK(hipMemsetAsync(E.ws + P->fin_cnt_off, 0, 2 * 64 * sizeof(unsigned), E.st));
   E.ginit.assign(P->tensors.size(), 0);
+  if (P->pack_pending) HIPCHK(hipStreamWaitEvent(E.st, P->ev_pack, 0));
   if (!serial_mode() && !E.data_only) {
     hipStream_t* wsp = P->tgraph_enabled ? &P->side : &P->side_bwd;
     if (!*wsp) HIPCHK(create_side_stream(wsp, !P->tgraph_enabled));
diff --git a/oct_segmentation_amd/csrc/plan_build.cpp b/oct_segmentation_amd/csrc/plan_build.cpp
--- a/oct_segmentation_amd/csrc/plan_build.cpp
+++ b/oct_segmentation_amd/csrc/plan_build.cpp
@@ -884,7 +884,6 @@
       for (auto& d : ld) if (d.ntaps > 0) { d0 = d; break; }
       d0.Cin = L.head ? P->dlogits_C : L.Cout;
       L.pk_dgrad = conv_pack_info(d0, P->dtype);
-      L.wimg_dgrad_off = off; off += align_up(conv_image_bytes(L.pk_dgrad, wtaps));
     }
     L.tie = 0;
     if (tie_mask() != 0 && !L.srcs.empty()) {
@@ -901,16 +900,19 @@
         L.tie = tie_mask(); L.tie_Ca = Ca; L.tie_Cs = Cs;
         const TieImages im = tie_images(P->dtype, tie_geom_up(L), tie_geom_skip(L));
         L.tie_pk_fu = im.pk_fu; L.tie_pk_du = im.pk_du; L.tie_du_masked = im.du_masked;
-        L.tie_fu_off = off; off += align_up(conv_image_bytes(L.tie_pk_fu, 16));
-        L.tie_du_off = off; off += align_up(conv_image_bytes(L.tie_pk_du, im.du_taps()));
-        if (Cs > 0) {
-          L.tie_pk_fs = im.pk_fs; L.tie_pk_ds = im.pk_ds;
-          L.tie_fs_off = off; off += align_up(conv_image_bytes(L.tie_pk_fs, 9));
-          L.tie_ds_off = off; off += align_up(conv_image_bytes(L.tie_pk_ds, 9));
+        if (Cs > 0) { L.tie_pk_fs = im.pk_fs; L.tie_pk_ds = im.pk_ds; }
+        if (L.tie & 1) {
+          L.tie_fu_off = off; off += align_up(conv_image_bytes(L.tie_pk_fu, 16));
+          if (Cs > 0) { L.tie_fs_off = off; off += align_up(conv_image_bytes(L.tie_pk_fs, 9)); }
+        }
+        if (L.tie & 2) {
+          L.tie_du_off = off; off += align_up(conv_image_bytes(L.tie_pk_du, im.du_taps()));
+          if (Cs > 0) { L.tie_ds_off = off; off += align_up(conv_image_bytes(L.tie_pk_ds, 9)); }
         }
         tie_scratch = std::max(tie_scratch, ((size_t)16 * Ca + (size_t)9 * Cs) * L.Cout * sizeof(float));
       }
     }
+    if (L.has_dgrad && !(L.tie & 2)) { L.wimg_dgrad_off = off; off += align_up(conv_image_bytes(L.pk_dgrad, wtaps)); }
     if ((L.tie & 1) && L.bn >= 0) {
       P->bns[L.bn].rows = 512;
       slab = std::max(slab, (size_t)512 * L.Cout * 2 * sizeof(float));
@@ -945,18 +947,27 @@
   for (auto& L : P->convs) {
     const int taps = L.stem ? 1 : L.R * L.S;
     for (int tr = 0; tr < 2; ++tr) {
-      if (tr == 1 && !L.has_dgrad) continue;
+      if (tr == 1 && !(L.has_dgrad && !(L.tie & 2))) continue;
       const ConvPackInfo& pk = tr ? L.pk_dgrad : L.pk_fwd;
       PackJob j{P->params[L.w].off, tr ? L.wimg_dgrad_off : L.wimg_fwd_off, taps, L.Cout, L.Cin, tr, pk.BN, pk.RB, pk.nchunks, pk.ntiles,
-                (!tr && L.bn >= 0) ? P->bns[L.bn].ss_off : (!tr && L.fold_bn >= 0) ? P->bns[L.fold_bn].ss_off + (size_t)L.out_c0 * sizeof(float) : ~(size_t)0};
-      P->pack_prefix.push_back(P->pack_total);
+                (!tr && L.bn >= 0) ? P->bns[L.bn].ss_off : (!tr && L.fold_bn >= 0) ? P->bns[L.fold_bn].ss_off + (size_t)L.out_c0 * sizeof(float) : ~(size_t)0,
+                0, 0, 0, tr ? PACK_GRAD : PACK_FWD};
       P->pack_jobs.push_back(j);
-      P->pack_total += (unsigned long long)taps * pk.nchunks * pk.ntiles * pk.BN * (pk.RB / 16);
-    }
-    if (L.tie)
+    }
+    if (L.tie & 3)
       tie_pack_jobs(TieImages{L.tie_pk_fu, L.tie_pk_du, L.tie_pk_fs, L.tie_pk_ds, L.tie_du_masked},
-                    TieOffsets{L.tie_fu_off, L.tie_du_off, L.tie_fs_off, L.tie_ds_off}, P->params[L.w].off, L.Cout, L.Cin, L.tie_Ca, L.tie_Cs,
+                    TieOffsets{L.tie_fu_off, L.tie_du_off, L.tie_fs_off, L.tie_ds_off}, L.tie, P->params[L.w].off, L.Cout, L.Cin, L.tie_Ca, L.tie_Cs,
                     P->pack_jobs, P->pack_prefix, P->pack_total);
+  }
+  std::stable_sort(P->pack_jobs.begin(), P->pack_jobs.end(), [](const PackJob& a, const PackJob& b) { return a.group < b.group; });
+  P->pack_prefix.clear(); P->pack_total = 0;
+  for (int k = 0; k < 3; ++k) { P->pack_group_end[k] = 0; P->pack_group_jobs[k] = 0; P->pack_group_bytes[k] = 0; }
+  for (auto& j : P->pack_jobs) {
+    if (j.RB > 128 || j.BN % 32 != 0) return fail(OCTSEG_BAD_SHAPE, "internal: a weight image with rows the packer does not stage");
+    P->pack_prefix.push_back(P->pack_total);
+    P->pack_total += pack_job_blocks(j);
+    P->pack_group_jobs[j.group] += 1; P->pack_group_bytes[j.group] += pack_job_bytes(j);
+    for (int k = j.group; k < 3; ++k) P->pack_group_end[k] = P->pack_total;
   }
   P->bn_jobs.clear(); P->bn_prefix.clear(); P->bn_total = 0;
   for (auto& b : P->bns) {
diff --git a/oct_segmentation_amd/csrc/plan_forward.cpp b/oct_segmentation_amd/csrc/plan_forward.cpp
--- a/oct_segmentation_amd/csrc/plan_forward.cpp
+++ b/oct_segmentation_amd/csrc/plan_forward.cpp
@@ -30,9 +30,10 @@
 
 int pack_all_weights(Exec& E, bool fold) {
   octseg_plan* P = E.P;
-  if (P->packed_valid && P->packed_fold == fold && P->packed_ws == (const void*)E.ws && P->packed_params == (const void*)E.params &&
-      (!fold || P->packed_buffers == (const void*)E.buffers))
-    return OCTSEG_OK;
+  if (P->packed_ws != (const void*)E.ws || P->packed_params != (const void*)E.params) P->packed_valid = P->packed_grad_valid = false;
+  const bool fwd_ok = P->packed_valid && P->packed_fold == fold && (!fold || P->packed_buffers == (const void*)E.buffers);
+  const bool grad_ok = fold || P->packed_grad_valid;
+  if (fwd_ok && grad_ok) return OCTSEG_OK;
   if (P->pack_tab_ws != (const void*)E.ws) {
     HIPCHK(hipMemcpyAsync(E.ws + P->pack_tab_off, P->pack_jobs.data(), P->pack_jobs.size() * sizeof(PackJob), hipMemcpyHostToDevice, E.st));
     HIPCHK(hipMemcpyAsync(E.ws + P->pack_prefix_off, P->pack_prefix.data(), P->pack_prefix.size() * sizeof(unsigned long long),
@@ -43,11 +44,35 @@
     }
     P->pack_tab_ws = E.ws;
   }
-  if (fold && !P->bn_jobs.empty())
-    HIPCHK(launch_bn_finalize_eval_all(E.params, E.buffers, E.ws, (const BnEvalJob*)(E.ws + P->bn_tab_off),
-                                       (const unsigned*)(E.ws + P->bn_prefix_off), (int)P->bn_jobs.size(), P->bn_total, 1e-5f, E.st));
-  HIPCHK(launch_pack_all(P->dtype, E.params, E.ws, (const PackJob*)(E.ws + P->pack_tab_off),
-                         (const unsigned long long*)(E.ws + P->pack_prefix_off), (int)P->pack_jobs.size(), P->pack_total, fold ? 1 : 0, E.st));
+  const PackJob* tab = (const PackJob*)(E.ws + P->pack_tab_off);
+  const unsigned long long* prefix = (const unsigned long long*)(E.ws + P->pack_prefix_off);
+  const unsigned long long fwd_end = P->pack_group_end[fold ? PACK_FWD : PACK_FWD_TIED], grad_blocks = P->pack_total - P->pack_group_end[PACK_FWD_TIED];
+  hipStream_t gst = E.st;
+  if (!grad_ok && grad_blocks > 0 && !serial_mode()) {
+    const bool low = !P->tgraph_enabled;
+    hipStream_t* sp = low ? &P->side_bwd : &P->side;
+    if (!*sp) HIPCHK(create_side_stream(sp, low));
+    if (!P->ev_pack) {
+      HIPCHK(hipEventCreateWithFlags(&P->ev_pack_fork, hipEventDisableTiming));
+      HIPCHK(hipEventCreateWithFlags(&P->ev_pack, hipEventDisableTiming));
+    }
+    gst = *sp;
+    HIPCHK(hipEventRecord(P->ev_pack_fork, E.st));
+    HIPCHK(hipStreamWaitEvent(gst, P->ev_pack_fork, 0));
+  }
+  if (!fwd_ok) {
+    if (fold && !P->bn_jobs.empty())
+      HIPCHK(launch_bn_finalize_eval_all(E.params, E.buffers, E.ws, (const BnEvalJob*)(E.ws + P->bn_tab_off),
+                                         (const unsigned*)(E.ws + P->bn_prefix_off), (int)P->bn_jobs.size(), P->bn_total, 1e-5f, E.st));
+    HIPCHK(launch_pack_all(P->dtype, E.params, E.ws, tab, prefix, (int)P->pack_jobs.size(), 0, fwd_end, fold ? 1 : 0, E.st));
+  }
+  if (!grad_ok) {
+    if (gst == E.st && P->pack_pending) HIPCHK(hipStreamWaitEvent(E.st, P->ev_pack, 0));
+    HIPCHK(launch_pack_all(P->dtype, E.params, E.ws, tab, prefix, (int)P->pack_jobs.size(), P->pack_group_end[PACK_FWD_TIED], grad_blocks, 0, gst));
+    P->pack_pending = gst != E.st;
+    if (P->pack_pending) HIPCHK(hipEventRecord(P->ev_pack, gst));
+    P->packed_grad_valid = true;
+  }
   P->packed_valid = true; P->packed_fold = fold; P->packed_ws = E.ws; P->packed_params = E.params; P->packed_buffers = E.buffers;
   return OCTSEG_OK;
 }
diff --git a/oct_segmentation_amd/csrc/plan_geom.cpp b/oct_segmentation_amd/csrc/plan_geom.cpp
--- a/oct_segmentation_amd/csrc/plan_geom.cpp
+++ b/oct_segmentation_amd/csrc/plan_geom.cpp
@@ -188,19 +188,19 @@
   return im;
 }
 
-void tie_pack_jobs(const TieImages& im, const TieOffsets& at, size_t w_off, int Cout, int Cin, int Ca, int Cs, std::vector<PackJob>& jobs,
+void tie_pack_jobs(const TieImages& im, const TieOffsets& at, int tie, size_t w_off, int Cout, int Cin, int Ca, int Cs, std::vector<PackJob>& jobs,
                    std::vector<unsigned long long>& prefix, unsigned long long& total) {
   auto add = [&](size_t dst, int ntaps, int I, int c0, int tr, int tied, const ConvPackInfo& pk) {
-    PackJob j{w_off, dst, ntaps, Cout, I, tr, pk.BN, pk.RB, pk.nchunks, pk.ntiles, ~(size_t)0, Cin, c0, tied};
+    PackJob j{w_off, dst, ntaps, Cout, I, tr, pk.BN, pk.RB, pk.nchunks, pk.ntiles, ~(size_t)0, Cin, c0, tied, tr ? PACK_GRAD : PACK_FWD_TIED};
     prefix.push_back(total);
     jobs.push_back(j);
-    total += (unsigned long long)ntaps * pk.nchunks * pk.ntiles * pk.BN * (pk.RB / 16);
+    total += pack_job_blocks(j);
   };
-  add(at.fu, 16, Ca, 0, 0, 1, im.pk_fu);
-  add(at.du, im.du_taps(), Ca, 0, 1, im.du_masked ? 2 : 1, im.pk_du);
+  if (tie & 1) add(at.fu, 16, Ca, 0, 0, 1, im.pk_fu);
+  if (tie & 2) add(at.du, im.du_taps(), Ca, 0, 1, im.du_masked ? 2 : 1, im.pk_du);
   if (Cs > 0) {
-    add(at.fs, 9, Cs, Ca, 0, 0, im.pk_fs);
-    add(at.ds, 9, Cs, Ca, 1, 0, im.pk_ds);
+    if (tie & 1) add(at.fs, 9, Cs, Ca, 0, 0, im.pk_fs);
+    if (tie & 2) add(at.ds, 9, Cs, Ca, 1, 0, im.pk_ds);
   }
 }
 
diff --git a/oct_segmentation_amd/csrc/plan_internal.h b/oct_segmentation_amd/csrc/plan_internal.h
--- a/oct_segmentation_amd/csrc/plan_internal.h
+++ b/oct_segmentation_amd/csrc/plan_internal.h
@@ -75,7 +75,7 @@
 };
 TieImages tie_images(int dtype, const Geom& up, const Geom& skip);
 struct TieOffsets { size_t fu, du, fs, ds; };
-void tie_pack_jobs(const TieImages& im, const TieOffsets& at, size_t w_off, int Cout, int Cin, int Ca, int Cs, std::vector<PackJob>& jobs,
+void tie_pack_jobs(const TieImages& im, const TieOffsets& at, int tie, size_t w_off, int Cout, int Cin, int Ca, int Cs, std::vector<PackJob>& jobs,
                    std::vector<unsigned long long>& prefix, unsigned long long& total);
 int side_wgs();
 double layer_macs(const ConvLayer& L);
```

Result: no change. 260.9 frames/s, median of 6 (+0.6%).
